# lppllppl920/EndoscopyDepthEstimation-Pytorch

Hardware: AMD Instinct MI355X
Metric: train frame-pairs/sec at 256x320 bs=8 (higher is better)
Workload: dtype f32

## Files before the change

endoscopydepthestimation-pytorch_amd/csrc/common.h:

```cpp
#pragma once

#include <hip/hip_runtime.h>
#include <stdint.h>

#include <map>
#include <mutex>
#include <utility>

#include "../../include/endo_hip.h"

#define ENDO_CHECK(expr)                                 \
    do {                                                 \
        hipError_t _e = (expr);                          \
        if (_e != hipSuccess) return static_cast<int>(_e); \
    } while (0)

#define ENDO_LAUNCH_CHECK() ENDO_CHECK(hipGetLastError())

namespace endo {

constexpr int kWave = 64;

__device__ __forceinline__ double wave_sum(double v) {
#pragma unroll
    for (int off = 32; off > 0; off >>= 1) v += __shfl_down(v, off, kWave);
    return v;
}

__device__ __forceinline__ float wave_sum(float v) {
#pragma unroll
    for (int off = 32; off > 0; off >>= 1) v += __shfl_down(v, off, kWave);
    return v;
}

constexpr int kBnSlots = 8;

__device__ __forceinline__ int64_t bn_slot_offset(int64_t slot_stride) {
    return static_cast<int64_t>((blockIdx.x + 11 * blockIdx.z) & (kBnSlots - 1)) * slot_stride;
}

__device__ __forceinline__ double bn_slot_sum(const double* __restrict__ s, int64_t slot_stride) {
    if (slot_stride == 0) return s[0];
    double t = 0.0;
#pragma unroll
    for (int k = 0; k < kBnSlots; ++k) t += s[k * slot_stride];
    return t;
}

typedef short bf16x4_bits __attribute__((ext_vector_type(4)));

__device__ __forceinline__ bf16x4_bits pack_bf16x4(float a, float b, float c, float d) {
    typedef float f32x2_t __attribute__((ext_vector_type(2)));
    typedef __bf16 bf16x2_t __attribute__((ext_vector_type(2)));
    typedef unsigned u32x2_t __attribute__((ext_vector_type(2)));
    const bf16x2_t lo = __builtin_convertvector(f32x2_t{a, b}, bf16x2_t), hi = __builtin_convertvector(f32x2_t{c, d}, bf16x2_t);
    return __builtin_bit_cast(bf16x4_bits, u32x2_t{__builtin_bit_cast(unsigned, lo), __builtin_bit_cast(unsigned, hi)});
}

typedef __bf16 bf16x8_t __attribute__((ext_vector_type(8)));
typedef float f32x4_acc __attribute__((ext_vector_type(4)));

__device__ __forceinline__ bf16x8_t pack_bf16x8(float a, float b, float c, float d, float e, float f, float g, float h) {
    typedef float f32x8_t __attribute__((ext_vector_type(8)));
    return __builtin_convertvector(f32x8_t{a, b, c, d, e, f, g, h}, bf16x8_t);
}

typedef unsigned u32x4_bits __attribute__((ext_vector_type(4)));

template <int K>
__device__ __forceinline__ void block_sum_atomic(const float (&part)[K], double* dst, double* scratch) {
    const int lane = threadIdx.x & 63;
    const int wave = threadIdx.x >> 6;
    const int nwave = (blockDim.x + 63) >> 6;
#pragma unroll
    for (int k = 0; k < K; ++k) {
        double v = wave_sum(static_cast<double>(part[k]));
        if (lane == 0) scratch[k * nwave + wave] = v;
    }
    __syncthreads();
    if (threadIdx.x < K) {
        double v = 0.0;
        for (int i = 0; i < nwave; ++i) v += scratch[threadIdx.x * nwave + i];
        atomicAdd(dst + threadIdx.x, v);
    }
    __syncthreads();
}

__device__ __forceinline__ int xcd_remap(int b, int total) {
    const int xcd = b & 7, idx = b >> 3;
    const int q = total >> 3, r = total & 7;
    return (xcd < r ? xcd * (q + 1) : r * (q + 1) + (xcd - r) * q) + idx;
}

struct TileWalk {
    int begin, end, step;
};

__host__ __device__ __forceinline__ TileWalk persistent_tile_walk(int r, int bpg, int t_total) {
    if ((bpg & 7) == 0) {
        const int q = bpg >> 3, xcd = r & 7, idx = r >> 3;
        return {static_cast<int>(static_cast<int64_t>(xcd * q) * t_total / bpg) + idx, static_cast<int>(static_cast<int64_t>((xcd + 1) * q) * t_total / bpg), q};
    }
    return {static_cast<int>(static_cast<int64_t>(r) * t_total / bpg), static_cast<int>(static_cast<int64_t>(r + 1) * t_total / bpg), 1};
}

inline int persistent_bpg(int blocks, int groups, int tiles_per_group) {
    int bpg = blocks / groups;
    if (bpg >= 8) bpg &= ~7;
    if (bpg > tiles_per_group) bpg = tiles_per_group;
    return bpg < 1 ? 1 : bpg;
}

inline int device_cu_count() {
    static std::mutex mu;
    static std::map<int, int> cus;
    int dev = 0;
    (void)hipGetDevice(&dev);
    std::lock_guard<std::mutex> lock(mu);
    int& n = cus[dev];
    if (n <= 0 && hipDeviceGetAttribute(&n, hipDeviceAttributeMultiprocessorCount, dev) != hipSuccess) n = 0;
    return n > 0 ? n : 256;
}

inline hipError_t ensure_dynamic_lds(const void* fn, size_t bytes) {
    if (bytes <= 48 * 1024) return hipSuccess;
    static std::mutex mu;
    static std::map<std::pair<const void*, int>, size_t> given;
    int dev = 0;
    (void)hipGetDevice(&dev);
    std::lock_guard<std::mutex> lock(mu);
    size_t& g = given[{fn, dev}];
    if (bytes <= g) return hipSuccess;
    const hipError_t e = hipFuncSetAttribute(fn, hipFuncAttributeMaxDynamicSharedMemorySize, static_cast<int>(bytes));
    if (e == hipSuccess) g = bytes;
    return e;
}

template <typename... Params, typename... Args>
inline hipError_t launch_dyn(void (*kernel)(Params...), dim3 grid, dim3 block, size_t smem, hipStream_t stream, Args&&... args) {
    const hipError_t e = ensure_dynamic_lds(reinterpret_cast<const void*>(kernel), smem);
    if (e != hipSuccess) return e;
    kernel<<<grid, block, smem, stream>>>(std::forward<Args>(args)...);
    return hipGetLastError();
}

}

int endo_depth_scale_fwd_impl(const float* pred, const float* sparse_depth, const float* sparse_mask, float* scaled, float* ratio, double* stats,
                              int n, int hw, float eps, int zero, hipStream_t stream);
int endo_depth_scale_bwd_impl(const float* grad_scaled, const float* grad_ratio, const float* pred, const float* sparse_depth, const double* stats,
                              float* grad_pred, double* work, int n, int hw, float eps, int zero, hipStream_t stream);
int endo_sparse_l1_fwd_impl(const float* flows, const float* flows_hat, const float* mask, float* loss, double* stats, int n, int c, int hw,
                            float eps, int zero, hipStream_t stream);

int endo_consistency_phase(int phase, const float* depth_1, const float* depth_2, const float* boundaries, const float* t_1_wrt_2,
                           const float* r_1_wrt_2, const float* t_2_wrt_1, const float* r_2_wrt_1, const float* intrinsics, float dcl_weight,
                           float eps, float* loss, float* grad_depth_1, float* grad_depth_2, float* workspace, int n, int h, int w,
                           int zero_grads, hipStream_t stream);

namespace endo {

struct ProfScope {
    int family;
    hipStream_t stream;
    void* slot;
    ProfScope(int family, hipStream_t stream, double flops, double bytes);
    ~ProfScope();
};

enum ProfFamily {
    kProfConv3x3Dense = 0,
    kProfConv3x3Up = 1,
    kProfConv1x1Pool = 2,
    kProfConvFirst = 3,
    kProfConvFinal = 4,
    kProfDgradDense = 5,
    kProfWgradDense = 6,
    kProfDgradOther = 7,
    kProfWgradOther = 8,
    kProfSmall = 9,
    kProfGeometry = 10,
    kProfLoss = 11,
    kProfOptimizer = 12,
};

}
```

endoscopydepthestimation-pytorch_amd/csrc/dgrad_wino_kernels.h:

```cpp
#pragma once

#include "dgrad_block_kernels.h"

namespace endo {

constexpr int kWinoDgradSlice = 16 * 12 * 16;
constexpr int kWinoDgradMaxLayers = 48;

struct WinoDgradTable {
    int layers;
    int start[kWinoDgradMaxLayers + 1];
    int cin[kWinoDgradMaxLayers];
    int groups[kWinoDgradMaxLayers];
    int64_t w_off[kWinoDgradMaxLayers];
    int64_t u_off[kWinoDgradMaxLayers];
};

static __global__ void __launch_bounds__(256) dgrad_wino_weights_kernel(const WinoDgradTable t, const float* __restrict__ params, float* __restrict__ u,
                                                                 int layout1_blocks = 0) {
    const int total = t.start[t.layers];
    for (int item = blockIdx.x * blockDim.x + threadIdx.x; item < total; item += gridDim.x * blockDim.x) {
        int l = 0;
        while (item >= t.start[l + 1]) ++l;
        const int e = item - t.start[l];
        const int j = e & 15, c = (e >> 4) % 12, grp = (e >> 4) / 12;
        const int ci = grp * 16 + j;
        float g[3][3];
#pragma unroll
        for (int a = 0; a < 3; ++a)
#pragma unroll
            for (int b = 0; b < 3; ++b) g[a][b] = 0.f;
        if (ci < t.cin[l]) {
            const float* src = params + t.w_off[l] + (static_cast<int64_t>(c) * t.cin[l] + ci) * 9;
#pragma unroll
            for (int a = 0; a < 3; ++a)
#pragma unroll
                for (int b = 0; b < 3; ++b) g[a][b] = src[(2 - a) * 3 + (2 - b)];
        }
        float h[4][3];
#pragma unroll
        for (int b = 0; b < 3; ++b) {
            h[0][b] = g[0][b];
            h[1][b] = 0.5f * (g[0][b] + g[1][b] + g[2][b]);
            h[2][b] = 0.5f * (g[0][b] - g[1][b] + g[2][b]);
            h[3][b] = g[2][b];
        }
        if ((layout1_blocks >> (l >> 2)) & 1) {
            float* dst = u + t.u_off[l] + static_cast<int64_t>(grp) * kWinoDgradSlice + (c * 64 + j) * 4;
#pragma unroll
            for (int a = 0; a < 4; ++a)
                *reinterpret_cast<f32x4*>(dst + a * 64) = f32x4{h[a][0], 0.5f * (h[a][0] + h[a][1] + h[a][2]), 0.5f * (h[a][0] - h[a][1] + h[a][2]), h[a][2]};
            continue;
        }
        float* dst = u + t.u_off[l] + static_cast<int64_t>(grp) * kWinoDgradSlice + c * 16 + j;
#pragma unroll
        for (int a = 0; a < 4; ++a) {
            dst[(4 * a + 0) * 192] = h[a][0];
            dst[(4 * a + 1) * 192] = 0.5f * (h[a][0] + h[a][1] + h[a][2]);
            dst[(4 * a + 2) * 192] = 0.5f * (h[a][0] - h[a][1] + h[a][2]);
            dst[(4 * a + 3) * 192] = h[a][2];
        }
    }
}

template <int NL>
struct DgradWino8Geom {
    static constexpr int kThreads = 512;
    static constexpr int kTileX = 32, kTileY = 8;
    static constexpr int kRows = kTileY + 2, kCols = kTileX + 2;
    static constexpr int kPlane = kRows * kCols;
    static constexpr int kCS = 352;
    static_assert(kCS >= kPlane && kCS % 64 == 32, "dY map stride");
    static constexpr int kU = kWinoDgradSlice;
    static constexpr int kUUnits = kU / 4;
    static constexpr int kRed = 4 * 16 * 2;
    static constexpr size_t kBytes = sizeof(float) * (NL * 12 * kCS + 2 * 2 * kU + 2 * 2 * kRed);
    static_assert(kBytes <= 160 * 1024, "one block per CU");
};

template <int NL, int EXP = 0>
__global__ void __launch_bounds__(512, 2) dgrad_wino8_kernel(const DgradBlockParams p0, const float* __restrict__ u0, const float* __restrict__ u1,
                                                             const float* __restrict__ u2, const float* __restrict__ u3) {
    using G = DgradWino8Geom<NL>;
    typedef float f32x2 __attribute__((ext_vector_type(2)));
    const int grp = p0.group_n > 0 ? blockIdx.z / p0.group_n : 0;
    const int n = blockIdx.z - grp * p0.group_n;
    const DgradBlockParams& p = p0;
    const int64_t grp_off = grp * p0.gs;
    extern __shared__ __attribute__((aligned(16))) float smem[];
    float* s_g = smem;
    float* s_u = s_g + NL * 12 * G::kCS;
    float* s_red = s_u + 4 * G::kU;

    const int tid = threadIdx.x;
    const int lane = tid & 63;
    const int wave = __builtin_amdgcn_readfirstlane(tid >> 6);
    const int half = wave >> 2, w4 = wave & 3;
    const int th = tid & 255;
    const int li = lane & 15;
    const int lk = lane >> 4;
    const int tile = (gridDim.x & 7) == 0 ? xcd_remap(blockIdx.x, gridDim.x) : blockIdx.x;
    const int x0 = (tile % p.tiles_x) * G::kTileX;
    const int y0 = (tile / p.tiles_x) * G::kTileY;
    const int px = x0 + 8 * lk;
    const int py = y0 + 2 * w4;
    const int ngroups = p.count / 16;
    const int g_per = (ngroups + gridDim.y - 1) / gridDim.y;
    const int g_begin = blockIdx.y * g_per;
    const int g_end = min(ngroups, g_begin + g_per);
    if (g_begin >= g_end) return;
    const int npairs = (g_end - g_begin + 1) / 2;
    const int nsteps = npairs * NL;
    const float* const u_layer[4] = {u0, u1, u2, u3};

    {
        int goff = 0;
        bool ok = false;
        if (tid < G::kPlane) {
            const int ry = tid / G::kCols, rx = tid - ry * G::kCols;
            const int gy = y0 - 1 + ry, gx = x0 - 1 + rx;
            if (gy >= 0 && gy < p.h && gx >= 0 && gx < p.w) { ok = true; goff = gy * p.g_w + gx; }
        }
        const float* g_n = p.g + grp_off + n * p.g_ns;
        const int e0 = wave * 64;
        if (e0 < G::kPlane) {
            for (int c = 0; c < NL * 12; ++c) {
                const float* src = ok ? g_n + static_cast<int64_t>(c) * p.g_cs + goff : g_pad_consts + 4;
                if (e0 + lane < G::kPlane) __builtin_amdgcn_global_load_lds((gptr_t)src, (lptr_t)(s_g + c * G::kCS + e0), 4, 0, 0);
            }
        }
    }

    auto step_group = [&](int step) { return g_begin + 2 * (step / NL) + half; };
    auto issue_weights = [&](int step, int buf) {
        const int gq = step_group(step), l = step % NL;
        if (gq >= g_end) return;
        const float* src = u_layer[l] + static_cast<int64_t>(gq) * G::kU + 4 * th;
        float* dst = s_u + (half * 2 + buf) * G::kU + w4 * 256;
#pragma unroll
        for (int k = 0; k < 3; ++k)
            __builtin_amdgcn_global_load_lds((gptr_t)(src + k * 1024), (lptr_t)(dst + k * 1024), 16, 0, 0);
    };

    const float* x_n = p.x + grp_off + n * p.ns;
    float* out_n = p.out + grp_off + n * p.ns;
    f32x4 xc[2][2], dc[2][2], total[2][2];
#pragma unroll
    for (int r = 0; r < 2; ++r)
#pragma unroll
        for (int hh = 0; hh < 2; ++hh) total[r][hh] = f32x4{0.f, 0.f, 0.f, 0.f};
    issue_weights(0, 0);
    asm volatile("s_waitcnt vmcnt(0)" ::: "memory");
    __syncthreads();

    for (int step = 0; step < nsteps; ++step) {
        const int buf = step & 1;
        const int gq = step_group(step), l = step % NL;
        const bool active = gq < g_end;
        const bool last_layer = (l == NL - 1);
        const int co = gq * 16 + li;
        float scale = 0.f, beta = 0.f, mean = 0.f, rstd = 0.f;
        if (active) {
            if (l == 0) {
#pragma unroll
                for (int r = 0; r < 2; ++r)
#pragma unroll
                    for (int hh = 0; hh < 2; ++hh) {
                        const int64_t o = static_cast<int64_t>(co) * p.cs + static_cast<int64_t>(py + r) * p.w + px + 4 * hh;
                        if constexpr ((EXP & 1) != 0) {
                            xc[r][hh] = f32x4{0.1f * lane, 0.2f, -0.3f, 0.4f}; dc[r][hh] = f32x4{0.f, 0.f, 0.f, 0.f};
                        } else {
                            xc[r][hh] = *reinterpret_cast<const f32x4*>(x_n + o);
                            dc[r][hh] = co >= p.acc_from ? *reinterpret_cast<const f32x4*>(out_n + o) : f32x4{0.f, 0.f, 0.f, 0.f};
                        }
                    }
            }
            mean = p.saved[l][grp_off + 2 * co]; rstd = p.saved[l][grp_off + 2 * co + 1];
            scale = p.gamma[l][co] * rstd;
            beta = p.beta[l][co];
        }
        if (step + 1 < nsteps && (!(EXP & 8) || step == 0)) issue_weights(step + 1, buf ^ 1);
        if (active) {
            f32x4 acc[16];
            const float* ub = s_u + (half * 2 + buf) * G::kU;
#pragma unroll
            for (int quad = 0; quad < 3; ++quad) {
                const float* a_base = s_g + (l * 12 + quad * 4 + lk) * G::kCS + (2 * w4) * G::kCols + 2 * li;
                const float* b_base = ub + (quad * 4 + lk) * 16 + li;
                f32x2 lo[4], hi[4];
#pragma unroll
                for (int row = 0; row < 4; ++row) {
                    lo[row] = *reinterpret_cast<const f32x2*>(a_base + row * G::kCols);
                    hi[row] = *reinterpret_cast<const f32x2*>(a_base + row * G::kCols + 2);
                }
                f32x2 tl[4], th2[4];
                tl[0] = lo[0] - lo[2]; th2[0] = hi[0] - hi[2];
                tl[1] = lo[1] + lo[2]; th2[1] = hi[1] + hi[2];
                tl[2] = lo[2] - lo[1]; th2[2] = hi[2] - hi[1];
                tl[3] = lo[1] - lo[3]; th2[3] = hi[1] - hi[3];
#pragma unroll
                for (int a = 0; a < 4; ++a) {
                    const float c0 = tl[a][0], c1 = tl[a][1], c2 = th2[a][0], c3 = th2[a][1];
                    float v0 = c0 - c2, v1 = c1 + c2, v2 = c2 - c1, v3 = c1 - c3;
                    if constexpr ((EXP & 64) != 0) { v0 = lo[a][0]; v1 = lo[a][1]; v2 = hi[a][0]; v3 = hi[a][1]; }
                    const float b0 = b_base[(4 * a + 0) * 192], b1 = b_base[(4 * a + 1) * 192];
                    const float b2 = b_base[(4 * a + 2) * 192], b3 = b_base[(4 * a + 3) * 192];
                    if constexpr ((EXP & 32) != 0) {
                        if (quad == 0) {
                            acc[4 * a + 0] = f32x4{v0 * b0, 0.f, 0.f, 0.f}; acc[4 * a + 1] = f32x4{v1 * b1, 0.f, 0.f, 0.f};
                            acc[4 * a + 2] = f32x4{v2 * b2, 0.f, 0.f, 0.f}; acc[4 * a + 3] = f32x4{v3 * b3, 0.f, 0.f, 0.f};
                        } else {
                            acc[4 * a + 0][quad] += v0 * b0; acc[4 * a + 1][quad] += v1 * b1;
                            acc[4 * a + 2][quad] += v2 * b2; acc[4 * a + 3][quad] += v3 * b3;
                        }
                    } else
// ... 101 lines not shown
```

endoscopydepthestimation-pytorch_amd/csrc/net.hip:

```cpp
#include <new>
#include <vector>

#include "dgrad_kernels.h"
#include "dgrad_block_kernels.h"
#include "dgrad_newmap_kernels.h"
#include "td_dgrad_kernels.h"
#include "td_fwd_kernels.h"
#include "wgrad_taps_kernels.h"
#include "wgrad1x1_kernels.h"
#include "wgrad_nsplit_kernels.h"
#include "wgrad_f34_kernels.h"
#include "wgrad_subpix_kernels.h"
#include "wino_fwd_kernels.h"
#include "wino4_fwd_kernels.h"
#include "dgrad_wino_kernels.h"
#include "dgrad_wino3_kernels.h"


namespace endo {

int run_dgrad_wino3_nl4(const DgradBlockParams& p, const float* const* u, hipStream_t stream);
bool dgrad_wino3p_applies(const DgradBlockParams& p);
int run_dgrad_wino3p_nl4(const DgradBlockParams& p, const float* const* u, int blocks, double* fw_parts, int* blocks_used, hipStream_t stream);

constexpr int kGrowth = 12;
constexpr int kLayers = 4;
constexpr int kFirst = 48;
constexpr int kLevels = 5;
constexpr int kNew = kGrowth * kLayers;
constexpr float kBnEps = 1.0e-5f;
constexpr float kBnMomentum = 0.1f;
constexpr int kSideStreamFromLevel = 0;

struct ConvP { int64_t w, b; int cout, cin, ks; int64_t u; int64_t ud; };
struct BnP { int64_t g, b; int c; int64_t run; int64_t saved; };

struct Table {
    ConvP first, final_;
    ConvP down_conv[kLevels][kLayers], td_conv[kLevels], bott_conv[kLayers], tu_conv[kLevels], up_conv[kLevels][kLayers];
    BnP down_bn[kLevels][kLayers], td_bn[kLevels], bott_bn[kLayers], up_bn[kLevels][kLayers];
    std::vector<int64_t> param_offsets;
    std::vector<BnP*> bn_order;
    int64_t param_floats = 0, bn_floats = 0, bn_width_total = 0;
    WinoWeightTable wino;
    WinoWeightTable wino4;
    int64_t wino4_floats = 0;
    int64_t wino_floats = 0;
    WinoDgradTable wino_dgrad;
    int64_t wino_dgrad_floats = 0;
};

inline int down_in(int level) { return kFirst + kNew * level; }
inline int level_channels(int level) { return level < kLevels ? 144 + down_in(level) : 288 + kNew; }

static const Table& table() {
    static Table* t = [] {
        Table* tb = new Table();
        int64_t off = 0;
        auto conv = [&](ConvP& c, int cout, int cin, int ks) {
            c.cout = cout; c.cin = cin; c.ks = ks; c.u = -1; c.ud = -1;
            c.w = off; tb->param_offsets.push_back(off); off += static_cast<int64_t>(cout) * cin * ks * ks;
            c.b = off; tb->param_offsets.push_back(off); off += cout;
        };
        int64_t run = 0, saved = 0;
        auto bn = [&](BnP& b, int c) {
            b.c = c;
            b.g = off; tb->param_offsets.push_back(off); off += c;
            b.b = off; tb->param_offsets.push_back(off); off += c;
            b.run = run; run += 2 * c;
            b.saved = saved; saved += c;
            tb->bn_order.push_back(&b);
        };
        conv(tb->first, kFirst, 3, 3);
        for (int l = 0; l < kLevels; ++l)
            for (int j = 0; j < kLayers; ++j) { bn(tb->down_bn[l][j], down_in(l) + kGrowth * j); conv(tb->down_conv[l][j], kGrowth, down_in(l) + kGrowth * j, 3); }
        for (int l = 0; l < kLevels; ++l) { bn(tb->td_bn[l], down_in(l) + kNew); conv(tb->td_conv[l], down_in(l) + kNew, down_in(l) + kNew, 1); }
        for (int j = 0; j < kLayers; ++j) { bn(tb->bott_bn[j], 288 + kGrowth * j); conv(tb->bott_conv[j], kGrowth, 288 + kGrowth * j, 3); }
        for (int i = 0; i < kLevels; ++i) conv(tb->tu_conv[i], kNew, kNew, 3);
        for (int i = 0; i < kLevels; ++i) {
            const int l = kLevels - 1 - i;
            for (int j = 0; j < kLayers; ++j) { const int cin = 96 + down_in(l) + kGrowth * j; bn(tb->up_bn[i][j], cin); conv(tb->up_conv[i][j], kGrowth, cin, 3); }
        }
        conv(tb->final_, 1, 192, 1);
        tb->param_floats = off;
        tb->bn_floats = run;
        tb->bn_width_total = saved;
        {
            WinoWeightTable& wt = tb->wino;
            wt.layers = 0; wt.start[0] = 0;
            int64_t uoff = 0;
            auto add = [&](ConvP& c) {
                const int l = wt.layers++;
                c.u = uoff;
                wt.cin[l] = c.cin; wt.cout[l] = c.cout; wt.w_off[l] = c.w; wt.u_off[l] = uoff;
                wt.start[l + 1] = wt.start[l] + c.cin * 16;
                uoff += static_cast<int64_t>(c.cin) * kWinoUStride;
            };
            for (int l = 0; l < kLevels; ++l) for (int j = 0; j < kLayers; ++j) add(tb->down_conv[l][j]);
            for (int j = 0; j < kLayers; ++j) add(tb->bott_conv[j]);
            for (int i = 0; i < kLevels; ++i) for (int j = 0; j < kLayers; ++j) add(tb->up_conv[i][j]);
            tb->wino_floats = uoff;
            tb->wino4 = wt;
            int64_t u4 = 0;
            for (int l = 0; l < wt.layers; ++l) { tb->wino4.u_off[l] = u4; u4 += static_cast<int64_t>(wt.cin[l]) * kW4UStride; }
            tb->wino4_floats = u4;
        }
        {
            WinoDgradTable& wd = tb->wino_dgrad;
            wd.layers = 0; wd.start[0] = 0;
            int64_t uoff = 0;
            auto add = [&](ConvP& c, int base) {
                const int l = wd.layers++;
                c.ud = uoff;
                wd.cin[l] = c.cin; wd.groups[l] = base / 16; wd.w_off[l] = c.w; wd.u_off[l] = uoff;
                wd.start[l + 1] = wd.start[l] + 16 * wd.groups[l] * 12;
                uoff += static_cast<int64_t>(wd.groups[l]) * kWinoDgradSlice;
            };
            for (int l = 0; l < kLevels; ++l) for (int j = 0; j < kLayers; ++j) add(tb->down_conv[l][j], down_in(l));
            for (int j = 0; j < kLayers; ++j) add(tb->bott_conv[j], 288);
            for (int i = 0; i < kLevels; ++i) for (int j = 0; j < kLayers; ++j) add(tb->up_conv[i][j], 96 + down_in(kLevels - 1 - i));
            tb->wino_dgrad_floats = uoff;
        }
        return tb;
    }();
    return *t;
}

}

using namespace endo;

struct endo_net {
    int n, h, w;
    int groups;
    int64_t gs;
    struct Level { int h, w, t; int64_t plane; int64_t act, grad; int64_t sums; int64_t pq; } lv[kLevels + 1];
    int64_t pre_off;
    int64_t saved_off;
    int64_t idx_off[kLevels];
    int64_t sums_off;
    int64_t sums_bytes;
    int64_t tape_floats;
    int64_t partial_off;
    int64_t wino_off;
    int64_t wino4_off;
    int64_t pq_off;
    int64_t pq_floats;
    int64_t scratch_off;
    int64_t scratch_bytes;
    int64_t slot_stride;
    int64_t wg_scratch_off;
    int64_t tuw_scratch_off;
    int64_t wd_off;
    int64_t gplane_off;
    int64_t bias_parts_off;
    int64_t fw_parts_off;
    int64_t bias_parts_floats;
    int64_t gradws_floats;
    hipStream_t wstream;
    hipEvent_t ev_fork, ev_join;
    int opt[ENDO_OPT_COUNT];
};

namespace endo {


constexpr int kBiasPartChannels = 2048;
constexpr int kBiasPartLaunches = 64;
constexpr int kFwPartBlocks = 512;
struct BiasReduceTable {
    int n;
    struct Entry { const float* parts; float* bias; int count; int nparts; } e[kBiasPartLaunches];
};
struct BiasParts {
    BiasReduceTable table;
    int64_t used;
};

struct BnFin4 {
    const double* scratch[4];
    const float* saved[4];
    const float* gamma[4];
    float* ggamma[4];
    float* gbeta[4];
};

__global__ void __launch_bounds__(256) prep_dy_kernel(float* __restrict__ dbuf, const float* __restrict__ x, int64_t ns, int plane,
                                                      const float* __restrict__ pq_p, const float* __restrict__ pq_q,
                                                      float* bias_grad, int group_n, int64_t gs, const BnFin4 fin, int nl,
                                                      double count, int training, int64_t slot_stride,
                                                      const float* __restrict__ vg, const float* __restrict__ vw, float* __restrict__ parts) {
    __shared__ double scratch[4];
    const int c = blockIdx.y;
    const int grp = blockIdx.z / group_n, n = blockIdx.z - grp * group_n;
    float pc = pq_p[grp * gs + c], qc = pq_q[grp * gs + c];
    if (nl > 0) {
        const int64_t go = grp * gs;
        double dp = 0.0, dq = 0.0;
#pragma unroll
        for (int j = 0; j < 4; ++j) {
            if (j >= nl) break;
            const double s1 = bn_slot_sum(fin.scratch[j] + go / 2 + 2 * c, slot_stride);
            const double s2 = bn_slot_sum(fin.scratch[j] + go / 2 + 2 * c + 1, slot_stride);
            if (blockIdx.x == 0 && n == 0 && threadIdx.x == 0) {
                atomicAdd(fin.ggamma[j] + c, static_cast<float>(s2));
                atomicAdd(fin.gbeta[j] + c, static_cast<float>(s1));
            }
            if (training) {
                const double mean = fin.saved[j][go + 2 * c], rstd = fin.saved[j][go + 2 * c + 1];
                const double scale = fin.gamma[j][c] * rstd;
                const double k = scale * rstd * s2 / count;
                dp += static_cast<double>(static_cast<float>(-k));
                dq += static_cast<double>(static_cast<float>(-scale * s1 / count + k * mean));
            }
        }
        pc += static_cast<float>(dp);
        qc += static_cast<float>(dq);
    }
    const int64_t base = grp * gs + n * ns + static_cast<int64_t>(c) * plane;
    const float* vg_n = vg ? vg + grp * gs + static_cast<int64_t>(n) * plane : nullptr;
    const float wf = vg ? vw[c] : 0.f;
    float part = 0.f;
    if ((plane & 3) == 0 && !vg_n) {
        const int stride = gridDim.x * blockDim.x * 4;
        int i = (blockIdx.x * blockDim.x + threadIdx.x) * 4;
        for (; i + stride < plane; i += 2 * stride) {
            f32x4 g0 = *reinterpret_cast<const f32x4*>(dbuf + base + i);
            f32x4 g1 = *reinterpret_cast<const f32x4*>(dbuf + base + i + stride);
            const f32x4 x0 = *reinterpret_cast<const f32x4*>(x + base + i);
            const f32x4 x1 = *reinterpret_cast<const f32x4*>(x + base + i + stride);
#pragma unroll
            for (int e = 0; e < 4; ++e) { g0[e] += fmaf(pc, x0[e], qc); part += g0[e]; }
#pragma unroll
            for (int e = 0; e < 4; ++e) { g1[e] += fmaf(pc, x1[e], qc); part += g1[e]; }
            *reinterpret_cast<f32x4*>(dbuf + base + i) = g0;
            *reinterpret_cast<f32x4*>(dbuf + base + i + stride) = g1;
        }
        for (; i < plane; i += stride) {
            f32x4 g = *reinterpret_cast<const f32x4*>(dbuf + base + i);
            const f32x4 xv = *reinterpret_cast<const f32x4*>(x + base + i);
#pragma unroll
            for (int e = 0; e < 4; ++e) { g[e] += fmaf(pc, xv[e], qc); part += g[e]; }
            *reinterpret_cast<f32x4*>(dbuf + base + i) = g;
        }
    } else if ((plane & 3) == 0) {
        for (int i = (blockIdx.x * blockDim.x + threadIdx.x) * 4; i < plane; i += gridDim.x * blockDim.x * 4) {
            f32x4 g;
            if (vg_n) {
                const f32x4 gv = *reinterpret_cast<const f32x4*>(vg_n + i);
                g = f32x4{gv[0] * wf, gv[1] * wf, gv[2] * wf, gv[3] * wf};
            } else {
                g = *reinterpret_cast<const f32x4*>(dbuf + base + i);
            }
            const f32x4 xv = *reinterpret_cast<const f32x4*>(x + base + i);
#pragma unroll
            for (int e = 0; e < 4; ++e) { g[e] += fmaf(pc, xv[e], qc); part += g[e]; }
            *reinterpret_cast<f32x4*>(dbuf + base + i) = g;
        }
    } else {
        for (int i = blockIdx.x * blockDim.x + threadIdx.x; i < plane; i += gridDim.x * blockDim.x) {
            const float g = (vg_n ? vg_n[i] * wf : dbuf[base + i]) + fmaf(pc, x[base + i], qc);
            dbuf[base + i] = g;
            part += g;
        }
    }
    const int lane = threadIdx.x & 63, wave = threadIdx.x >> 6;
    double v = wave_sum(static_cast<double>(part));
    if (lane == 0) scratch[wave] = v;
    __syncthreads();
    if (threadIdx.x == 0 && bias_grad) {
        const float t = static_cast<float>(scratch[0] + scratch[1] + scratch[2] + scratch[3]);
        if (parts) parts[(static_cast<int64_t>(c) * gridDim.z + blockIdx.z) * gridDim.x + blockIdx.x] = t;
        else atomicAdd(bias_grad + c, t);
    }
}

__global__ void __launch_bounds__(256) bias_reduce_kernel(const BiasReduceTable tb) {
    const BiasReduceTable::Entry& e = tb.e[blockIdx.x];
    const int lane = threadIdx.x & 63, wave = threadIdx.x >> 6;
    for (int c = blockIdx.y * 4 + wave; c < e.count; c += gridDim.y * 4) {
        const float* src = e.parts + static_cast<int64_t>(c) * e.nparts;
        double t = 0.0;
        for (int i = lane; i < e.nparts; i += 64) t += static_cast<double>(src[i]);
        t = wave_sum(t);
        if (lane == 0) e.bias[c] += static_cast<float>(t);
    }
}

__global__ void bn_bwd_finalize_kernel(const double* __restrict__ scratch, const float* __restrict__ saved,
                                       const float* __restrict__ gamma, float* __restrict__ ggamma, float* __restrict__ gbeta,
                                       float* __restrict__ pq_p, float* __restrict__ pq_q, int c_count, double count, int training,
                                       int64_t gs, int64_t slot_stride) {
    scratch += blockIdx.y * (gs / 2); saved += blockIdx.y * gs; pq_p += blockIdx.y * gs; pq_q += blockIdx.y * gs;
    for (int c = blockIdx.x * blockDim.x + threadIdx.x; c < c_count; c += gridDim.x * blockDim.x) {
        const double s1 = bn_slot_sum(scratch + 2 * c, slot_stride), s2 = bn_slot_sum(scratch + 2 * c + 1, slot_stride);
        atomicAdd(ggamma + c, static_cast<float>(s2));
        atomicAdd(gbeta + c, static_cast<float>(s1));
        if (training) {
            const double mean = saved[2 * c], rstd = saved[2 * c + 1];
            const double scale = gamma[c] * rstd;
            const double k = scale * rstd * s2 / count;
            pq_p[c] += static_cast<float>(-k);
            pq_q[c] += static_cast<float>(-scale * s1 / count + k * mean);
        }
    }
}

__global__ void bn_bwd_finalize4_kernel(const BnFin4 a, int nl, float* __restrict__ pq_p, float* __restrict__ pq_q, int c_count, double count,
                                        int training, int64_t gs, int64_t slot_stride) {
    const int64_t go = blockIdx.y * gs;
    pq_p += go; pq_q += go;
    for (int c = blockIdx.x * blockDim.x + threadIdx.x; c < c_count; c += gridDim.x * blockDim.x) {
        double dp = 0.0, dq = 0.0;
#pragma unroll
        for (int j = 0; j < 4; ++j) {
            if (j >= nl) break;
            const double s1 = bn_slot_sum(a.scratch[j] + go / 2 + 2 * c, slot_stride);
            const double s2 = bn_slot_sum(a.scratch[j] + go / 2 + 2 * c + 1, slot_stride);
            atomicAdd(a.ggamma[j] + c, static_cast<float>(s2));
            atomicAdd(a.gbeta[j] + c, static_cast<float>(s1));
            if (training) {
                const double mean = a.saved[j][go + 2 * c], rstd = a.saved[j][go + 2 * c + 1];
                const double scale = a.gamma[j][c] * rstd;
                const double k = scale * rstd * s2 / count;
                dp += static_cast<double>(static_cast<float>(-k));
                dq += static_cast<double>(static_cast<float>(-scale * s1 / count + k * mean));
            }
        }
        if (training) {
            pq_p[c] += static_cast<float>(dp);
            pq_q[c] += static_cast<float>(dq);
        }
    }
}

__global__ void tu_phase_weights_kernel(const float* __restrict__ w, int cout, int cin, float* __restrict__ out) {
    constexpr int kPhW = 2 * 12 * 16 + 16;
    const int total = 2 * cin * 2 * 12 * 16;
    for (int i = blockIdx.x * blockDim.x + threadIdx.x; i < total; i += gridDim.x * blockDim.x) {
        const int lane16 = i & 15;
        const int slot = (i >> 4) % 12;
        const int t = (i / (16 * 12)) & 1;
        const int ci = (i / (16 * 12 * 2)) % cin;
        const int a = i / (16 * 12 * 2 * cin);
        int ctap, tile;
        if (slot < 3) { ctap = 0; tile = slot; } else if (slot < 9) { ctap = 1; tile = slot - 3; } else { ctap = 2; tile = slot - 9 + 3; }
        const int b = tile / 3, co = (tile % 3) * 16 + lane16;
        float v = 0.f;
        if (co < cout) {
            const float* src = w + (static_cast<int64_t>(co) * cin + ci) * 9;
            const int ky0 = a == 0 ? (t == 0 ? 0 : 1) : (t == 0 ? 0 : 2), ky1 = a == 0 ? (t == 0 ? 0 : 2) : (t == 0 ? 1 : 2);
            int kx0, kx1;
            if (b == 0) { kx0 = ctap == 0 ? 0 : 1; kx1 = ctap == 0 ? 0 : 2; }
            else { kx0 = ctap == 1 ? 0 : 2; kx1 = ctap == 1 ? 1 : 2; }
            for (int ky = ky0; ky <= ky1; ++ky)
                for (int kx = kx0; kx <= kx1; ++kx) v += src[ky * 3 + kx];
        }
        out[(static_cast<int64_t>(a) * cin + ci) * kPhW + (t * 12 + slot) * 16 + lane16] = v;
    }
}

__global__ void tu_subpix_dgrad_weights_kernel(const float* __restrict__ w, int cout, int cin, float* __restrict__ out) {
    const int pitch = 4 * cin + 16;
    const int total = 4 * cout * 4 * cin;
    for (int i = blockIdx.x * blockDim.x + threadIdx.x; i < total; i += gridDim.x * blockDim.x) {
        const int ci = i % cin;
        const int tap = (i / cin) & 3;
        const int co = (i / (4 * cin)) % cout;
        const int ph = i / (4 * cin * cout);
        const int alpha = ph >> 1, beta = ph & 1, tyi = tap >> 1, txi = tap & 1;
        const int ky0 = alpha == 0 ? (tyi == 0 ? 1 : 0) : (tyi == 0 ? 2 : 0), ky1 = alpha == 0 ? (tyi == 0 ? 2 : 0) : (tyi == 0 ? 2 : 1);
        const int kx0 = beta == 0 ? (txi == 0 ? 1 : 0) : (txi == 0 ? 2 : 0), kx1 = beta == 0 ? (txi == 0 ? 2 : 0) : (txi == 0 ? 2 : 1);
        const float* src = w + (static_cast<int64_t>(co) * cin + ci) * 9;
        float v = 0.f;
        for (int ky = ky0; ky <= ky1; ++ky)
            for (int kx = kx0; kx <= kx1; ++kx) v += src[ky * 3 + kx];
        out[static_cast<int64_t>(ph * cout + co) * pitch + tap * cin + ci] = v;
    }
}

__global__ void __launch_bounds__(256) finalize_partial_kernel(const float* __restrict__ partial, int64_t split_stride, int ksplit,
                                                               int64_t pns, int plane, const float* __restrict__ bias,
                                                               float* __restrict__ out, int64_t out_ns, double* out_sums,
                                                               int group_n, int64_t gs) {
    __shared__ double scratch[2 * 4];
    const int c = blockIdx.y;
    const int grp = blockIdx.z / group_n, n = blockIdx.z - grp * group_n;
    partial += grp * gs; out += grp * gs;
    if (out_sums) out_sums += grp * (gs / 2);
    const float b = bias[c];
    float part[2] = {0.f, 0.f};
    for (int i = blockIdx.x * blockDim.x + threadIdx.x; i < plane; i += gridDim.x * blockDim.x) {
        float v = b;
        for (int s = 0; s < ksplit; ++s) v += partial[s * split_stride + n * pns + static_cast<int64_t>(c) * plane + i];
        out[n * out_ns + static_cast<int64_t>(c) * plane + i] = v;
        part[0] += v;
        part[1] += v * v;
    }
    if (out_sums) block_sum_atomic<2>(part, out_sums + 2 * c, scratch);
}

__global__ void __launch_bounds__(256) final_fwd_kernel(const float* __restrict__ u, int64_t ns, int plane, int cin,
                                                        const float* __restrict__ wgt, const float* __restrict__ bias,
                                                        float* __restrict__ pre, float* __restrict__ out, int group_n, int64_t gs, int c_first) {
    __shared__ float s_w[192];
    for (int c = threadIdx.x; c < cin; c += blockDim.x) s_w[c] = wgt[c];
    __syncthreads();
    const int grp = blockIdx.y / group_n, n = blockIdx.y - grp * group_n;
    u += grp * gs;
    if (pre) pre += grp * gs;
    out += static_cast<int64_t>(grp) * group_n * plane;
    const bool vec = (plane & 3) == 0;
    if (vec) {
        for (int i = (blockIdx.x * blockDim.x + threadIdx.x) * 4; i < plane; i += gridDim.x * blockDim.x * 4) {
            f32x4 acc = {0.f, 0.f, 0.f, 0.f};
            if (c_first > 0) acc = *reinterpret_cast<const f32x4*>(pre + static_cast<int64_t>(n) * plane + i);
            const float* src = u + n * ns + i;
            for (int c = c_first; c < cin; ++c) {
                const f32x4 v = *reinterpret_cast<const f32x4*>(src + static_cast<int64_t>(c) * plane);
                const float wc = s_w[c];
                acc[0] = fmaf(v[0], wc, acc[0]); acc[1] = fmaf(v[1], wc, acc[1]);
                acc[2] = fmaf(v[2], wc, acc[2]); acc[3] = fmaf(v[3], wc, acc[3]);
            }
            const float b = bias[0];
            f32x4 o;
            for (int e = 0; e < 4; ++e) { acc[e] += b; o[e] = fabsf(acc[e]); }
            if (pre) *reinterpret_cast<f32x4*>(pre + static_cast<int64_t>(n) * plane + i) = acc;
            *reinterpret_cast<f32x4*>(out + static_cast<int64_t>(n) * plane + i) = o;
        }
    } else {
        for (int i = blockIdx.x * blockDim.x + threadIdx.x; i < plane; i += gridDim.x * blockDim.x) {
            float acc = c_first > 0 ? pre[static_cast<int64_t>(n) * plane + i] : 0.f;
            for (int c = c_first; c < cin; ++c) acc = fmaf(u[n * ns + static_cast<int64_t>(c) * plane + i], s_w[c], acc);
            acc += bias[0];
            if (pre) pre[static_cast<int64_t>(n) * plane + i] = acc;
            out[static_cast<int64_t>(n) * plane + i] = fabsf(acc);
        }
    }
}

__device__ __forceinline__ float sign_of(float v) { return v > 0.f ? 1.f : (v < 0.f ? -1.f : 0.f); }

__global__ void __launch_bounds__(256) final_g_kernel(const float* __restrict__ gout, const float* __restrict__ pre, float* __restrict__ g,
                                                      int plane, int group_n, int64_t gs) {
    const int grp = blockIdx.y / group_n, n = blockIdx.y - grp * group_n;
    gout += static_cast<int64_t>(blockIdx.y) * plane; pre += grp * gs + static_cast<int64_t>(n) * plane; g += grp * gs + static_cast<int64_t>(n) * plane;
    for (int i = blockIdx.x * blockDim.x + threadIdx.x; i < plane; i += gridDim.x * blockDim.x) g[i] = gout[i] * sign_of(pre[i]);
}

__global__ void __launch_bounds__(256) final_bwd_data_kernel(const float* __restrict__ gout, const float* __restrict__ pre,
                                                             const float* __restrict__ wgt, float* __restrict__ dbuf,
                                                             int64_t ns, int plane, int cin, int group_n, int64_t gs, int c_first) {
    __shared__ float s_w[192];
    for (int c = threadIdx.x; c < cin; c += blockDim.x) s_w[c] = wgt[c];
    __syncthreads();
    const int grp = blockIdx.y / group_n, n = blockIdx.y - grp * group_n;
    gout += static_cast<int64_t>(grp) * group_n * plane; pre += grp * gs; dbuf += grp * gs;
    for (int i = blockIdx.x * blockDim.x + threadIdx.x; i < plane; i += gridDim.x * blockDim.x) {
        const float g = gout[static_cast<int64_t>(n) * plane + i] * sign_of(pre[static_cast<int64_t>(n) * plane + i]);
        for (int c = c_first; c < cin; ++c) dbuf[n * ns + static_cast<int64_t>(c) * plane + i] = g * s_w[c];
    }
}

__global__ void __launch_bounds__(256) final_bwd_weight_kernel(const float* __restrict__ gout, const float* __restrict__ pre,
                                                               const float* __restrict__ u, int64_t ns, int plane, int cin,
                                                               int group_n, int64_t gs, float* __restrict__ gw, float* __restrict__ gb, int c_first) {
    __shared__ double scratch[4];
    const int c = c_first + blockIdx.x;
    const int grp = blockIdx.z / group_n, n = blockIdx.z - grp * group_n;
    const float* gp = gout + static_cast<int64_t>(blockIdx.z) * plane;
    const float* pp = pre + grp * gs + static_cast<int64_t>(n) * plane;
    const float* up = u + grp * gs + n * ns + static_cast<int64_t>(c < cin ? c : 0) * plane;
    float part = 0.f, part2 = 0.f;
    if ((plane & 3) == 0) {
        const int stride = gridDim.y * blockDim.x * 4;
        for (int i = (blockIdx.y * blockDim.x + threadIdx.x) * 4; i < plane; i += stride) {
            const f32x4 gv = *reinterpret_cast<const f32x4*>(gp + i);
            const f32x4 pv = *reinterpret_cast<const f32x4*>(pp + i);
            f32x4 uv = {1.f, 1.f, 1.f, 1.f};
            if (c < cin) uv = *reinterpret_cast<const f32x4*>(up + i);
            part += gv[0] * sign_of(pv[0]) * uv[0] + gv[1] * sign_of(pv[1]) * uv[1];
            part2 += gv[2] * sign_of(pv[2]) * uv[2] + gv[3] * sign_of(pv[3]) * uv[3];
        }
    } else {
        for (int i = blockIdx.y * blockDim.x + threadIdx.x; i < plane; i += gridDim.y * blockDim.x)
            part += gp[i] * sign_of(pp[i]) * (c < cin ? up[i] : 1.f);
    }
    const int lane = threadIdx.x & 63, wave = threadIdx.x >> 6;
    double v = wave_sum(static_cast<double>(part + part2));
    if (lane == 0) scratch[wave] = v;
    __syncthreads();
    if (threadIdx.x == 0) {
        const float t = static_cast<float>(scratch[0] + scratch[1] + scratch[2] + scratch[3]);
        if (c < cin) atomicAdd(gw + c, t); else atomicAdd(gb, t);
    }
}

__global__ void __launch_bounds__(64) final_w_reduce_kernel(const double* __restrict__ parts, int nblocks, int count, float* __restrict__ gw) {
    const int c = blockIdx.x;
    double t = 0.0;
    for (int b = threadIdx.x; b < nblocks; b += 64) t += parts[static_cast<int64_t>(b) * count + c];
    t = wave_sum(t);
    if (threadIdx.x == 0) atomicAdd(gw + c, static_cast<float>(t));
}

constexpr int kBlocks = 2 * kLevels + 1, kDense = kBlocks * kLayers;

enum class DenseFwd { Wino4, Wino2_32x16, Wino2_32x8, SplitK, Direct32x8, Direct16x8, DirectAuto };
struct FwdPlan {
    struct Dense {
        DenseFwd form;
        int ksplit;
        bool chunk_weights;
    } dense[kDense];
    bool bf16;
    bool wino4_weights;
    bool fuse_final;
    bool td_persistent[kLevels];
    bool tu_subpix[kLevels];
};

enum class NewMap { Bf16, Persistent, Vec16, Dword };
enum class BasePass { Block8, Block8Bf16, Wino3, Wino3Persistent, Wino8 };
enum class DenseWgrad { F34, NSplit, Taps, Direct };
enum class TdDgrad { Persistent, Runs128, Dma, Staged };
enum class TuWgrad { Subpix, Taps, Direct };
enum class TuDgrad { Subpix32x8, Subpix16x8, Subpix16x4, Plain };
enum class FirstWgrad { F34Prep, F34, Taps, Direct };
struct BwdPlan {
    struct Block {
        bool fused;
        NewMap newmap[kLayers];
        BasePass base;
        bool wino3_layout;
    } block[kBlocks];
    DenseWgrad wgrad[kDense];
    bool td_wgrad_dma[kLevels];
    TdDgrad td_dgrad[kLevels];
    TuWgrad tu_wgrad[kLevels];
    TuDgrad tu_dgrad[kLevels];
    int overlap;
    bool bf16_wgrad, bf16_dgrad;
    bool dgrad_weights;
    bool use_virt;
    bool virt_base;
    bool virt_base_w;
    int materialise;
    int c_first;
    FirstWgrad first;
};

struct Ctx {
    const endo_net* net;
    const float* params;
    float* bn_running;
    float* tape;
    float* grads;
    float* gradws;
    int training;
    hipStream_t stream;
    BiasParts* bias_parts = nullptr;
    const float* x = nullptr;
    const FwdPlan* fwd = nullptr;
    const BwdPlan* bwd = nullptr;

    int nt() const { return net->n * net->groups; }
    int fork_wgrad(Ctx& side, int level) const {
        side = *this;
        if (!net->wstream || !bwd->overlap || level < kSideStreamFromLevel) return 0;
        ENDO_CHECK(hipEventRecord(net->ev_fork, stream));
        ENDO_CHECK(hipStreamWaitEvent(net->wstream, net->ev_fork, 0));
        side.stream = net->wstream;
        return 0;
    }
    float* act(int level) const { return tape + net->lv[level].act; }
    float* gbuf(int level) const { return gradws + net->lv[level].grad; }
    double* sums(int level) const { return reinterpret_cast<double*>(reinterpret_cast<char*>(tape) + net->sums_off) + net->lv[level].sums; }
    double* out_sums(int level, int channel) const { return training ? sums(level) + 2 * channel : nullptr; }
    float* saved(const BnP& b) const { return tape + net->saved_off + 2 * b.saved; }
    double* scratch(const BnP& b) const { return reinterpret_cast<double*>(reinterpret_cast<char*>(gradws) + net->scratch_off) + 2 * b.saved; }
    float* pq_p(int level) const { return gradws + net->pq_off + 2 * net->lv[level].pq; }
    float* pq_q(int level) const { return pq_p(level) + net->lv[level].t; }
    uint8_t* idx(int level) const { return reinterpret_cast<uint8_t*>(tape) + net->idx_off[level]; }
};

static void fill_bn_in(const Ctx& c, ConvParams& p, const BnP& b, int level, int ic0) {
    const auto& lv = c.net->lv[level];
    p.in_sums = c.sums(level) + 2 * ic0;
    p.gamma = c.params + b.g;
    p.beta = c.params + b.b;
    p.running_mean = c.bn_running + b.run;
    p.running_var = c.bn_running + b.run + b.c;
    p.saved = c.tape ? c.saved(b) : nullptr;
    p.count = static_cast<double>(c.net->n) * lv.h * lv.w;
    p.eps = kBnEps;
    p.momentum = kBnMomentum;
    p.training = c.training;
}

static void fill_in(const Ctx& c, ConvParams& p, const float* base, int level, int ic0, int cin) {
    const auto& lv = c.net->lv[level];
    p.in = base + ic0 * lv.plane;
    p.in_ns = lv.t * lv.plane;
    p.in_cs = static_cast<int>(lv.plane);
    p.in_w = lv.w;
    p.cin = cin;
}

static void fill_out(const Ctx& c, ConvParams& p, float* base, int level, int oc0, int cout) {
    const auto& lv = c.net->lv[level];
    p.out = base + oc0 * lv.plane;
    p.out_ns = lv.t * lv.plane;
    p.out_cs = static_cast<int>(lv.plane);
    p.out_w = lv.w;
    p.cout = cout;
}

static void fill_grid(const Ctx& c, ConvParams& p, int level) {
    const auto& lv = c.net->lv[level];
    p.n = c.nt(); p.h = lv.h; p.w = lv.w;
    p.group_n = c.net->n; p.gs = c.net->gs; p.in_gs = c.net->gs; p.out_gs = c.net->gs;
}

static double conv_flops(const endo_net* net, int level, int cin, int cout, int ks) {
    return 2.0 * net->n * net->groups * net->lv[level].plane * cin * cout * ks * ks;
}

static void default_options(int (&opt)[ENDO_OPT_COUNT]) {
    opt[ENDO_OPT_WINO_FWD] = 5;
    opt[ENDO_OPT_WINO_DGRAD] = 3;
    opt[ENDO_OPT_DGRAD_VEC] = 2;
    opt[ENDO_OPT_WINO_MIN_TILES] = 1024;
    opt[ENDO_OPT_MFMA_BF16] = 0;
    opt[ENDO_OPT_WGRAD_OVERLAP] = 1;
    opt[ENDO_OPT_WGRAD_F34] = 1;
    opt[ENDO_OPT_FINAL_VIRTUAL] = 1;
    opt[ENDO_OPT_TD_PERSIST] = 3;
}
static int bf16_mask(const int* opt) { const int v = opt[ENDO_OPT_MFMA_BF16]; return v == 1 ? 7 : (v >> 1); }

struct DenseBlock { int level, ic0, c0; const BnP* bn; const ConvP* cv; bool base_overwrite; };
static DenseBlock dense_block(int b) {
    const Table& tb = table();
    if (b < kLevels) return {b, 48, down_in(b), tb.down_bn[b], tb.down_conv[b], false};
    if (b == kLevels) return {kLevels, 0, 288, tb.bott_bn, tb.bott_conv, true};
    const int i = b - kLevels - 1, l = kLevels - 1 - i;
    return {l, 0, 96 + down_in(l), tb.up_bn[i], tb.up_conv[i], l > 0};
}
static long tile_count(const Ctx& c, int level, int tx, int ty) {
    const auto& lv = c.net->lv[level];
    return static_cast<long>((lv.w + tx - 1) / tx) * ((lv.h + ty - 1) / ty) * c.nt();
}

static ConvParams dense_fwd_params(const Ctx& c, const DenseBlock& k, int j, DenseFwd form) {
    const ConvP& cv = k.cv[j];
    const int oc0 = k.ic0 + k.c0 + kGrowth * j;
    ConvParams p{};
    fill_grid(c, p, k.level);
    fill_in(c, p, c.act(k.level), k.level, k.ic0, cv.cin);
    fill_bn_in(c, p, k.bn[j], k.level, k.ic0);
    p.wgt = c.params + cv.w; p.bias = c.params + cv.b; p.w_cout = cv.cout; p.w_cin = cv.cin;
    fill_out(c, p, c.act(k.level), k.level, oc0, cv.cout);
    p.out_sums = c.out_sums(k.level, oc0);
    if (form == DenseFwd::Wino4) p.wgt = c.tape + c.net->wino4_off + cv.u / kWinoUStride * kW4UStride;
    if (form == DenseFwd::Wino2_32x16 || form == DenseFwd::Wino2_32x8) p.wgt = c.tape + c.net->wino_off + cv.u;
    return p;
}

static ConvParams td_fwd_params(const Ctx& c, int level) {
    const BnP& b = table().td_bn[level];
    const ConvP& cv = table().td_conv[level];
    const int next = level + 1;
    const int oc0 = next < kLevels ? 48 : 0;
    ConvParams p{};
    fill_grid(c, p, level);
    fill_in(c, p, c.act(level), level, 48, cv.cin);
    fill_bn_in(c, p, b, level, 48);
    p.wgt = c.params + cv.w; p.bias = c.params + cv.b; p.w_cout = cv.cout; p.w_cin = cv.cin;
    fill_out(c, p, c.act(next), next, oc0, cv.cout);
    p.out_idx = c.idx(level);
    p.idx_ns = static_cast<int64_t>(cv.cout) * c.net->lv[next].plane;
    p.out_sums = c.out_sums(next, oc0);
    return p;
}

static FwdPlan plan_fwd(const Ctx& c) {
    const int* opt = c.net->opt;
    const int mode = opt[ENDO_OPT_WINO_FWD];
    const long min_tiles = opt[ENDO_OPT_WINO_MIN_TILES];
    FwdPlan pl{};
    pl.bf16 = (bf16_mask(opt) & 2) != 0;
    pl.wino4_weights = !pl.bf16 && mode == 5;
    for (int b = 0; b < kBlocks; ++b) {
        const DenseBlock k = dense_block(b);
        const long t64x16 = tile_count(c, k.level, 64, 16), t32x16 = tile_count(c, k.level, 32, 16), t32x8 = tile_count(c, k.level, 32, 8);
        const long t16x16 = tile_count(c, k.level, 16, 16), t16x8 = tile_count(c, k.level, 16, 8);
        const bool big = t32x16 >= min_tiles, small = t32x8 >= (min_tiles * 3) / 4;
        const bool wino4_tiles = mode == 5 && !pl.bf16 && 2 * t64x16 >= min_tiles;
        const bool wino2_tiles = mode != 0 && !pl.bf16 && (big || small);
        for (int j = 0; j < kLayers; ++j) {
            FwdPlan::Dense& d = pl.dense[b * kLayers + j];
            const int nchunks = (k.cv[j].cin + 15) / 16;
            d.chunk_weights = !pl.bf16 && !wino4_tiles && !wino2_tiles;
            if (wino4_tiles && wino4_fwd_ok(dense_fwd_params(c, k, j, DenseFwd::Wino4))) {
                d.form = DenseFwd::Wino4;
            } else if (wino2_tiles && wino_fwd_ok(dense_fwd_params(c, k, j, DenseFwd::Wino2_32x16))) {
                d.form = big ? DenseFwd::Wino2_32x16 : DenseFwd::Wino2_32x8;
            } else if (t32x16 < 512 && t16x16 < 384 && t16x8 < 512 && nchunks >= 4) {
                int want = static_cast<int>(((t16x8 < 256 ? 512 : 768) + t16x8 - 1) / t16x8);
                if (want > nchunks) want = nchunks;
                const int per = (nchunks + want - 1) / want;
                d.form = DenseFwd::SplitK;
                d.ksplit = (nchunks + per - 1) / per;
            } else {
                d.form = (t32x16 < 1024 && t32x8 >= 1024) ? DenseFwd::Direct32x8
                       : (t32x16 < 1024 && t16x8 >= 768) ? DenseFwd::Direct16x8 : DenseFwd::DirectAuto;
            }
        }
    }
    pl.fuse_final = opt[ENDO_OPT_FINAL_VIRTUAL] && pl.dense[kDense - 1].form == DenseFwd::Wino4;
    for (int l = 0; l < kLevels; ++l) {
        pl.td_persistent[l] = (opt[ENDO_OPT_TD_PERSIST] & 2) && !pl.bf16 && c.training && td_fwd_ok(td_fwd_params(c, l));
        const ConvP& tu = table().tu_conv[kLevels - 1 - l];
        pl.tu_subpix[l] = c.net->lv[l + 1].w % 4 == 0 && tu.cout == kNew && tu.cin % 4 == 0;
    }
    return pl;
}

static int dense_fwd(const Ctx& c, int b, int j) {
    const DenseBlock k = dense_block(b);
    const FwdPlan::Dense& d = c.fwd->dense[b * kLayers + j];
    const ConvP& cv = k.cv[j];
    const auto& lv = c.net->lv[k.level];
    const int oc0 = k.ic0 + k.c0 + kGrowth * j;
    ConvParams p = dense_fwd_params(c, k, j, d.form);
    ProfScope prof(kProfConv3x3Dense, c.stream, conv_flops(c.net, k.level, cv.cin, cv.cout, 3),
                   4.0 * c.nt() * lv.plane * (cv.cin + cv.cout));
    const float* chunk_weights = d.chunk_weights ? c.tape + c.net->wino_off + cv.u : nullptr;
    const bool bf16 = c.fwd->bf16;
    switch (d.form) {
        case DenseFwd::Wino4:
            if (c.fwd->fuse_final && b == kBlocks - 1 && j == kLayers - 1) { p.fin_w = c.params + table().final_.w + k.ic0; p.fin_out = c.tape + c.net->pre_off; }
            return launch_wino4_fwd(p, c.stream);
        case DenseFwd::Wino2_32x16:
            return launch_wino_fwd<2, 4, 2>(p, c.stream);
        case DenseFwd::Wino2_32x8:
            return launch_wino_fwd<1, 4, 3>(p, c.stream);
        case DenseFwd::SplitK: {
            float* partial = c.tape + c.net->partial_off;
            p.ksplit = d.ksplit;
            p.split_stride = static_cast<int64_t>(c.net->n) * cv.cout * lv.plane;
            p.out = partial; p.out_ns = static_cast<int64_t>(cv.cout) * lv.plane;
            p.bias = nullptr; p.out_sums = nullptr;
            p.wgt_chunks = chunk_weights;
            int rc = bf16 ? launch_conv_dma<3, 16, 1, IN_BNRELU, EPI_FWD, 1, 2, 2, 1, 1>(p, c.stream)
                          : launch_conv_dma<3, 16, 1, IN_BNRELU, EPI_FWD, 1, 2, 2, 1>(p, c.stream);
            if (rc) return rc;
            int bx = static_cast<int>((lv.plane + 255) / 256);
            bx = bx > 8 ? 8 : bx;
            finalize_partial_kernel<<<dim3(bx, cv.cout, c.nt()), 256, 0, c.stream>>>(
                partial, p.split_stride, d.ksplit, p.out_ns, static_cast<int>(lv.plane), c.params + cv.b, c.act(k.level) + oc0 * lv.plane,
                lv.t * lv.plane, c.out_sums(k.level, oc0), c.net->n, c.net->gs);
            ENDO_LAUNCH_CHECK();
            return 0;
        }
        case DenseFwd::Direct32x8:
            return bf16 ? launch_conv_dma<3, 4, 1, IN_BNRELU, EPI_FWD, 2, 4, 2, 1, 1>(p, c.stream) : launch_conv_dma<3, 4, 1, IN_BNRELU, EPI_FWD, 2, 4, 2, 1>(p, c.stream);
        case DenseFwd::Direct16x8:
            return bf16 ? launch_conv_dma<3, 8, 1, IN_BNRELU, EPI_FWD, 1, 2, 2, 1, 1>(p, c.stream) : launch_conv_dma<3, 8, 1, IN_BNRELU, EPI_FWD, 1, 2, 2, 1>(p, c.stream);
        case DenseFwd::DirectAuto:
            if (bf16) return launch_conv_dma_auto<3, 4, 1, IN_BNRELU, EPI_FWD, 8, 2, 1, 1>(p, c.stream);
            p.wgt_chunks = chunk_weights;
            return launch_conv_dma_auto<3, 4, 1, IN_BNRELU, EPI_FWD, 8, 2, 1>(p, c.stream);
    }
    return ENDO_E_BADARG;
}

static int td_fwd(const Ctx& c, int level) {
    const ConvP& cv = table().td_conv[level];
    const ConvParams p = td_fwd_params(c, level);
    ProfScope prof(kProfConv1x1Pool, c.stream, conv_flops(c.net, level, cv.cin, cv.cout, 1),
                   4.0 * c.nt() * c.net->lv[level].plane * (cv.cin + cv.cout / 4.0));
    if (c.fwd->td_persistent[level]) return launch_td_fwd(p, device_cu_count(), c.stream);
    if (c.fwd->bf16) return launch_conv_dma_auto<1, 8, 3, IN_BNRELU, EPI_FWD_POOL, 4, 2, 1, 1>(p, c.stream);
    return launch_conv_dma_auto<1, 8, 3, IN_BNRELU, EPI_FWD_POOL, 4>(p, c.stream);
}

static int tu_fwd(const Ctx& c, int level, int src_level, int src_c0, const ConvP& cv) {
    ProfScope prof(kProfConv3x3Up, c.stream, conv_flops(c.net, level, cv.cin, cv.cout, 3),
                   4.0 * c.nt() * c.net->lv[level].plane * (cv.cin / 4.0 + cv.cout));
    if (c.fwd->tu_subpix[level]) {
        float* w3 = c.tape + c.net->partial_off;
        tu_phase_weights_kernel<<<(2 * cv.cin * 384 + 255) / 256, 256, 0, c.stream>>>(c.params + cv.w, cv.cout, cv.cin, w3);
        ENDO_LAUNCH_CHECK();
        ConvParams p{};
        fill_grid(c, p, src_level);
        fill_in(c, p, c.act(src_level), src_level, src_c0, cv.cin);
        p.wgt = w3; p.w_cout = 2 * cv.cout; p.w_cin = cv.cin;
        p.bias = c.params + cv.b;
        fill_out(c, p, c.act(level), level, 0, cv.cout);
        p.out_sums = c.out_sums(level, 0);
        return launch_conv_dma_vec<3, 4, 6, IN_PLAIN, EPI_FWD, 2, 4, 2, 1, 4, 0, 0, 2>(p, c.stream);
    }
    ConvParams p{};
    fill_grid(c, p, level);
    fill_in(c, p, c.act(src_level), src_level, src_c0, cv.cin);
    p.wgt = c.params + cv.w; p.bias = c.params + cv.b; p.w_cout = cv.cout; p.w_cin = cv.cin;
    fill_out(c, p, c.act(level), level, 0, cv.cout);
    p.out_sums = c.out_sums(level, 0);
    return launch_conv_dma_auto<3, 4, 3, IN_UPSAMPLE, EPI_FWD>(p, c.stream);
}

struct FinalVirt { const float* vg; const float* vw; float* gw; };

static int prep_dy(const Ctx& c, int level, int c0, int count, float* bias_grad, const BnFin4* fin = nullptr, int nl = 0, const FinalVirt* fv = nullptr) {
    const auto& lv = c.net->lv[level];
    BnFin4 none{};
    int bx = static_cast<int>((lv.plane + 4095) / 4096);
    bx = bx < 1 ? 1 : (bx > 32 ? 32 : bx);
    float* parts = nullptr;
    if (bias_grad && c.bias_parts) {
        BiasParts& bp = *c.bias_parts;
        const int64_t need = static_cast<int64_t>(count) * c.nt() * bx;
        if (bp.table.n >= kBiasPartLaunches || bp.used + need > c.net->bias_parts_floats) return ENDO_E_UNSUPPORTED;
        parts = c.gradws + c.net->bias_parts_off + bp.used;
        bp.table.e[bp.table.n++] = {parts, bias_grad, count, c.nt() * bx};
        bp.used += need;
    }
    ProfScope prof(kProfSmall, c.stream, 0.0, 12.0 * c.nt() * lv.plane * count);
    prep_dy_kernel<<<dim3(bx, count, c.nt()), 256, 0, c.stream>>>(c.gbuf(level) + c0 * lv.plane, c.act(level) + c0 * lv.plane,
                                                                     lv.t * lv.plane, static_cast<int>(lv.plane), c.pq_p(level) + c0,
                                                                     c.pq_q(level) + c0, bias_grad, c.net->n, c.net->gs, fin ? *fin : none, fin ? nl : 0,
                                                                     static_cast<double>(c.net->n) * lv.h * lv.w, c.training, c.net->slot_stride,
                                                                     fv ? fv->vg : nullptr, fv ? fv->vw + c0 : nullptr, parts);
    ENDO_LAUNCH_CHECK();
    return 0;
}

static int bn_finalize(const Ctx& c, const BnP& b, int level, int ic0, int first = 0, int count = -1) {
    const auto& lv = c.net->lv[level];
    if (count < 0) count = b.c - first;
    if (count <= 0) return 0;
    ProfScope prof(kProfSmall, c.stream, 0.0, 0.0);
    bn_bwd_finalize_kernel<<<dim3((count + 127) / 128, c.net->groups), 128, 0, c.stream>>>(c.scratch(b) + 2 * first, c.saved(b) + 2 * first, c.params + b.g + first,
                                                                       c.grads + b.g + first, c.grads + b.b + first,
                                                                       c.pq_p(level) + ic0 + first, c.pq_q(level) + ic0 + first, count,
                                                                       static_cast<double>(c.net->n) * lv.h * lv.w, c.training, c.net->gs, c.net->slot_stride);
    ENDO_LAUNCH_CHECK();
    return 0;
}

static void fill_wgrad_grid(const Ctx& c, WgradParams& p, int level) {
    const auto& lv = c.net->lv[level];
    p.n = c.nt(); p.h = lv.h; p.w = lv.w;
    p.group_n = c.net->n; p.gs = c.net->gs; p.in_gs = c.net->gs;
    p.tiles_x = (lv.w + kWgTileX - 1) / kWgTileX;
    p.tiles_y = (lv.h + kWgTileY - 1) / kWgTileY;
}

static WgradParams dense_wgrad_params(const Ctx& c, const DenseBlock& k, int j) {
    const auto& lv = c.net->lv[k.level];
    const BnP& b = k.bn[j];
    const ConvP& cv = k.cv[j];
    const int oc0 = k.ic0 + k.c0 + kGrowth * j;
    WgradParams p{};
    fill_wgrad_grid(c, p, k.level);
    p.in = c.act(k.level) + k.ic0 * lv.plane; p.in_ns = lv.t * lv.plane; p.in_cs = static_cast<int>(lv.plane); p.in_w = lv.w; p.cin = cv.cin;
    p.saved = c.saved(b); p.gamma = c.params + b.g; p.beta = c.params + b.b;
    p.dy = c.gbuf(k.level) + oc0 * lv.plane; p.dy_ns = lv.t * lv.plane; p.dy_cs = static_cast<int>(lv.plane); p.dy_w = lv.w; p.cout = cv.cout;
    p.dw = c.grads + cv.w;
    return p;
}

static void fill_dgrad_block(const Ctx& c, DgradBlockParams& p, int level) {
    const auto& lv = c.net->lv[level];
    p.n = c.nt(); p.h = lv.h; p.w = lv.w;
    p.group_n = c.net->n; p.gs = c.net->gs; p.slot_stride = c.net->slot_stride;
    p.g_ns = lv.t * lv.plane; p.g_cs = static_cast<int>(lv.plane); p.g_w = lv.w;
    p.ns = lv.t * lv.plane; p.cs = static_cast<int>(lv.plane);
}

static DgradBlockParams newmap_params(const Ctx& c, const DenseBlock& k, int j, BnFin4* a = nullptr) {
    const auto& lv = c.net->lv[k.level];
    const int nl = kLayers - j;
    const int t0 = k.c0 + kGrowth * (j - 1);
    DgradBlockParams p{};
    fill_dgrad_block(c, p, k.level);
    p.g = c.gbuf(k.level) + (k.ic0 + k.c0 + kGrowth * j) * lv.plane;
    p.x = c.act(k.level) + (k.ic0 + t0) * lv.plane;
    p.out = c.gbuf(k.level) + (k.ic0 + t0) * lv.plane;
    p.count = kGrowth;
    p.acc_from = 0;
    p.w_ci_off = t0;
    for (int l = 0; l < nl; ++l) {
        const BnP& b = k.bn[j + l];
        p.wgt[l] = c.params + k.cv[j + l].w; p.w_cin[l] = k.cv[j + l].cin;
        p.saved[l] = c.saved(b) + 2 * t0; p.gamma[l] = c.params + b.g + t0; p.beta[l] = c.params + b.b + t0;
        p.scratch[l] = c.scratch(b) + 2 * t0;
        if (a) { a->scratch[l] = p.scratch[l]; a->saved[l] = p.saved[l]; a->gamma[l] = p.gamma[l]; a->ggamma[l] = c.grads + b.g + t0; a->gbeta[l] = c.grads + b.b + t0; }
    }
    return p;
}

static DgradBlockParams base_pass_params(const Ctx& c, const DenseBlock& k) {
    const auto& lv = c.net->lv[k.level];
    DgradBlockParams p{};
    fill_dgrad_block(c, p, k.level);
    p.g = c.gbuf(k.level) + (k.ic0 + k.c0) * lv.plane;
    p.x = c.act(k.level) + k.ic0 * lv.plane;
    p.out = c.gbuf(k.level) + k.ic0 * lv.plane;
    p.count = k.c0;
    p.acc_from = k.base_overwrite ? k.c0 : 0;
    p.w_ci_off = 0;
    for (int j = 0; j < kLayers; ++j) {
        p.wgt[j] = c.params + k.cv[j].w; p.w_cin[j] = k.cv[j].cin;
        p.saved[j] = c.saved(k.bn[j]); p.gamma[j] = c.params + k.bn[j].g; p.beta[j] = c.params + k.bn[j].b;
        p.scratch[j] = c.scratch(k.bn[j]);
    }
    return p;
}

static WgradParams td_wgrad_params(const Ctx& c, int level) {
    const BnP& b = table().td_bn[level];
    const ConvP& cv = table().td_conv[level];
    const int next = level + 1, oc0 = next < kLevels ? 48 : 0;
    const auto& lv = c.net->lv[level];
    const auto& nx = c.net->lv[next];
    WgradParams p{};
    fill_wgrad_grid(c, p, level);
    p.in = c.act(level) + 48 * lv.plane; p.in_ns = lv.t * lv.plane; p.in_cs = static_cast<int>(lv.plane); p.in_w = lv.w; p.cin = cv.cin;
    p.saved = c.saved(b); p.gamma = c.params + b.g; p.beta = c.params + b.b;
    p.dy = c.gbuf(next) + oc0 * nx.plane; p.dy_ns = nx.t * nx.plane; p.dy_cs = static_cast<int>(nx.plane); p.dy_w = nx.w; p.cout = cv.cout;
    p.dy_idx = c.idx(level); p.idx_ns = static_cast<int64_t>(cv.cout) * nx.plane;
    p.dw = c.grads + cv.w;
    return p;
}

static ConvParams td_dgrad_params(const Ctx& c, int level) {
    const BnP& b = table().td_bn[level];
    const ConvP& cv = table().td_conv[level];
    const int next = level + 1, oc0 = next < kLevels ? 48 : 0;
    const auto& lv = c.net->lv[level];
    ConvParams p{};
    fill_grid(c, p, level);
    fill_in(c, p, c.gbuf(next), next, oc0, cv.cout);
    p.in_idx = c.idx(level); p.idx_ns = static_cast<int64_t>(cv.cout) * c.net->lv[next].plane;
    p.wgt = c.params + cv.w; p.w_cout = cv.cout; p.w_cin = cv.cin;
    fill_out(c, p, c.gbuf(level), level, 48, cv.cin);
    p.x = c.act(level) + 48 * lv.plane; p.x_ns = lv.t * lv.plane; p.x_cs = static_cast<int>(lv.plane);
    p.bn_saved = c.saved(b); p.bn_gamma = c.params + b.g; p.bn_beta = c.params + b.b;
    p.bn_scratch = c.scratch(b); p.bn_slot_stride = c.net->slot_stride;
    p.acc_from = 0;
    return p;
}

static WgradParams tu_wgrad_params(const Ctx& c, int level, bool subpix) {
    const ConvP& cv = table().tu_conv[kLevels - 1 - level];
    const int src_level = level + 1, src_c0 = src_level == kLevels ? 288 : 96 + down_in(src_level);
    const auto& lv = c.net->lv[level];
    const auto& sv = c.net->lv[src_level];
    WgradParams p{};
    fill_wgrad_grid(c, p, level);
    p.in = c.act(src_level) + src_c0 * sv.plane; p.in_ns = sv.t * sv.plane; p.in_cs = static_cast<int>(sv.plane); p.in_w = sv.w; p.cin = cv.cin;
    p.dy = c.gbuf(level); p.dy_ns = lv.t * lv.plane; p.dy_cs = static_cast<int>(lv.plane); p.dy_w = lv.w; p.cout = cv.cout;
    p.dw = c.grads + cv.w;
    if (subpix) { p.h = sv.h; p.w = sv.w; }
    return p;
}

static WgradParams first_wgrad_params(const Ctx& c) {
    const auto& lv = c.net->lv[0];
    WgradParams p{};
    fill_wgrad_grid(c, p, 0);
    p.in = c.x; p.in_ns = 3 * lv.plane; p.in_cs = static_cast<int>(lv.plane); p.in_w = lv.w; p.cin = 3;
    p.in_gs = c.net->n * p.in_ns;
    p.dy = c.gbuf(0) + 48 * lv.plane; p.dy_ns = lv.t * lv.plane; p.dy_cs = static_cast<int>(lv.plane); p.dy_w = lv.w; p.cout = kFirst;
    p.dw = c.grads + table().first.w;
    return p;
}

static BwdPlan plan_bwd(const Ctx& c) {
    const int* opt = c.net->opt;
    const int wino_dgrad = opt[ENDO_OPT_WINO_DGRAD];
    const long min_tiles = opt[ENDO_OPT_WINO_MIN_TILES];
    BwdPlan pl{};
    pl.overlap = opt[ENDO_OPT_WGRAD_OVERLAP];
    pl.bf16_wgrad = (bf16_mask(opt) & 1) != 0;
    pl.bf16_dgrad = (bf16_mask(opt) & 4) != 0;
    const bool f34 = opt[ENDO_OPT_WGRAD_F34] && !pl.bf16_wgrad;
    const long f34_min_tiles = min_tiles / 4;
    pl.dgrad_weights = wino_dgrad != 0 && !pl.bf16_dgrad;
    for (int b = 0; b < kBlocks; ++b) {
        const DenseBlock k = dense_block(b);
        const auto& lv = c.net->lv[k.level];
        BwdPlan::Block& bl = pl.block[b];
        const DgradBlockParams base = base_pass_params(c, k);
        bl.fused = dgrad_block_ok(base);
        const long wtiles = static_cast<long>(lv.w / 32) * (lv.h / 8) * c.nt();
        if (pl.bf16_dgrad) bl.base = BasePass::Block8Bf16;
        else if (wino_dgrad != 0 && dgrad_wino_ok(base) && wtiles >= min_tiles)
            bl.base = !((wino_dgrad == 1 || wino_dgrad == 3) && dgrad_wino3_ok(base)) ? BasePass::Wino8
                    : (wino_dgrad == 3 && dgrad_wino3p_applies(base)) ? BasePass::Wino3Persistent : BasePass::Wino3;
        else bl.base = BasePass::Block8;
        bl.wino3_layout = bl.base == BasePass::Wino3 || bl.base == BasePass::Wino3Persistent;
        for (int j = 1; j < kLayers; ++j) {
            const DgradBlockParams p = newmap_params(c, k, j);
            const bool vec = dgrad_block_vec_ok(p);
            bl.newmap[j] = (pl.bf16_dgrad && vec) ? NewMap::Bf16 : (vec && opt[ENDO_OPT_DGRAD_VEC] >= 2 && dgrad_newmap_ok(p)) ? NewMap::Persistent
                         : (vec && opt[ENDO_OPT_DGRAD_VEC] != 0) ? NewMap::Vec16 : NewMap::Dword;
        }
        for (int j = 0; j < kLayers; ++j) {
            const WgradParams p = dense_wgrad_params(c, k, j);
            pl.wgrad[b * kLayers + j] = (f34 && wgrad_f34_ok(p, f34_min_tiles)) ? DenseWgrad::F34 : wgrad_nsplit_ok(p) ? DenseWgrad::NSplit
                                      : wgrad_taps_ok(p) ? DenseWgrad::Taps : DenseWgrad::Direct;
        }
    }
    for (int l = 0; l < kLevels; ++l) {
        const auto& sv = c.net->lv[l + 1];
        pl.td_wgrad_dma[l] = wgrad1x1_dma_ok(td_wgrad_params(c, l));
        const ConvParams td = td_dgrad_params(c, l);
        const bool persist = (opt[ENDO_OPT_TD_PERSIST] & 1) && !pl.bf16_dgrad;
        pl.td_dgrad[l] = (persist && td_dgrad_ok(td)) ? TdDgrad::Persistent : (persist && sv.w % 4 != 0 && td_dgrad_small_ok(td)) ? TdDgrad::Runs128
                       : sv.w % 4 == 0 ? TdDgrad::Dma : TdDgrad::Staged;
        const ConvP& tu = table().tu_conv[kLevels - 1 - l];
        pl.tu_wgrad[l] = tu_wgrad_subpix_ok(tu_wgrad_params(c, l, true)) ? TuWgrad::Subpix : wgrad_taps_ok(tu_wgrad_params(c, l, false), true) ? TuWgrad::Taps : TuWgrad::Direct;
        pl.tu_dgrad[l] = !(sv.w % 4 == 0 && tu.cin == kNew && tu.cout == kNew) ? TuDgrad::Plain : tile_count(c, l + 1, 32, 8) >= 1024 ? TuDgrad::Subpix32x8
                       : tile_count(c, l + 1, 16, 8) >= 512 ? TuDgrad::Subpix16x8 : TuDgrad::Subpix16x4;
    }
    const BwdPlan::Block& last = pl.block[kBlocks - 1];
    const int last_base = dense_block(kBlocks - 1).c0;
    pl.use_virt = opt[ENDO_OPT_FINAL_VIRTUAL] && last.fused;
    pl.virt_base = pl.use_virt && last.wino3_layout;
    pl.virt_base_w = pl.use_virt && last.base == BasePass::Wino3Persistent;
    pl.materialise = !pl.use_virt ? 192 : (pl.virt_base ? 0 : last_base);
    pl.c_first = pl.virt_base_w ? last_base : 0;
    const WgradParams first = first_wgrad_params(c);
    pl.first = (f34 && wgrad_f34_raw_ok(first, f34_min_tiles)) ? (opt[ENDO_OPT_FINAL_VIRTUAL] ? FirstWgrad::F34Prep : FirstWgrad::F34)
             : wgrad_taps_ok(first) ? FirstWgrad::Taps : FirstWgrad::Direct;
    return pl;
}

static int dense_wgrad(const Ctx& c, int b, int j, F34ReduceBatch* batch = nullptr, int slice = 0) {
    const DenseBlock k = dense_block(b);
    const ConvP& cv = k.cv[j];
    const auto& lv = c.net->lv[k.level];
    const WgradParams p = dense_wgrad_params(c, k, j);
    float* scratch = c.gradws + c.net->wg_scratch_off;
    ProfScope prof(kProfWgradDense, c.stream, conv_flops(c.net, k.level, cv.cin, cv.cout, 3), 4.0 * c.nt() * lv.plane * (cv.cin + cv.cout));
    switch (c.bwd->wgrad[b * kLayers + j]) {
        case DenseWgrad::F34: return launch_wgrad_f34(p, scratch + (batch ? slice : 0) * kF34ScratchFloats, c.stream, batch);
        case DenseWgrad::NSplit: return launch_wgrad_nsplit(p, scratch, c.stream, c.bwd->bf16_wgrad);
        case DenseWgrad::Taps: return c.bwd->bf16_wgrad ? launch_wgrad_taps<12, IN_BNRELU, 1>(p, c.stream) : launch_wgrad_taps<12, IN_BNRELU>(p, c.stream);
        case DenseWgrad::Direct: return launch_wgrad<3, 1, IN_BNRELU, DY_PLAIN>(p, c.stream);
    }
    return ENDO_E_BADARG;
}

static int dense_bwd(const Ctx& c, int b, int j, int acc_from) {
    const DenseBlock k = dense_block(b);
    const BnP& bn = k.bn[j];
    const ConvP& cv = k.cv[j];
    const int level = k.level, ic0 = k.ic0, oc0 = k.ic0 + k.c0 + kGrowth * j;
    const auto& lv = c.net->lv[level];
    int rc = prep_dy(c, level, oc0, cv.cout, c.grads + cv.b);
    if (rc) return rc;
    {
        Ctx cw;
        rc = c.fork_wgrad(cw, level);
        if (rc) return rc;
        rc = dense_wgrad(cw, b, j);
        if (rc) return rc;
    }
    {
        ConvParams p{};
        fill_grid(c, p, level);
        fill_in(c, p, c.gbuf(level), level, oc0, cv.cout);
        p.wgt = c.params + cv.w; p.w_cout = cv.cout; p.w_cin = cv.cin;
        fill_out(c, p, c.gbuf(level), level, ic0, cv.cin);
        p.x = c.act(level) + ic0 * lv.plane; p.x_ns = lv.t * lv.plane; p.x_cs = static_cast<int>(lv.plane);
        p.bn_saved = c.saved(bn); p.bn_gamma = c.params + bn.g; p.bn_beta = c.params + bn.b;
        p.bn_scratch = c.scratch(bn); p.bn_slot_stride = c.net->slot_stride;
        p.acc_from = acc_from - ic0;
        ProfScope prof(kProfDgradDense, c.stream, conv_flops(c.net, level, cv.cin, cv.cout, 3), 4.0 * c.nt() * lv.plane * (3.0 * cv.cin + cv.cout));
        rc = launch_dgrad_dense_auto(p, c.stream);
        if (rc) return rc;
    }
    return bn_finalize(c, bn, level, ic0);
}

template <int NL>
static int launch_newmap(NewMap form, const DgradBlockParams& p, hipStream_t stream) {
    switch (form) {
        case NewMap::Bf16: return launch_dgrad_block<NL, 2, 3, 1, 0, 4, 1>(p, stream);
        case NewMap::Persistent: return launch_dgrad_newmap<NL>(p, stream);
        case NewMap::Vec16: return launch_dgrad_block<NL, 2, 3, 1, 0, 4>(p, stream);
        case NewMap::Dword: return launch_dgrad_block<NL, 2, 3>(p, stream);
    }
    return ENDO_E_BADARG;
}

static int dense_block_bwd(const Ctx& c, int b, const FinalVirt* fv = nullptr) {
    const DenseBlock k = dense_block(b);
    const BwdPlan::Block& bl = c.bwd->block[b];
    const int level = k.level, ic0 = k.ic0, c0 = k.c0, new0 = ic0 + c0;
    const auto& lv = c.net->lv[level];
    if (!bl.fused) {
        for (int j = kLayers - 1; j >= 0; --j) {
            const int acc_from = (j == kLayers - 1 && k.base_overwrite) ? new0 : 0;
            int rc = dense_bwd(c, b, j, acc_from < ic0 ? ic0 : acc_from);
            if (rc) return rc;
        }
        return 0;
    }
    BnFin4 pending{};
    int pending_nl = 0;
    F34ReduceBatch red{};
    for (int j = kLayers - 1; j >= 0; --j) {
        int rc = prep_dy(c, level, new0 + kGrowth * j, kGrowth, c.grads + k.cv[j].b, &pending, pending_nl, (fv && j == kLayers - 1) ? fv : nullptr);
        if (rc) return rc;
        const bool defer = c.bwd->overlap == 2;
        if (!defer || j == 0) {
            Ctx cw;
            rc = c.fork_wgrad(cw, level);
            if (rc) return rc;
            for (int jj = defer ? kLayers - 1 : j; jj >= j; --jj) {
                rc = dense_wgrad(cw, b, jj, &red, jj);
                if (rc) return rc;
            }
            if (j == 0 && red.count > 0) {
                ProfScope prof(kProfSmall, cw.stream, 0.0, 0.0);
                rc = launch_wgrad_f34_reduce_batch(red, cw.stream);
                if (rc) return rc;
            }
        }
        if (j > 0) {
            const int nl = kLayers - j;
            BnFin4 a{};
            DgradBlockParams p = newmap_params(c, k, j, &a);
            if (fv) { p.vg = fv->vg; p.vw = fv->vw + ic0 + p.w_ci_off; }
            ProfScope prof(kProfDgradDense, c.stream, 2.0 * c.nt() * lv.plane * kGrowth * kGrowth * 9 * nl,
                           4.0 * c.nt() * lv.plane * (3.0 * kGrowth + kGrowth * nl));
            rc = nl == 1 ? launch_newmap<1>(bl.newmap[j], p, c.stream) : nl == 2 ? launch_newmap<2>(bl.newmap[j], p, c.stream) : launch_newmap<3>(bl.newmap[j], p, c.stream);
            if (rc) return rc;
            pending = a;
            pending_nl = nl;
        }
    }
    {
        DgradBlockParams p = base_pass_params(c, k);
        const bool virt = fv && c.bwd->virt_base;
        if (virt) { p.vg = fv->vg; p.vw = fv->vw + ic0; }
        ProfScope prof(kProfDgradDense, c.stream, 2.0 * c.nt() * lv.plane * c0 * kGrowth * 9 * kLayers,
                       4.0 * c.nt() * lv.plane * (3.0 * c0 + kGrowth * kLayers));
        const float* ub = c.gradws + c.net->wd_off;
        const float* const u[4] = {ub + k.cv[0].ud, ub + k.cv[1].ud, ub + k.cv[2].ud, ub + k.cv[3].ud};
        int rc = 0;
        switch (bl.base) {
            case BasePass::Block8Bf16: rc = launch_dgrad_block8<4, 1>(p, c.stream); break;
            case BasePass::Block8: rc = launch_dgrad_block8<4>(p, c.stream); break;
            case BasePass::Wino8: rc = launch_dgrad_wino8<4>(p, u, c.stream); break;
            case BasePass::Wino3: rc = run_dgrad_wino3_nl4(p, u, c.stream); break;
            case BasePass::Wino3Persistent: {
                double* fwp = (virt && c.bwd->virt_base_w) ? reinterpret_cast<double*>(c.gradws + c.net->fw_parts_off) : nullptr;
                int used = 0;
                rc = run_dgrad_wino3p_nl4(p, u, std::min(device_cu_count(), kFwPartBlocks), fwp, &used, c.stream);
                if (rc == 0 && fwp) {
                    final_w_reduce_kernel<<<c0, 64, 0, c.stream>>>(fwp, used, c0, fv->gw + ic0);
                    ENDO_LAUNCH_CHECK();
                }
                break;
            }
        }
        if (rc) return rc;
    }
    {
        BnFin4 a;
        for (int j = 0; j < kLayers; ++j) {
            a.scratch[j] = c.scratch(k.bn[j]); a.saved[j] = c.saved(k.bn[j]); a.gamma[j] = c.params + k.bn[j].g;
            a.ggamma[j] = c.grads + k.bn[j].g; a.gbeta[j] = c.grads + k.bn[j].b;
        }
        ProfScope prof(kProfSmall, c.stream, 0.0, 0.0);
        bn_bwd_finalize4_kernel<<<dim3((c0 + 127) / 128, c.net->groups), 128, 0, c.stream>>>(a, kLayers, c.pq_p(level) + ic0, c.pq_q(level) + ic0, c0,
                                                                         static_cast<double>(c.net->n) * lv.h * lv.w, c.training, c.net->gs,
                                                                         c.net->slot_stride);
        ENDO_LAUNCH_CHECK();
    }
    return 0;
}

static int td_bwd(const Ctx& c, int level) {
    const BnP& b = table().td_bn[level];
    const ConvP& cv = table().td_conv[level];
    const int next = level + 1;
    const auto& lv = c.net->lv[level];
    int rc = prep_dy(c, next, next < kLevels ? 48 : 0, cv.cout, c.grads + cv.b);
    if (rc) return rc;
    {
        const WgradParams p = td_wgrad_params(c, level);
        Ctx cw;
        rc = c.fork_wgrad(cw, level);
        if (rc) return rc;
        ProfScope prof(kProfWgradOther, cw.stream, conv_flops(c.net, level, cv.cin, cv.cout, 1), 4.0 * c.nt() * lv.plane * cv.cin);
        rc = !c.bwd->td_wgrad_dma[level] ? launch_wgrad1x1(p, cw.stream) : c.bwd->bf16_wgrad ? launch_wgrad1x1_dma<1>(p, cw.stream) : launch_wgrad1x1_dma<0>(p, cw.stream);
        if (rc) return rc;
    }
    {
        const ConvParams p = td_dgrad_params(c, level);
        ProfScope prof(kProfDgradOther, c.stream, conv_flops(c.net, level, cv.cin, cv.cout, 1), 4.0 * c.nt() * lv.plane * 3.0 * cv.cin);
        switch (c.bwd->td_dgrad[level]) {
            case TdDgrad::Persistent: rc = launch_td_dgrad(p, device_cu_count(), c.stream); break;
            case TdDgrad::Runs128: rc = launch_td_dgrad_small(p, c.stream); break;
            case TdDgrad::Dma: rc = c.bwd->bf16_dgrad ? launch_conv_dma_auto<1, 16, 2, IN_UNPOOL, EPI_DGRAD_BN, 4, 2, 1, 1>(p, c.stream)
                                                      : launch_conv_dma_auto<1, 16, 2, IN_UNPOOL, EPI_DGRAD_BN, 4>(p, c.stream); break;
            case TdDgrad::Staged: rc = launch_conv_auto<1, 16, 3, IN_UNPOOL, EPI_DGRAD_BN, 4>(p, c.stream); break;
        }
        if (rc) return rc;
    }
    return bn_finalize(c, b, level, 48);
}

static int tu_bwd(const Ctx& c, int level, int src_level, int src_c0, const ConvP& cv) {
    const auto& lv = c.net->lv[level];
    int rc = prep_dy(c, level, 0, cv.cout, c.grads + cv.b);
    if (rc) return rc;
    {
        const TuWgrad form = c.bwd->tu_wgrad[level];
        const WgradParams p = tu_wgrad_params(c, level, form == TuWgrad::Subpix);
        Ctx cw;
        rc = c.fork_wgrad(cw, level);
        if (rc) return rc;
        ProfScope prof(kProfWgradOther, cw.stream, conv_flops(c.net, level, cv.cin, cv.cout, 3), 4.0 * c.nt() * lv.plane * (cv.cin / 4.0 + cv.cout));
        rc = form == TuWgrad::Subpix ? launch_tu_wgrad_subpix(p, c.gradws + c.net->wg_scratch_off, cw.stream)
           : form == TuWgrad::Taps ? launch_wgrad_taps<12, IN_UPSAMPLE>(p, cw.stream) : launch_wgrad<3, 1, IN_UPSAMPLE, DY_PLAIN>(p, cw.stream);
        if (rc) return rc;
    }
    ProfScope prof(kProfDgradOther, c.stream, conv_flops(c.net, level, cv.cin, cv.cout, 3), 4.0 * c.nt() * lv.plane * (cv.cout + cv.cin / 4.0));
    const TuDgrad form = c.bwd->tu_dgrad[level];
    if (form == TuDgrad::Plain) {
        ConvParams p{};
        fill_grid(c, p, level);
        fill_in(c, p, c.gbuf(level), level, 0, cv.cout);
        p.wgt = c.params + cv.w; p.w_cout = cv.cout; p.w_cin = cv.cin;
        fill_out(c, p, c.gbuf(src_level), src_level, src_c0, cv.cin);
        return launch_conv_dma_auto<3, 4, 3, IN_PLAIN, EPI_DGRAD_SUMPOOL, 4>(p, c.stream);
    }
    float* wd = c.gradws + c.net->tuw_scratch_off;
    tu_subpix_dgrad_weights_kernel<<<(16 * cv.cout * cv.cin + 255) / 256, 256, 0, c.stream>>>(c.params + cv.w, cv.cout, cv.cin, wd);
    ENDO_LAUNCH_CHECK();
    ConvParams p{};
    fill_grid(c, p, src_level);
    fill_in(c, p, c.gbuf(level), level, 0, 4 * cv.cout);
    p.sub_c = cv.cout;
    p.wgt = wd; p.w_cout = cv.cin; p.w_cin = 4 * cv.cout;
    fill_out(c, p, c.gbuf(src_level), src_level, src_c0, cv.cin);
    if (form == TuDgrad::Subpix32x8) return launch_conv_dma_vec<3, 8, 3, IN_SUBPIX, EPI_FWD, 2, 4, 2, 1, 1>(p, c.stream);
    if (form == TuDgrad::Subpix16x8) return launch_conv_dma_vec<3, 8, 3, IN_SUBPIX, EPI_FWD, 1, 2, 2, 1, 1>(p, c.stream);
    return launch_conv_dma_vec<3, 8, 3, IN_SUBPIX, EPI_FWD, 1, 1, 2, 1, 1>(p, c.stream);
}

static int64_t align_up(int64_t v, int64_t a) { return (v + a - 1) / a * a; }

}

extern "C" int endo_net_create_grouped(endo_net** out, int n, int h, int w, int groups) {
    if (!out || n <= 0 || h <= 0 || w <= 0 || groups <= 0) return ENDO_E_BADARG;
    if (groups > kMaxGroups) return ENDO_E_UNSUPPORTED;
    if ((h % 32) != 0 || (w % 32) != 0) return ENDO_E_UNSUPPORTED;
    const Table& tb = table();
    endo_net* net = new (std::nothrow) endo_net();
    if (!net) return ENDO_E_BADARG;
    net->n = n; net->h = h; net->w = w; net->groups = groups;
    net->wstream = nullptr; net->ev_fork = nullptr; net->ev_join = nullptr;
    default_options(net->opt);
    int64_t off = 0, sums = 0, pq = 0;
    for (int l = 0; l <= kLevels; ++l) {
        auto& lv = net->lv[l];
        lv.h = h >> l; lv.w = w >> l; lv.t = level_channels(l);
        lv.plane = static_cast<int64_t>(lv.h) * lv.w;
        lv.act = off; lv.grad = off;
        off += align_up(static_cast<int64_t>(n) * lv.t * lv.plane, 64);
        lv.sums = sums; sums += 2 * lv.t;
        lv.pq = pq; pq += lv.t;
    }
    const int64_t acts = off;
    net->pre_off = off; off += align_up(static_cast<int64_t>(n) * h * w, 64);
    net->saved_off = off; off += align_up(2 * tb.bn_width_total, 64);
    int64_t byte_off = off * 4;
    for (int l = 0; l < kLevels; ++l) {
        net->idx_off[l] = byte_off;
        byte_off += align_up(static_cast<int64_t>(n) * (down_in(l) + kNew) * net->lv[l + 1].plane, 256);
    }
    net->sums_off = byte_off;
    net->sums_bytes = sums * 8;
    byte_off += align_up(net->sums_bytes, 256);
    net->partial_off = byte_off / 4;
    byte_off += static_cast<int64_t>(kGrowth) * 163840 * 4;
    net->wino_off = byte_off / 4;
    byte_off += align_up(tb.wino_floats * 4, 256);
    net->wino4_off = byte_off / 4;
    byte_off += align_up(tb.wino4_floats * 4, 256);
    net->tape_floats = byte_off / 4;
    net->pq_off = acts;
    net->pq_floats = 2 * pq;
    net->scratch_off = align_up((acts + net->pq_floats) * 4, 256);
    net->slot_stride = align_up(tb.bn_width_total * 2, 32);
    net->scratch_bytes = net->slot_stride * 8 * kBnSlots;
    net->wg_scratch_off = (net->scratch_off + align_up(net->scratch_bytes, 256)) / 4;
    net->tuw_scratch_off = net->wg_scratch_off + std::max(std::max(kNsScratchFloats, kSpScratchFloats), 4 * kF34ScratchFloats);
    net->wd_off = align_up(net->tuw_scratch_off + 4 * kNew * (4 * kNew + 16), 64);
    net->gplane_off = align_up(net->wd_off + tb.wino_dgrad_floats, 64);
    net->bias_parts_off = net->gplane_off + align_up(static_cast<int64_t>(n) * h * w, 64);
    net->bias_parts_floats = static_cast<int64_t>(kBiasPartChannels) * n * groups * 32;
    {
        int launches = 1, channels = tb.first.cout;
        for (int l = 0; l < kLevels; ++l) {
            for (int j = 0; j < kLayers; ++j) { launches += 2; channels += tb.down_conv[l][j].cout + tb.up_conv[l][j].cout; }
            launches += 2; channels += tb.td_conv[l].cout + tb.tu_conv[l].cout;
        }
        for (int j = 0; j < kLayers; ++j) { ++launches; channels += tb.bott_conv[j].cout; }
        if (launches > kBiasPartLaunches || channels > kBiasPartChannels) { delete net; return ENDO_E_UNSUPPORTED; }
    }
    net->fw_parts_off = net->bias_parts_off + align_up(net->bias_parts_floats, 64);
    net->gradws_floats = net->fw_parts_off + 2 * static_cast<int64_t>(kFwPartBlocks) * 192;
    net->gs = align_up(net->tape_floats > net->gradws_floats ? net->tape_floats : net->gradws_floats, 64);
    *out = net;
    return 0;
}

extern "C" int endo_net_create(endo_net** out, int n, int h, int w) { return endo_net_create_grouped(out, n, h, w, 1); }

static bool option_id_ok(int id) { return id >= 0 && id < ENDO_OPT_COUNT && id != 6; }

extern "C" int endo_net_set_option(endo_net* net, int option_id, int value) {
    if (!net || !option_id_ok(option_id)) return ENDO_E_BADARG;
    const int old = net->opt[option_id];
    net->opt[option_id] = value;
    return old;
}

extern "C" int endo_net_get_option(const endo_net* net, int option_id) {
    if (!net || !option_id_ok(option_id)) return ENDO_E_BADARG;
    return net->opt[option_id];
}

extern "C" void endo_net_destroy(endo_net* net) {
    if (!net) return;
    if (net->ev_fork) (void)hipEventDestroy(net->ev_fork);
    if (net->ev_join) (void)hipEventDestroy(net->ev_join);
    if (net->wstream) (void)hipStreamDestroy(net->wstream);
    delete net;
}
extern "C" int64_t endo_net_param_floats(void) { return table().param_floats; }
extern "C" int64_t endo_net_bn_floats(void) { return table().bn_floats; }
extern "C" int64_t endo_net_tape_floats(const endo_net* net) { return !net ? 0 : (net->groups > 1 ? net->groups * net->gs : net->tape_floats); }
extern "C" int64_t endo_net_gradws_floats(const endo_net* net) { return !net ? 0 : (net->groups > 1 ? net->groups * net->gs : net->gradws_floats); }
extern "C" int endo_net_groups(const endo_net* net) { return net ? net->groups : 0; }
extern "C" int64_t endo_net_group_stride(const endo_net* net) { return net ? net->gs : 0; }
extern "C" int64_t endo_net_param_offset(int index) {
    const Table& tb = table();
    if (index < 0 || index >= static_cast<int>(tb.param_offsets.size())) return -1;
    return tb.param_offsets[index];
}
extern "C" int64_t endo_net_bn_offset(int bn_index, int which) {
    const Table& tb = table();
    if (bn_index < 0 || bn_index >= static_cast<int>(tb.bn_order.size()) || which < 0 || which > 1) return -1;
    return tb.bn_order[bn_index]->run + which * tb.bn_order[bn_index]->c;
}
extern "C" int endo_net_level_channels(int level) { return (level < 0 || level > kLevels) ? -1 : level_channels(level); }
extern "C" int64_t endo_net_act_offset(const endo_net* net, int level) { return (!net || level < 0 || level > kLevels) ? -1 : net->lv[level].act; }

extern "C" int64_t endo_net_tape_offset(const endo_net* net, int what, int index) {
    if (!net) return -1;
    const Table& tb = table();
    switch (what) {
        case ENDO_TAPE_PRE: return net->pre_off;
        case ENDO_TAPE_BN_SAVED:
            if (index < 0 || index >= static_cast<int>(tb.bn_order.size())) return -1;
            return net->saved_off + 2 * tb.bn_order[index]->saved;
        case ENDO_TAPE_POOL:
            if (index < 0 || index >= kLevels) return -1;
            return net->idx_off[index];
        default: return -1;
    }
}

extern "C" int endo_net_fwd(endo_net* net, const float* params, float* bn_running, const float* x, float* out, float* tape,
                            int training, void* stream_) {
    if (!net || !params || !bn_running || !x || !out || !tape) return ENDO_E_BADARG;
    const Table& tb = table();
    Ctx c{net, params, bn_running, tape, nullptr, nullptr, training, static_cast<hipStream_t>(stream_)};
    const FwdPlan plan = plan_fwd(c);
    c.fwd = &plan;
    for (int g = 0; g < net->groups; ++g)
        ENDO_CHECK(hipMemsetAsync(reinterpret_cast<char*>(tape + g * net->gs) + net->sums_off, 0, net->sums_bytes, c.stream));
    if (!plan.bf16) {
        ProfScope prof(kProfSmall, c.stream, 0.0, 4.0 * (tb.wino_floats + tb.wino_floats * 9 / 16));
        WinoWeightTable wt = tb.wino;
        for (int l = 0; l < wt.layers; ++l) wt.mode[l] = plan.dense[l].chunk_weights ? 1 : 0;
        wino_fwd_weights_kernel<<<(wt.start[wt.layers] + 255) / 256, 256, 0, c.stream>>>(wt, params, tape + net->wino_off);
        ENDO_LAUNCH_CHECK();
        if (plan.wino4_weights) wino4_fwd_weights_kernel<<<(tb.wino4.start[tb.wino4.layers] + 255) / 256, 256, 0, c.stream>>>(tb.wino4, params, tape + net->wino4_off);
        ENDO_LAUNCH_CHECK();
    }
    int rc;
    {
        ConvParams p{};
        fill_grid(c, p, 0);
        p.in = x; p.in_ns = 3 * net->lv[0].plane; p.in_cs = static_cast<int>(net->lv[0].plane); p.in_w = net->w; p.cin = 3;
        p.in_gs = net->n * p.in_ns;
        p.wgt = params + tb.first.w; p.bias = params + tb.first.b; p.w_cout = kFirst; p.w_cin = 3;
        fill_out(c, p, c.act(0), 0, 48, kFirst);
        p.out_sums = c.out_sums(0, 48);
        ProfScope prof(kProfConvFirst, c.stream, conv_flops(net, 0, 3, kFirst, 3), 4.0 * c.nt() * net->lv[0].plane * (3 + kFirst));
        rc = launch_conv_dma_auto<3, 4, 3, IN_PLAIN, EPI_FWD>(p, c.stream);
        if (rc) return rc;
    }
    for (int b = 0; b < kBlocks; ++b) {
        if (b > kLevels) {
            const int i = b - kLevels - 1, l = kLevels - 1 - i;
            rc = tu_fwd(c, l, l + 1, (i == 0) ? 288 : 96 + down_in(l + 1), tb.tu_conv[i]);
            if (rc) return rc;
        }
        for (int j = 0; j < kLayers; ++j) {
            rc = dense_fwd(c, b, j);
            if (rc) return rc;
        }
        if (b < kLevels) {
            rc = td_fwd(c, b);
            if (rc) return rc;
        }
    }
    {
        const auto& lv = net->lv[0];
        const int c_first = plan.fuse_final ? 96 + down_in(0) + kGrowth * (kLayers - 1) : 0;
        ProfScope prof(kProfConvFinal, c.stream, 2.0 * c.nt() * lv.plane * 192, 4.0 * c.nt() * lv.plane * (194 - c_first));
        int bx = static_cast<int>((lv.plane / 4 + 255) / 256);
        bx = bx < 1 ? 1 : bx;
        final_fwd_kernel<<<dim3(bx, c.nt()), 256, 0, c.stream>>>(c.act(0), lv.t * lv.plane, static_cast<int>(lv.plane), 192,
                                                                 params + tb.final_.w, params + tb.final_.b, tape + net->pre_off, out,
                                                                 net->n, net->gs, c_first);
        ENDO_LAUNCH_CHECK();
    }
    return 0;
}

extern "C" int endo_net_bwd(endo_net* net, const float* params, const float* x, const float* tape, const float* grad_out,
                            float* grads, float* gradws, int training, void* stream_) {
    if (!net || !params || !x || !tape || !grad_out || !grads || !gradws) return ENDO_E_BADARG;
    const Table& tb = table();
    Ctx c{net, params, nullptr, const_cast<float*>(tape), grads, gradws, training, static_cast<hipStream_t>(stream_)};
    c.x = x;
    const BwdPlan plan = plan_bwd(c);
    c.bwd = &plan;
    BiasParts bias_parts{};
    c.bias_parts = &bias_parts;
    if (!net->wstream) {
        ENDO_CHECK(hipStreamCreateWithFlags(&net->wstream, hipStreamNonBlocking));
        ENDO_CHECK(hipEventCreateWithFlags(&net->ev_fork, hipEventDisableTiming));
        ENDO_CHECK(hipEventCreateWithFlags(&net->ev_join, hipEventDisableTiming));
    }
    for (int g = 0; g < net->groups; ++g)
        ENDO_CHECK(hipMemsetAsync(gradws + g * net->gs + net->pq_off, 0,
                                  static_cast<size_t>(net->scratch_off + net->scratch_bytes - net->pq_off * 4), c.stream));
    if (plan.dgrad_weights) {
        ProfScope prof(kProfSmall, c.stream, 0.0, 4.0 * 2.0 * tb.wino_dgrad_floats);
        int layout1_blocks = 0;
        for (int b = 0; b < kBlocks; ++b) layout1_blocks |= plan.block[b].wino3_layout ? 1 << b : 0;
        dgrad_wino_weights_kernel<<<(tb.wino_dgrad.start[tb.wino_dgrad.layers] + 255) / 256, 256, 0, c.stream>>>(tb.wino_dgrad, params, gradws + net->wd_off, layout1_blocks);
        ENDO_LAUNCH_CHECK();
    }
    int rc;
    const FinalVirt virt{gradws + net->gplane_off, params + tb.final_.w, grads + tb.final_.w};
    {
        const auto& lv = net->lv[0];
        const int materialise = plan.materialise;
        {
            Ctx cw;
            rc = c.fork_wgrad(cw, 0);
            if (rc) return rc;
            const int c_first = plan.c_first;
            int by = static_cast<int>((lv.plane + 256 * 16 - 1) / (256 * 16));
            by = by < 1 ? 1 : (by > 16 ? 16 : by);
            ProfScope prof(kProfConvFinal, cw.stream, 2.0 * c.nt() * lv.plane * (192 - c_first), 4.0 * c.nt() * lv.plane * (192 - c_first + 2));
            final_bwd_weight_kernel<<<dim3(192 - c_first + 1, by, c.nt()), 256, 0, cw.stream>>>(grad_out, tape + net->pre_off, c.act(0), lv.t * lv.plane,
                                                                         static_cast<int>(lv.plane), 192, net->n, net->gs, grads + tb.final_.w,
                                                                         grads + tb.final_.b, c_first);
            ENDO_LAUNCH_CHECK();
        }
        ProfScope prof(kProfConvFinal, c.stream, 2.0 * c.nt() * lv.plane * 192, 4.0 * c.nt() * lv.plane * (materialise + 2));
        if (plan.use_virt) {
            int bx = static_cast<int>((lv.plane + 1023) / 1024);
            final_g_kernel<<<dim3(bx, c.nt()), 256, 0, c.stream>>>(grad_out, tape + net->pre_off, gradws + net->gplane_off, static_cast<int>(lv.plane), net->n, net->gs);
            ENDO_LAUNCH_CHECK();
        }
        if (materialise > 0) {
            int bx = static_cast<int>((lv.plane + 255) / 256);
            final_bwd_data_kernel<<<dim3(bx, c.nt()), 256, 0, c.stream>>>(grad_out, tape + net->pre_off, params + tb.final_.w, c.gbuf(0),
                                                                          lv.t * lv.plane, static_cast<int>(lv.plane), materialise, net->n, net->gs, 0);
            ENDO_LAUNCH_CHECK();
        }
    }
    for (int b = kBlocks - 1; b >= 0; --b) {
        if (b < kLevels) {
            rc = td_bwd(c, b);
            if (rc) return rc;
        }
        rc = dense_block_bwd(c, b, (b == kBlocks - 1 && plan.use_virt) ? &virt : nullptr);
        if (rc) return rc;
        if (b > kLevels) {
            const int i = b - kLevels - 1, l = kLevels - 1 - i;
            rc = tu_bwd(c, l, l + 1, (i == 0) ? 288 : 96 + down_in(l + 1), tb.tu_conv[i]);
            if (rc) return rc;
        }
    }
    {
        WgradParams p = first_wgrad_params(c);
        const auto& lv = net->lv[0];
        if (plan.first == FirstWgrad::F34Prep) {
            p.prep_x = c.act(0) + 48 * lv.plane;
            p.prep_p = c.pq_p(0) + 48; p.prep_q = c.pq_q(0) + 48;
            p.prep_bias = grads + tb.first.b;
        } else {
            rc = prep_dy(c, 0, 48, kFirst, grads + tb.first.b);
            if (rc) return rc;
        }
        Ctx cw;
        rc = c.fork_wgrad(cw, 0);
        if (rc) return rc;
        ProfScope prof(kProfWgradOther, cw.stream, conv_flops(net, 0, 3, kFirst, 3), 4.0 * c.nt() * lv.plane * (3 + kFirst));
        switch (plan.first) {
            case FirstWgrad::F34Prep: rc = launch_wgrad_f34<0, true, true>(p, gradws + net->wg_scratch_off, cw.stream); break;
            case FirstWgrad::F34: rc = launch_wgrad_f34<0, true>(p, gradws + net->wg_scratch_off, cw.stream); break;
            case FirstWgrad::Taps: rc = launch_wgrad_taps<12, IN_PLAIN>(p, cw.stream); break;
            case FirstWgrad::Direct: rc = launch_wgrad<3, 3, IN_PLAIN, DY_PLAIN>(p, cw.stream); break;
        }
        if (rc) return rc;
    }
    if (bias_parts.table.n > 0) {
        ProfScope prof(kProfSmall, c.stream, 0.0, 4.0 * bias_parts.used);
        bias_reduce_kernel<<<dim3(bias_parts.table.n, 8), 256, 0, c.stream>>>(bias_parts.table);
        ENDO_LAUNCH_CHECK();
    }
    if (net->wstream) {
        ENDO_CHECK(hipEventRecord(net->ev_join, net->wstream));
        ENDO_CHECK(hipStreamWaitEvent(c.stream, net->ev_join, 0));
    }
    return 0;
}
```

endoscopydepthestimation-pytorch_amd/csrc/wgrad_f34_kernels.h:

```cpp
#pragma once

#include <algorithm>

#include "conv_dma_kernels.h"
#include "wgrad_kernels.h"

namespace endo {

typedef float f32x2 __attribute__((ext_vector_type(2)));

constexpr int kF34XsPair = 264;
constexpr int kF34Xs = 8 * kF34XsPair;
constexpr int kF34WavesPerXcd = 256;

struct F34Plan {
    int groups;
    int wpg;
    int segq;
    int spb;
    int slots;
};
__host__ __device__ inline int f34_first_block(const F34Plan& plan, int g) { return (g * plan.wpg) >> 2; }
__host__ __device__ inline int f34_block_count(const F34Plan& plan, int g) { return (((g + 1) * plan.wpg - 1) >> 2) - ((g * plan.wpg) >> 2) + 1; }
__host__ __device__ inline bool f34_row_written(const F34Plan& plan, int g, int slot) { return slot % plan.spb < f34_block_count(plan, g); }

template <typename T>
__device__ __forceinline__ T f34_fma(const float a, const T b, const T c) {
    if constexpr (sizeof(T) == 8) return __builtin_elementwise_fma(T{a, a}, b, c);
    else return fmaf(a, b, c);
}
template <typename T>
__device__ __forceinline__ void f34_bt(const T d0, const T d1, const T d2, const T d3, const T d4, const T d5, T (&t)[6]) {
    t[0] = f34_fma<T>(4.f, d0, f34_fma<T>(-5.f, d2, d4));
    const T pp = f34_fma<T>(-4.f, d2, d4), qq = f34_fma<T>(-4.f, d1, d3);
    t[1] = pp + qq;
    t[2] = pp - qq;
    const T rr = d4 - d2, ss = d3 - d1;
    t[3] = f34_fma<T>(2.f, ss, rr);
    t[4] = f34_fma<T>(-2.f, ss, rr);
    t[5] = f34_fma<T>(4.f, d1, f34_fma<T>(-5.f, d3, d5));
}

template <typename T>
__device__ __forceinline__ void f34_s(const T g0, const T g1, const T g2, const T g3, T (&u)[6]) {
    const T e = g0 + g2, o = g1 + g3;
    const T e4 = f34_fma<T>(4.f, g2, g0), o4 = f34_fma<T>(4.f, g3, g1);
    u[0] = g0;
    u[1] = e + o;
    u[2] = e - o;
    u[3] = f34_fma<T>(2.f, o4, e4);
    u[4] = f34_fma<T>(-2.f, o4, e4);
    u[5] = g3;
}

__device__ __forceinline__ void f34_pin(f32x2& v) { asm("" : "+v"(v)); }

__device__ __forceinline__ __amdgpu_buffer_rsrc_t f34_rsrc(const void* base, int bytes) {
    return __builtin_amdgcn_make_buffer_rsrc(const_cast<void*>(base), 0, bytes, 0x00020000);
}
__device__ __forceinline__ f32x4 f34_ld4(__amdgpu_buffer_rsrc_t r, unsigned voff, unsigned soff) {
    typedef unsigned u32x4 __attribute__((ext_vector_type(4)));
    return __builtin_bit_cast(f32x4, __builtin_amdgcn_raw_buffer_load_b128(r, voff, soff, 0));
}
__device__ __forceinline__ float f34_ld1(__amdgpu_buffer_rsrc_t r, unsigned voff, unsigned soff) {
    return __builtin_bit_cast(float, __builtin_amdgcn_raw_buffer_load_b32(r, voff, soff, 0));
}

template <int EXP = 0, bool RAW = false, bool PREP = false>
__global__ void __launch_bounds__(kConvThreads, 2) wgrad_f34_kernel(const WgradParams p, float* __restrict__ partial, const F34Plan plan) {
    extern __shared__ __attribute__((aligned(16))) float smem[];
    const int tid = threadIdx.x;
    const int lane = tid & 63;
    const int wave = __builtin_amdgcn_readfirstlane(tid >> 6);
    const int li = lane & 15;
    const int lk = lane >> 4;

    const int xcd = blockIdx.x & 7;
    const int bi = blockIdx.x >> 3;
    const int wi = bi * 4 + wave;
    const bool active = wi < plan.groups * plan.wpg;
    const int group = active ? wi / plan.wpg : 0;
    const int wq = wi - group * plan.wpg;

    const int S = (p.w + 15) >> 4, CY = p.h >> 4, segq = plan.segq, YS = CY / segq;
    const int units = p.n * YS * S;
    const int per_xcd = (units + 7) >> 3;
    const int u_end = min(units, (xcd + 1) * per_xcd);
    const int u_first = active ? xcd * per_xcd + wq : u_end;

    f32x4 acc[36];
#pragma unroll
    for (int m = 0; m < 36; ++m) acc[m] = f32x4{0.f, 0.f, 0.f, 0.f};

    const int ch = RAW ? li : 16 * group + li;
    const bool ch_ok = ch < p.cin;
    const unsigned bo = 4u * static_cast<unsigned>(min(ch, p.cin - 1) * p.in_cs + 4 * lk);
    float* const xs = smem + wave * 2 * kF34Xs;
    const unsigned x_vo = 4u * static_cast<unsigned>((lane >> 5) * p.in_cs + ((lane >> 3) & 3) * p.in_w + 4 * (lane & 7));
    const float* const xs_r = xs + (li >> 1) * kF34XsPair + (li & 1) * 128 + 4 * lk;
    const unsigned x_grp = RAW ? 0u : 4u * static_cast<unsigned>(16 * group * p.in_cs);
    const unsigned g_vo_in = li < 12 ? 4u * static_cast<unsigned>(li * p.dy_cs + 4 * lk) : 0x80000000u;

    float sc = 0.f, sh = 0.f;
    int cst_grp = -1;
    float prep_pc = 0.f, prep_qc = 0.f, prep_sum = 0.f;
    float keep[2][6];

    auto act_row = [&](const float hl, const f32x4 m, const float hr, const f32x2 sc_e, const f32x2 sh_e, float (&o)[6]) {
        const f32x2 e = __builtin_elementwise_fma(f32x2{hl, hr}, sc_e, sh_e);
        const f32x2 a = __builtin_elementwise_fma(f32x2{m[0], m[1]}, f32x2{sc, sc}, f32x2{sh, sh});
        const f32x2 b = __builtin_elementwise_fma(f32x2{m[2], m[3]}, f32x2{sc, sc}, f32x2{sh, sh});
        if constexpr (RAW) {
            o[0] = sc_e[0] != 0.f ? e[0] : 0.f; o[1] = sc_e[1] != 0.f ? e[1] : 0.f;
            o[2] = a[0]; o[3] = a[1]; o[4] = b[0]; o[5] = b[1];
        } else {
            o[0] = fmaxf(e[0], 0.f); o[1] = fmaxf(e[1], 0.f);
            o[2] = fmaxf(a[0], 0.f); o[3] = fmaxf(a[1], 0.f);
            o[4] = fmaxf(b[0], 0.f); o[5] = fmaxf(b[1], 0.f);
        }
    };
    auto x_issue = [&](const __amdgpu_buffer_rsrc_t r, int s, int row, int img) {
        const unsigned so = x_grp + 4u * static_cast<unsigned>(row * p.in_w + 16 * s - (s > 0 ? 8 : 0));
        const int unit = lane & 7;
        float* dst = xs + img * kF34Xs;
        if (s > 0 ? (unit >= 1 && unit <= 6) : unit <= 4) {
#pragma unroll
            for (int i = 0; i < 8; ++i)
                if (!(EXP & 2))
                    __builtin_amdgcn_raw_ptr_buffer_load_lds(r, (lptr_t)(dst + i * kF34XsPair), 16, x_vo, so + 8u * static_cast<unsigned>(i * p.in_cs), 0, 0);
        }
    };

    for (int u = u_first; u < u_end; u += plan.wpg) {
        const int s = u % S;
        const int rest = u / S;
        const int yseg = rest % YS;
        const int n = rest / YS;
        const WgSample sm(p, n);
        const __amdgpu_buffer_rsrc_t xr = f34_rsrc(p.in + sm.in_off(p), p.cin * p.in_cs * 4);
        const __amdgpu_buffer_rsrc_t gr = f34_rsrc(p.dy + sm.dy_off(p) + (RAW ? static_cast<int64_t>(12 * group) * p.dy_cs : 0), 12 * p.dy_cs * 4);
        const __amdgpu_buffer_rsrc_t pr = f34_rsrc((PREP ? p.prep_x : p.dy) + sm.dy_off(p) + (RAW ? static_cast<int64_t>(12 * group) * p.dy_cs : 0), 12 * p.dy_cs * 4);
        if (PREP && sm.grp != cst_grp) {
            prep_pc = li < 12 ? p.prep_p[sm.grp * p.gs + 12 * group + li] : 0.f;
            prep_qc = li < 12 ? p.prep_q[sm.grp * p.gs + 12 * group + li] : 0.f;
        }
        if (sm.grp != cst_grp) {
            sc = 0.f; sh = 0.f;
            if constexpr (RAW) {
                if (ch_ok) sc = 1.f;
            } else if (ch_ok) {
                const float* saved = p.saved + sm.grp * p.gs;
                sc = p.gamma[ch] * saved[2 * ch + 1];
                sh = fmaf(-saved[2 * ch], sc, p.beta[ch]);
            }
            cst_grp = sm.grp;
        }
        const unsigned g_vo = 16 * s + 4 * lk < p.w ? g_vo_in : 0x80000000u;
        const bool l_out = s == 0 && lk == 0, r_out = 16 * s + 4 * lk + 4 >= p.w;
        const f32x2 sc_e = {l_out ? 0.f : sc, r_out ? 0.f : sc}, sh_e = {l_out ? 0.f : sh, r_out ? 0.f : sh};
        const int rd_shift = s > 0 ? 8 : 0;
        const int row_begin = 16 * yseg * segq, row_end = row_begin + 16 * segq;

        x_issue(xr, s, row_begin + 1, 0);
        if (row_begin + 4 < row_end) x_issue(xr, s, row_begin + 5, 1);
#pragma unroll
        for (int i = 0; i < 2; ++i) {
            const int row = row_begin - 1 + i;
            if (row >= 0) {
                const unsigned off = bo + 4u * static_cast<unsigned>(row * p.in_w + 16 * s);
                const f32x4 m = f34_ld4(xr, off, 0);
                const float a = f34_ld1(xr, off - (l_out ? 0u : 4u), 0), b = f34_ld1(xr, off + (r_out ? 0u : 16u), 0);
                act_row(a, m, b, sc_e, sh_e, keep[i]);
            } else {
#pragma unroll
                for (int e = 0; e < 6; ++e) keep[i][e] = 0.f;
            }
        }

#pragma unroll 1
        for (int row = row_begin; row < row_end; row += 4) {
            f32x4 gt[4], xa[4];
            {
                const unsigned so = 4u * static_cast<unsigned>(row * p.dy_w + 16 * s);
                const unsigned pitch = 4u * static_cast<unsigned>(p.dy_w);
#pragma unroll
                for (int i = 0; i < 4; ++i) gt[i] = f34_ld4(gr, g_vo, so + i * pitch);
                if constexpr (PREP) {
#pragma unroll
                    for (int i = 0; i < 4; ++i) xa[i] = f34_ld4(pr, g_vo, so + i * pitch);
                }
            }
            const int img = ((row - row_begin) >> 2) & 1;
            if (row + 4 < row_end) asm volatile("s_waitcnt vmcnt(%0)" ::"n"(PREP ? 16 : 12) : "memory");
            else asm volatile("s_waitcnt vmcnt(%0)" ::"n"(PREP ? 8 : 4) : "memory");
            __builtin_amdgcn_sched_barrier(0);
            float d[6][6];
#pragma unroll
            for (int e = 0; e < 6; ++e) { d[0][e] = keep[0][e]; d[1][e] = keep[1][e]; }
            {
                const float* rp = xs_r + img * kF34Xs + rd_shift;
                f32x4 m[4];
                float hl[4], hr[4];
#pragma unroll
                for (int i = 0; i < 4; ++i) {
                    m[i] = *reinterpret_cast<const f32x4*>(rp + 32 * i);
                    hl[i] = rp[32 * i - 1];
                    hr[i] = rp[32 * i + 4];
                }
                asm volatile("s_waitcnt lgkmcnt(0)" ::: "memory");
                __builtin_amdgcn_sched_barrier(0);
                if (row + 8 < row_end) x_issue(xr, s, row + 9, img);
                __builtin_amdgcn_sched_barrier(0);
#pragma unroll
                for (int i = 0; i < 4; ++i) act_row(hl[i], m[i], hr[i], sc_e, sh_e, d[2 + i]);
            }
            if (row + 4 >= p.h) {
#pragma unroll
                for (int e = 0; e < 6; ++e) d[5][e] = 0.f;
            }
#pragma unroll
            for (int e = 0; e < 6; ++e) { keep[0][e] = d[4][e]; keep[1][e] = d[5][e]; }

            if constexpr (PREP) {
                const float pc = g_vo != 0x80000000u ? prep_pc : 0.f, qc = g_vo != 0x80000000u ? prep_qc : 0.f;
#pragma unroll
                for (int i = 0; i < 4; ++i)
#pragma unroll
                    for (int k = 0; k < 4; ++k) { gt[i][k] += fmaf(pc, xa[i][k], qc); prep_sum += gt[i][k]; }
            }
            f32x2 va[6], vb[6];
            f34_s(f32x2{gt[0][0], gt[0][1]}, f32x2{gt[1][0], gt[1][1]}, f32x2{gt[2][0], gt[2][1]}, f32x2{gt[3][0], gt[3][1]}, va);
            f34_s(f32x2{gt[0][2], gt[0][3]}, f32x2{gt[1][2], gt[1][3]}, f32x2{gt[2][2], gt[2][3]}, f32x2{gt[3][2], gt[3][3]}, vb);
            f32x2 t05[6], t12[6], t34[6];
            f34_bt(f32x2{d[0][0], d[0][1]}, f32x2{d[1][0], d[1][1]}, f32x2{d[2][0], d[2][1]}, f32x2{d[3][0], d[3][1]}, f32x2{d[4][0], d[4][1]},
                   f32x2{d[5][0], d[5][1]}, t05);
            f34_bt(f32x2{d[0][2], d[0][3]}, f32x2{d[1][2], d[1][3]}, f32x2{d[2][2], d[2][3]}, f32x2{d[3][2], d[3][3]}, f32x2{d[4][2], d[4][3]},
                   f32x2{d[5][2], d[5][3]}, t12);
            f34_bt(f32x2{d[0][4], d[0][5]}, f32x2{d[1][4], d[1][5]}, f32x2{d[2][4], d[2][5]}, f32x2{d[3][4], d[3][5]}, f32x2{d[4][4], d[4][5]},
                   f32x2{d[5][4], d[5][5]}, t34);
#pragma unroll
            for (int i = 0; i < 6; ++i) { f34_pin(va[i]); f34_pin(vb[i]); f34_pin(t05[i]); f34_pin(t12[i]); f34_pin(t34[i]); }
#pragma unroll
            for (int i = 0; i < 6; ++i) {
                f32x2 eo = va[i] + vb[i], eo4 = f34_fma<f32x2>(4.f, vb[i], va[i]);
                f34_pin(eo); f34_pin(eo4);
                const float u0 = va[i][0], u1 = eo[0] + eo[1], u2 = eo[0] - eo[1];
                const float u3 = fmaf(2.f, eo4[1], eo4[0]), u4 = fmaf(-2.f, eo4[1], eo4[0]), u5 = vb[i][1];
                const f32x2 p05 = t05[i], p12 = t12[i], p34 = t34[i];
                const float x0 = fmaf(4.f, p05[0], fmaf(-5.f, p12[1], p34[1]));
                const float x5 = fmaf(4.f, p12[0], fmaf(-5.f, p34[0], p05[1]));
                f32x2 qp = f34_fma<f32x2>(-4.f, p12, p34);
                f32x2 sr = p34 - p12;
                f34_pin(qp); f34_pin(sr);
                const float x1 = qp[1] + qp[0], x2 = qp[1] - qp[0];
                const float x3 = fmaf(2.f, sr[0], sr[1]), x4 = fmaf(-2.f, sr[0], sr[1]);
                acc[6 * i + 0] = __builtin_amdgcn_mfma_f32_16x16x4f32(u0, x0, acc[6 * i + 0], 0, 0, 0);
                acc[6 * i + 1] = __builtin_amdgcn_mfma_f32_16x16x4f32(u1, x1, acc[6 * i + 1], 0, 0, 0);
                acc[6 * i + 2] = __builtin_amdgcn_mfma_f32_16x16x4f32(u2, x2, acc[6 * i + 2], 0, 0, 0);
                acc[6 * i + 3] = __builtin_amdgcn_mfma_f32_16x16x4f32(u3, x3, acc[6 * i + 3], 0, 0, 0);
                acc[6 * i + 4] = __builtin_amdgcn_mfma_f32_16x16x4f32(u4, x4, acc[6 * i + 4], 0, 0, 0);
                acc[6 * i + 5] = __builtin_amdgcn_mfma_f32_16x16x4f32(u5, x5, acc[6 * i + 5], 0, 0, 0);
            }
        }
    }

    if constexpr (PREP) {
        if (p.prep_bias) {
            float v = prep_sum;
            v += __shfl_xor(v, 16, 64);
            v += __shfl_xor(v, 32, 64);
            if (active && lk == 0 && li < 12) atomicAdd(p.prep_bias + 12 * group + li, v);
        }
    }
    const float C[3][6] = {{0.25f, -1.f / 6.f, -1.f / 6.f, 1.f / 24.f, 1.f / 24.f, 0.f},
                           {0.f, -1.f / 6.f, 1.f / 6.f, 1.f / 12.f, -1.f / 12.f, 0.f},
                           {0.f, -1.f / 6.f, -1.f / 6.f, 1.f / 6.f, 1.f / 6.f, 1.f}};
    f32x4 h[3][6];
#pragma unroll
    for (int j = 0; j < 6; ++j) {
        const f32x4 m1 = acc[6 + j], m2 = acc[12 + j], m3 = acc[18 + j], m4 = acc[24 + j];
        const f32x4 s12 = m1 + m2, d12 = m2 - m1, s34 = m3 + m4, d34 = m3 - m4;
        h[0][j] = 0.25f * acc[j] - (1.f / 6.f) * s12 + (1.f / 24.f) * s34;
        h[1][j] = (1.f / 6.f) * d12 + (1.f / 12.f) * d34;
        h[2][j] = -(1.f / 6.f) * s12 + (1.f / 6.f) * s34 + acc[30 + j];
    }
    __syncthreads();
    float* const red = smem + wave * (9 * 256);
#pragma unroll
    for (int a = 0; a < 3; ++a)
#pragma unroll
        for (int b = 0; b < 3; ++b) {
            f32x4 o = {0.f, 0.f, 0.f, 0.f};
#pragma unroll
            for (int j = 0; j < 6; ++j)
                if (C[b][j] != 0.f) o += C[b][j] * h[a][j];
#pragma unroll
            for (int r = 0; r < 4; ++r) red[(3 * a + b) * 256 + r * 64 + lane] = o[r];
        }
    __syncthreads();
    const int total = plan.groups * plan.wpg;
    int gw[5];
    int64_t row[4];
#pragma unroll
    for (int w = 0; w < 4; ++w) {
        gw[w] = bi * 4 + w < total ? (bi * 4 + w) / plan.wpg : -1;
        row[w] = ((static_cast<int64_t>(max(gw[w], 0)) * 9) * plan.slots + xcd * plan.spb + (bi - f34_first_block(plan, max(gw[w], 0)))) * 256 + tid;
    }
    gw[4] = -1;
#pragma unroll
    for (int t = 0; t < 9; ++t) {
        float sum = 0.f;
#pragma unroll
        for (int w = 0; w < 4; ++w) {
            if (gw[w] < 0) continue;
            sum += smem[w * (9 * 256) + t * 256 + tid];
            if (gw[w + 1] != gw[w]) {
                partial[row[w] + static_cast<int64_t>(t) * plan.slots * 256] = sum;
                sum = 0.f;
            }
        }
    }
}

__global__ void __launch_bounds__(256) wgrad_f34_reduce_kernel(const float* __restrict__ partial, const F34Plan plan, int cin, float* __restrict__ dw, int raw) {
    __shared__ f32x4 s_part[4][64];
    const int gm = blockIdx.x;
    const int group = gm / 9, tap = gm - group * 9;
    const int slots = plan.slots;
    const int per = (slots + gridDim.y - 1) / gridDim.y;
    const int b0 = blockIdx.y * per, b1 = min(slots, b0 + per);
    if (b0 >= b1) return;
    const int q = threadIdx.x & 63, sub = threadIdx.x >> 6;
    const f32x4* src = reinterpret_cast<const f32x4*>(partial + (static_cast<int64_t>(gm) * slots) * 256) + q;
    f32x4 s0 = {0.f, 0.f, 0.f, 0.f};
    for (int b = b0 + sub; b < b1; b += 4)
        if (f34_row_written(plan, group, b)) s0 += src[static_cast<int64_t>(b) * 64];
    s_part[sub][q] = s0;
    __syncthreads();
    const int e = threadIdx.x;
    const float* sp = reinterpret_cast<const float*>(s_part);
    const float total = (sp[e] + sp[256 + e]) + (sp[512 + e] + sp[768 + e]);
    const int lane = e & 63, r = e >> 6;
    const int co = 4 * (lane >> 4) + r;
    const int ci = (raw ? 0 : 16 * group) + (lane & 15);
    if (co < 12 && ci < cin) atomicAdd(dw + (static_cast<int64_t>(co + (raw ? 12 * group : 0)) * cin + ci) * 9 + tap, total);
}

struct F34ReduceBatch {
    const float* partial[4];
    float* dw[4];
    F34Plan plan[4];
    int cin[4];
    int count;
};
__global__ void __launch_bounds__(256) wgrad_f34_reduce_batch_kernel(const F34ReduceBatch a) {
    __shared__ f32x4 s_part[4][64];
    const int l = blockIdx.z;
    const int gm = blockIdx.x;
    const F34Plan plan = a.plan[l];
    if (gm >= plan.groups * 9) return;
    const int slots = plan.slots, cin = a.cin[l];
    const int group = gm / 9, tap = gm - group * 9;
    const int per = (slots + gridDim.y - 1) / gridDim.y;
    const int b0 = blockIdx.y * per, b1 = min(slots, b0 + per);
    if (b0 >= b1) return;
    const int q = threadIdx.x & 63, sub = threadIdx.x >> 6;
    const f32x4* src = reinterpret_cast<const f32x4*>(a.partial[l] + (static_cast<int64_t>(gm) * slots) * 256) + q;
    f32x4 s0 = {0.f, 0.f, 0.f, 0.f};
    for (int b = b0 + sub; b < b1; b += 4)
        if (f34_row_written(plan, group, b)) s0 += src[static_cast<int64_t>(b) * 64];
    s_part[sub][q] = s0;
    __syncthreads();
    const int e = threadIdx.x;
    const float* sp = reinterpret_cast<const float*>(s_part);
    const float total = (sp[e] + sp[256 + e]) + (sp[512 + e] + sp[768 + e]);
    const int lane = e & 63, r = e >> 6;
    const int co = 4 * (lane >> 4) + r;
    const int ci = 16 * group + (lane & 15);
    if (co < 12 && ci < cin) atomicAdd(a.dw[l] + (static_cast<int64_t>(co) * cin + ci) * 9 + tap, total);
}

constexpr int kF34Blocks = 512;
constexpr int kF34MinTiles = 256;
constexpr int64_t kF34ScratchFloats = static_cast<int64_t>(9) * 8 * kF34WavesPerXcd * 256;

inline bool wgrad_f34_ok(const WgradParams& p, long min_tiles = kF34MinTiles) {
    const bool aligned = (p.w % 4 == 0) && (p.h % 16 == 0) && (p.dy_w % 4 == 0) && (p.dy_cs % 4 == 0) && (p.dy_ns % 4 == 0) && (p.in_w % 4 == 0) &&
                         (p.in_cs % 4 == 0) && (p.in_ns % 4 == 0) && (reinterpret_cast<uintptr_t>(p.dy) % 16 == 0) &&
                         (reinterpret_cast<uintptr_t>(p.in) % 16 == 0);
    const long quads = static_cast<long>((p.w + 15) / 16) * (p.h / 16) * p.n;
    const bool small = static_cast<int64_t>(p.in_cs) * (p.cin + 16) * 4 < (1ll << 31) && static_cast<int64_t>(p.dy_cs) * 12 * 4 < (1ll << 31);
    return aligned && small && p.cout == 12 && p.cin >= 16 && (p.cin + 15) / 16 <= kF34WavesPerXcd && quads * 16 >= min_tiles;
}
inline bool wgrad_f34_raw_ok(const WgradParams& p, long min_tiles = kF34MinTiles) {
    WgradParams q = p;
    q.cout = 12; q.cin = 16;
    return p.cin <= 16 && p.cout % 12 == 0 && p.cout / 12 <= 16 && static_cast<int64_t>(p.in_cs) * 32 * 4 < (1ll << 31) && wgrad_f34_ok(q, min_tiles);
}

inline F34Plan wgrad_f34_plan(const WgradParams& p, int waves_per_xcd = kF34WavesPerXcd, bool raw = false) {
    F34Plan plan{};
    plan.groups = raw ? p.cout / 12 : (p.cin + 15) / 16;
    const int CY = p.h / 16, S = (p.w + 15) / 16;
    float best = 1e30f;
    for (int segq = 4; segq >= 1; segq >>= 1) {
        if (CY % segq) continue;
        const int per_xcd = (p.n * (CY / segq) * S + 7) / 8;
        const int wpg = std::min(waves_per_xcd / plan.groups, per_xcd);
        const int iters = (per_xcd + wpg - 1) / wpg;
        const float cost = iters * (4.f * segq + 1.5f);
        if (cost < best * 0.97f) { best = cost; plan.segq = segq; plan.wpg = wpg; }
    }
    plan.spb = 1;
    for (int g = 0; g < plan.groups; ++g) plan.spb = std::max(plan.spb, f34_block_count(plan, g));
    plan.slots = 8 * plan.spb;
    return plan;
}

template <int EXP = 0, bool RAW = false, bool PREP = false>
inline int launch_wgrad_f34(const WgradParams& p, float* scratch, hipStream_t stream, F34ReduceBatch* batch = nullptr) {
    static_assert(!PREP || RAW, "the fused gradient preparation belongs to the first convolution's form");
    const F34Plan plan = wgrad_f34_plan(p, kF34Blocks / 2, RAW);
    constexpr int lds = 4 * 2 * kF34Xs * 4;
    ENDO_CHECK(launch_dyn(wgrad_f34_kernel<EXP, RAW, PREP>, kF34Blocks, kConvThreads, lds, stream, p, scratch, plan));
    if (batch && !RAW && batch->count < 4) {
        const int k = batch->count++;
        batch->partial[k] = scratch; batch->dw[k] = p.dw; batch->plan[k] = plan; batch->cin[k] = p.cin;
        return 0;
    }
    wgrad_f34_reduce_kernel<<<dim3(plan.groups * 9, 2), 256, 0, stream>>>(scratch, plan, p.cin, p.dw, RAW ? 1 : 0);
    ENDO_LAUNCH_CHECK();
    return 0;
}

inline int launch_wgrad_f34_reduce_batch(F34ReduceBatch& batch, hipStream_t stream) {
    if (batch.count == 0) return 0;
    int gmax = 0;
    for (int k = 0; k < batch.count; ++k) gmax = std::max(gmax, batch.plan[k].groups);
    wgrad_f34_reduce_batch_kernel<<<dim3(gmax * 9, 1, batch.count), 256, 0, stream>>>(batch);
    ENDO_LAUNCH_CHECK();
    batch.count = 0;
    return 0;
}

}
```

endoscopydepthestimation-pytorch_amd/csrc/wgrad_kernels.h:

```cpp
#pragma once

#include "conv_kernels.h"

namespace endo {

constexpr int kWgTileX = 32;
constexpr int kWgTileY = 8;
constexpr int kWgKC = 16;

enum DyMode { DY_PLAIN = 0, DY_UNPOOL = 1 };

struct WgradParams {
    int n, h, w;
    int tiles_x, tiles_y;
    const float* in;
    int64_t in_ns;
    int in_cs, in_w;
    int cin;
    const float* saved;
    const float* gamma;
    const float* beta;
    const float* dy;
    int64_t dy_ns;
    int dy_cs, dy_w;
    const uint8_t* dy_idx;
    int64_t idx_ns;
    int cout;
    float* dw;
    int group_n;
    int64_t gs, in_gs;
    const float* prep_x;
    const float* prep_p;
    const float* prep_q;
    float* prep_bias;
};

constexpr int kMaxGroups = 4;

struct WgSample {
    int grp, nl;
    __device__ __forceinline__ WgSample(const WgradParams& p, int s) {
        grp = p.group_n > 0 ? s / p.group_n : 0;
        nl = s - grp * p.group_n;
    }
    __device__ __forceinline__ int64_t in_off(const WgradParams& p) const { return grp * p.in_gs + nl * p.in_ns; }
    __device__ __forceinline__ int64_t dy_off(const WgradParams& p) const { return grp * p.gs + nl * p.dy_ns; }
    __device__ __forceinline__ int64_t idx_off(const WgradParams& p) const { return 4 * grp * p.gs + nl * p.idx_ns; }
};
__device__ __forceinline__ int wg_groups(const WgradParams& p) { return p.group_n > 0 ? p.n / p.group_n : 1; }

template <int KS>
struct WgradGeom {
    static constexpr int kHalo = KS / 2;
    static constexpr int kRows = kWgTileY + 2 * kHalo;
    static constexpr int kCols = kWgTileX + 2 * kHalo;
    static constexpr int kPlane = kRows * kCols;
    static constexpr int kCS = ((kPlane - 2 + 31) / 32) * 32 + 2;
    static constexpr int kDyPlane = kWgTileX * kWgTileY;
    static constexpr int kDS = kDyPlane + 2;
    static constexpr int kPos = (kPlane + kConvThreads - 1) / kConvThreads;
    static constexpr int kPre = kWgKC * kPos;
};

template <int KS, int Q, int IN, int DY>
__global__ void __launch_bounds__(kConvThreads) wgrad_mfma_kernel(const WgradParams p) {
    using G = WgradGeom<KS>;
    constexpr int KK = KS * KS;
    constexpr int NB = 16 * Q;
    constexpr int kDyElems = NB * G::kDyPlane;
    constexpr int kDyPre = kDyElems / kConvThreads;
    constexpr int RW = kWgTileY / 4;

    extern __shared__ __attribute__((aligned(16))) float smem[];
    float* s_in = smem;
    float* s_dy = s_in + kWgKC * G::kCS;
    __shared__ float s_cst[kMaxGroups * 4 * kWgKC];

    const int tid = threadIdx.x;
    const int lane = tid & 63;
    const int wave = tid >> 6;
    const int li = lane & 15;
    const int lk = lane >> 4;
    const int ci_base = blockIdx.x * kWgKC;
    const int co_base = blockIdx.z * NB;
    const int tiles_per_sample = p.tiles_x * p.tiles_y;
    const int tiles_total = tiles_per_sample * p.n;

    if constexpr (IN == IN_BNRELU) {
        if (tid < kWgKC * wg_groups(p)) {
            const int g = tid / kWgKC, t = tid - g * kWgKC;
            const int c = ci_base + t;
            float scale = 0.f, mean = 0.f, beta = 0.f;
            if (c < p.cin) {
                const float* saved = p.saved + g * p.gs;
                mean = saved[2 * c];
                scale = p.gamma[c] * saved[2 * c + 1];
                beta = p.beta[c];
            }
            s_cst[g * 4 * kWgKC + t] = scale;
            s_cst[g * 4 * kWgKC + kWgKC + t] = mean;
            s_cst[g * 4 * kWgKC + 2 * kWgKC + t] = beta;
        }
    }

    f32x4 acc[KK][Q];
#pragma unroll
    for (int t = 0; t < KK; ++t)
#pragma unroll
        for (int q = 0; q < Q; ++q) acc[t][q] = f32x4{0.f, 0.f, 0.f, 0.f};

    float pre[G::kPre];
    float dpre[kDyPre];
    unsigned pos_ok = 0;

    int in_ry[G::kPos], in_rx[G::kPos];
#pragma unroll
    for (int k = 0; k < G::kPos; ++k) {
        const int e = tid + k * kConvThreads;
        in_ry[k] = e / G::kCols;
        in_rx[k] = e - in_ry[k] * G::kCols;
    }
    const int dy_ry = tid / kWgTileX, dy_rx = tid % kWgTileX;
    static_assert(kWgTileX * kWgTileY == kConvThreads, "one dY pixel per thread");
    static_assert(kDyPre == NB, "dY staging is one value per thread per output channel");

    int pre_grp = 0;
    auto load_tile = [&](int tile) {
        const int n = tile / tiles_per_sample;
        const int trem = tile - n * tiles_per_sample;
        const int x0 = (trem % p.tiles_x) * kWgTileX;
        const int y0 = (trem / p.tiles_x) * kWgTileY;
        const WgSample sm(p, n);
        pre_grp = sm.grp;
        const float* in_n = p.in + sm.in_off(p);
        pos_ok = 0;
        int goff[G::kPos];
#pragma unroll
        for (int k = 0; k < G::kPos; ++k) {
            const int gy = y0 - G::kHalo + in_ry[k];
            const int gx = x0 - G::kHalo + in_rx[k];
            goff[k] = 0;
            if (tid + k * kConvThreads < G::kPlane && gy >= 0 && gy < p.h && gx >= 0 && gx < p.w) {
                pos_ok |= (1u << k);
                if constexpr (IN == IN_UPSAMPLE) goff[k] = (gy >> 1) * p.in_w + (gx >> 1);
                else goff[k] = gy * p.in_w + gx;
            }
        }
#pragma unroll
        for (int c = 0; c < kWgKC; ++c) {
            const int ch = ci_base + c;
            const int64_t coff = static_cast<int64_t>(ch) * p.in_cs;
#pragma unroll
            for (int k = 0; k < G::kPos; ++k)
                pre[c * G::kPos + k] = (ch < p.cin && (pos_ok & (1u << k))) ? in_n[coff + goff[k]] : 0.f;
        }
        const int gy = y0 + dy_ry, gx = x0 + dy_rx;
        const bool ok = gy < p.h && gx < p.w;
        const float* dy_n = p.dy + sm.dy_off(p);
#pragma unroll
        for (int j = 0; j < NB; ++j) {
            const int co = co_base + j;
            float v = 0.f;
            if (ok && co < p.cout) {
                if constexpr (DY == DY_UNPOOL) {
                    const int64_t o = static_cast<int64_t>(co) * p.dy_cs + (gy >> 1) * p.dy_w + (gx >> 1);
                    const int code = ((gy & 1) << 1) | (gx & 1);
                    v = (p.dy_idx[sm.idx_off(p) + o] == code) ? dy_n[o] : 0.f;
                } else {
                    v = dy_n[static_cast<int64_t>(co) * p.dy_cs + gy * p.dy_w + gx];
                }
            }
            dpre[j] = v;
        }
    };

    auto store_tile = [&]() {
        const float* cst = s_cst + pre_grp * 4 * kWgKC;
#pragma unroll
        for (int c = 0; c < kWgKC; ++c) {
#pragma unroll
            for (int k = 0; k < G::kPos; ++k) {
                const int e = tid + k * kConvThreads;
                if (e < G::kPlane) {
                    float v = pre[c * G::kPos + k];
                    if constexpr (IN == IN_BNRELU) {
                        if (ci_base + c < p.cin && (pos_ok & (1u << k))) {
// ... 235 lines not shown
```

endoscopydepthestimation-pytorch_amd/csrc/wino4_fwd_kernels.h:

```cpp
#pragma once

#include "conv_dma_kernels.h"
#include "wgrad_f34_kernels.h"
#include "wino_fwd_kernels.h"

namespace endo {

constexpr float kW4A = 0.625f, kW4B = 1.5f;
constexpr float kW4A2 = kW4A * kW4A, kW4B2 = kW4B * kW4B;
constexpr float kW4A3 = kW4A2 * kW4A, kW4B3 = kW4B2 * kW4B;
constexpr float kW4P = kW4A2 * kW4B2, kW4S = kW4A2 + kW4B2;
constexpr float kW4N0 = 1.f / kW4P;
constexpr float kW4NA = 1.f / (2.f * kW4A2 * (kW4A2 - kW4B2));
constexpr float kW4NB = 1.f / (2.f * kW4B2 * (kW4B2 - kW4A2));

constexpr int kW4UStride = 576;

__global__ void __launch_bounds__(256) wino4_fwd_weights_kernel(const WinoWeightTable t, const float* __restrict__ params, float* __restrict__ u) {
    const int total = t.start[t.layers];
    for (int item = blockIdx.x * blockDim.x + threadIdx.x; item < total; item += gridDim.x * blockDim.x) {
        int l = 0;
        while (item >= t.start[l + 1]) ++l;
        const int e = item - t.start[l];
        const int ci = e >> 4, j = e & 15;
        float g[3][3];
#pragma unroll
        for (int a = 0; a < 3; ++a)
#pragma unroll
            for (int b = 0; b < 3; ++b) g[a][b] = 0.f;
        if (j < t.cout[l]) {
            const float* src = params + t.w_off[l] + (static_cast<int64_t>(j) * t.cin[l] + ci) * 9;
#pragma unroll
            for (int a = 0; a < 3; ++a)
#pragma unroll
                for (int b = 0; b < 3; ++b) g[a][b] = src[a * 3 + b];
        }
        auto gt = [](float a, float b, float c, float (&o)[6]) {
            const float ea = fmaf(kW4A2, c, a), eb = fmaf(kW4B2, c, a);
            o[0] = kW4N0 * a;
            o[1] = kW4NA * fmaf(kW4A, b, ea);
            o[2] = kW4NA * fmaf(-kW4A, b, ea);
            o[3] = kW4NB * fmaf(kW4B, b, eb);
            o[4] = kW4NB * fmaf(-kW4B, b, eb);
            o[5] = c;
        };
        float h[6][3];
#pragma unroll
        for (int b = 0; b < 3; ++b) {
            float o[6];
            gt(g[0][b], g[1][b], g[2][b], o);
#pragma unroll
            for (int i = 0; i < 6; ++i) h[i][b] = o[i];
        }
        float* dst = u + t.u_off[l] + static_cast<int64_t>(ci) * kW4UStride + j * 12;
#pragma unroll
        for (int i = 0; i < 6; ++i) {
            float o[6];
            gt(h[i][0], h[i][1], h[i][2], o);
#pragma unroll
            for (int jj = 0; jj < 6; ++jj) dst[(i >> 1) * 192 + (i & 1) * 6 + jj] = o[jj];
        }
    }
}

struct Wino4Geom {
    static constexpr int kTileX = 64, kTileY = 16;
    static constexpr int kCols = kTileX + 8;
    static constexpr int kRows = kTileY + 2;
    static constexpr int kPlane = kRows * kCols;
    static constexpr int kKC = 4;
    static constexpr int kXUnits = kKC * kPlane / 4;
    static constexpr int kUUnits = kKC * kW4UStride / 4;
    static constexpr int kXRounds = (kXUnits + kConvThreads - 1) / kConvThreads;
    static constexpr int kURounds = (kUUnits + kConvThreads - 1) / kConvThreads;
    static constexpr int kBuf = kKC * kPlane + kKC * kW4UStride;
    static constexpr int kTail = 4 * 16 * 2;
    static size_t bytes(int bn_cap) { return sizeof(float) * (2 * kBuf + 4 * bn_cap + kTail); }
};

__device__ __forceinline__ void w4_at(const float m0, const float m1, const float m2, const float m3, const float m4, const float m5, float (&y)[4]) {
    const float s1 = m1 + m2, d1 = m1 - m2, s2 = m3 + m4, d2 = m3 - m4;
    y[0] = m0 + s1 + s2;
    y[1] = fmaf(kW4B, d2, kW4A * d1);
    y[2] = fmaf(kW4B2, s2, kW4A2 * s1);
    y[3] = fmaf(kW4B3, d2, fmaf(kW4A3, d1, m5));
}

template <typename T>
__device__ __forceinline__ void w4_bt(const T d0, const T d1, const T d2, const T d3, const T d4, const T d5, T (&t)[6]) {
    t[0] = f34_fma<T>(kW4P, d0, f34_fma<T>(-kW4S, d2, d4));
    const T pp = f34_fma<T>(-kW4B2, d2, d4), qh = f34_fma<T>(-kW4B2, d1, d3);
    t[1] = f34_fma<T>(kW4A, qh, pp);
    t[2] = f34_fma<T>(-kW4A, qh, pp);
    const T rr = f34_fma<T>(-kW4A2, d2, d4), sh = f34_fma<T>(-kW4A2, d1, d3);
    t[3] = f34_fma<T>(kW4B, sh, rr);
    t[4] = f34_fma<T>(-kW4B, sh, rr);
    t[5] = f34_fma<T>(kW4P, d1, f34_fma<T>(-kW4S, d3, d5));
}

template <bool FIN = false>
__global__ void __launch_bounds__(kConvThreads, 2) wino4_fwd_kernel(const ConvParams p0) {
    using G = Wino4Geom;
    extern __shared__ __attribute__((aligned(16))) float smem[];
    float* s_aux = smem + 2 * G::kBuf;
    int grp, n;
    group_of(p0, blockIdx.z, grp, n);
    const ConvParams p = group_view(p0, grp);
    const int groups = p0.group_n > 0 ? gridDim.z / p0.group_n : 1;
    const bool first_of_group = blockIdx.x == 0 && n == 0;
    const int cap = p.bn_cap;

    const int tid = threadIdx.x;
    const int lane = tid & 63;
    const int wave = __builtin_amdgcn_readfirstlane(tid >> 6);
    const int li = lane & 15;
    const int lk = lane >> 4;
    const int tile = (gridDim.x & 7) == 0 ? xcd_remap(blockIdx.x, gridDim.x) : blockIdx.x;
    const int x0 = (tile % p.tiles_x) * G::kTileX;
    const int y0 = (tile / p.tiles_x) * G::kTileY;

    for (int c = tid; c < p.cin; c += kConvThreads) {
        float scale, mean, beta;
        bn_input_constants(p, p0, grp, groups, first_of_group, c, scale, mean, beta);
        s_aux[c] = scale;
        s_aux[cap + c] = mean;
        s_aux[2 * cap + c] = beta;
        if constexpr (FIN) s_aux[3 * cap + G::kTail + c] = p.fin_w[c];
    }
    f32x4 fin[4];
#pragma unroll
    for (int r = 0; r < 4; ++r) fin[r] = f32x4{0.f, 0.f, 0.f, 0.f};

    f32x4 acc[36];
#pragma unroll
    for (int xi = 0; xi < 36; ++xi) acc[xi] = f32x4{0.f, 0.f, 0.f, 0.f};

    const __amdgpu_buffer_rsrc_t xr = f34_rsrc(p.in + n * p.in_ns, p.cin * p.in_cs * 4);
    const __amdgpu_buffer_rsrc_t ur = f34_rsrc(p.wgt, p.cin * kW4UStride * 4);
    unsigned x_vo[G::kXRounds];
#pragma unroll
    for (int k = 0; k < G::kXRounds; ++k) {
        const int e = tid + k * kConvThreads;
        x_vo[k] = 0x80000000u;
        if (e < G::kXUnits) {
            const int c = e / (G::kPlane / 4), u = e - c * (G::kPlane / 4);
            const int ry = u / (G::kCols / 4);
            const int rx = (u - ry * (G::kCols / 4)) * 4;
            const int gy = y0 - 1 + ry;
            const int gx = x0 - 4 + rx;
            if (gy >= 0 && gy < p.h && gx >= 0 && gx < p.w) x_vo[k] = 4u * static_cast<unsigned>(c * p.in_cs + gy * p.in_w + gx);
        }
    }
    const unsigned u_vo = 16u * static_cast<unsigned>(tid);
    const int nchunks = p.cin / G::kKC;

    auto issue_dma = [&](int chunk, int buf) {
        float* s_stage = smem + buf * G::kBuf + wave * 256;
        const unsigned xs = 4u * static_cast<unsigned>(chunk * G::kKC * p.in_cs);
        const unsigned us = 4u * static_cast<unsigned>(chunk * G::kKC * kW4UStride);
#pragma unroll
        for (int k = 0; k < G::kXRounds; ++k) {
            const int e0 = k * kConvThreads + wave * 64;
            if (e0 < G::kXUnits) {
                if (e0 + 64 <= G::kXUnits || e0 + lane < G::kXUnits)
                    __builtin_amdgcn_raw_ptr_buffer_load_lds(xr, (lptr_t)(s_stage + k * 4 * kConvThreads), 16, x_vo[k], xs, 0, 0);
            }
        }
        float* s_u = s_stage + G::kKC * G::kPlane;
#pragma unroll
        for (int k = 0; k < G::kURounds; ++k) {
            const int e0 = k * kConvThreads + wave * 64;
            if (e0 < G::kUUnits)
                __builtin_amdgcn_raw_ptr_buffer_load_lds(ur, (lptr_t)(s_u + k * 4 * kConvThreads), 16, u_vo + 16u * static_cast<unsigned>(k * kConvThreads), us, 0, 0);
        }
    };

    const bool l_out = x0 + 4 * li == 0, r_out = x0 + 4 * li + 4 >= p.w;
    const int py = y0 + 4 * wave - 1;
    const bool top_out = py < 0, bottom_out = py + 5 >= p.h;

    auto compute = [&](int chunk, int buf) {
        const float* s_in = smem + buf * G::kBuf;
        const float* s_u = s_in + G::kKC * G::kPlane;
        const int ch = chunk * G::kKC + lk;
        const float sc = s_aux[ch], mn = s_aux[cap + ch], bt = s_aux[2 * cap + ch];
        const float sh = fmaf(-mn, sc, bt);
        const f32x2 sc_m = {sc, sc}, sh_m = {sh, sh};
        const f32x2 sc_e = {l_out ? 0.f : sc, r_out ? 0.f : sc}, sh_e = {l_out ? 0.f : sh, r_out ? 0.f : sh};
        const float* a_base = s_in + lk * G::kPlane + (4 * wave) * G::kCols + 4 * li + 4;
        float wfin = 0.f;
        if constexpr (FIN) wfin = s_aux[3 * cap + G::kTail + ch];
        float d[6][6];
#pragma unroll
        for (int r = 0; r < 6; ++r) {
            const f32x4 m = *reinterpret_cast<const f32x4*>(a_base + r * G::kCols);
            if constexpr (FIN) {
                if (r >= 1 && r <= 4) {
#pragma unroll
                    for (int k = 0; k < 4; ++k) fin[r - 1][k] = fmaf(wfin, m[k], fin[r - 1][k]);
                }
            }
            const float hl = a_base[r * G::kCols - 1], hr = a_base[r * G::kCols + 4];
            const f32x2 e = __builtin_elementwise_fma(f32x2{hl, hr}, sc_e, sh_e);
            const f32x2 a = __builtin_elementwise_fma(f32x2{m[0], m[1]}, sc_m, sh_m);
            const f32x2 b = __builtin_elementwise_fma(f32x2{m[2], m[3]}, sc_m, sh_m);
            d[r][0] = fmaxf(e[0], 0.f); d[r][1] = fmaxf(e[1], 0.f);
            d[r][2] = fmaxf(a[0], 0.f); d[r][3] = fmaxf(a[1], 0.f);
            d[r][4] = fmaxf(b[0], 0.f); d[r][5] = fmaxf(b[1], 0.f);
        }
        if (top_out) {
#pragma unroll
            for (int e = 0; e < 6; ++e) d[0][e] = 0.f;
        }
        if (bottom_out) {
#pragma unroll
// ... 128 lines not shown
```

endoscopydepthestimation-pytorch_amd/csrc/wino_fwd_kernels.h:

```cpp
#pragma once

#include "conv_dma_kernels.h"

namespace endo {

constexpr int kWinoUStride = 16 * 16 + 16;
constexpr int kWinoMaxLayers = 48;

struct WinoWeightTable {
    int layers;
    int start[kWinoMaxLayers + 1];
    int cin[kWinoMaxLayers];
    int cout[kWinoMaxLayers];
    int64_t w_off[kWinoMaxLayers];
    int64_t u_off[kWinoMaxLayers];
    int mode[kWinoMaxLayers];
};
constexpr int kDenseChunkFloats = 9 * 16 * 16;

__global__ void __launch_bounds__(256) wino_fwd_weights_kernel(const WinoWeightTable t, const float* __restrict__ params, float* __restrict__ u) {
    const int total = t.start[t.layers];
    for (int item = blockIdx.x * blockDim.x + threadIdx.x; item < total; item += gridDim.x * blockDim.x) {
        int l = 0;
        while (item >= t.start[l + 1]) ++l;
        const int e = item - t.start[l];
        const int ci = e >> 4, j = e & 15;
        float g[3][3];
#pragma unroll
        for (int a = 0; a < 3; ++a)
#pragma unroll
            for (int b = 0; b < 3; ++b) g[a][b] = 0.f;
        if (j < t.cout[l]) {
            const float* src = params + t.w_off[l] + (static_cast<int64_t>(j) * t.cin[l] + ci) * 9;
#pragma unroll
            for (int a = 0; a < 3; ++a)
#pragma unroll
                for (int b = 0; b < 3; ++b) g[a][b] = src[a * 3 + b];
        }
        if (t.mode[l] == 1) {
            float* dst = u + t.u_off[l] + static_cast<int64_t>(ci >> 4) * kDenseChunkFloats + (ci & 15) * 16 + j;
#pragma unroll
            for (int tap = 0; tap < 9; ++tap) dst[tap * 256] = g[tap / 3][tap % 3];
            if (ci == t.cin[l] - 1)
                for (int cz = (ci & 15) + 1; cz < 16; ++cz)
#pragma unroll
                    for (int tap = 0; tap < 9; ++tap) dst[tap * 256 + (cz - (ci & 15)) * 16] = 0.f;
            continue;
        }
        float h[4][3];
#pragma unroll
        for (int b = 0; b < 3; ++b) {
            h[0][b] = g[0][b];
            h[1][b] = 0.5f * (g[0][b] + g[1][b] + g[2][b]);
            h[2][b] = 0.5f * (g[0][b] - g[1][b] + g[2][b]);
            h[3][b] = g[2][b];
        }
        float* dst = u + t.u_off[l] + static_cast<int64_t>(ci) * kWinoUStride + j;
#pragma unroll
        for (int a = 0; a < 4; ++a) {
            dst[(4 * a + 0) * 16] = h[a][0];
            dst[(4 * a + 1) * 16] = 0.5f * (h[a][0] + h[a][1] + h[a][2]);
            dst[(4 * a + 2) * 16] = 0.5f * (h[a][0] - h[a][1] + h[a][2]);
            dst[(4 * a + 3) * 16] = h[a][2];
        }
        if (j == 0) {
#pragma unroll
            for (int k = 0; k < 16; ++k) dst[256 + k] = 0.f;
        }
    }
}

constexpr int kWinoFwdStages = 2;

template <int R, int KC>
struct WinoFwdGeom {
    static constexpr int kTileX = 32;
    static constexpr int kTileY = 8 * R;
    static constexpr int kLeft = 4;
    static constexpr int kCols = kTileX + 2 * kLeft;
    static constexpr int kRows = kTileY + 2;
    static constexpr int kPlane = kRows * kCols;
    static constexpr int kCS = ((kPlane - 32 + 63) / 64) * 64 + 32;
    static constexpr int kUnits = kCS / 4;
    static constexpr int kPos = (kUnits + kConvThreads - 1) / kConvThreads;
    static constexpr int kUUnits = KC * kWinoUStride / 4;
    static constexpr int kUPos = (kUUnits + kConvThreads - 1) / kConvThreads;
    static constexpr int kFlat = KC * kUnits + kUUnits;
    static constexpr int kDma = (kFlat + kConvThreads - 1) / kConvThreads;
    static constexpr int kDmaMin = (kFlat - (kDma - 1) * kConvThreads > 3 * 64) ? kDma : kDma - 1;
    static_assert(kCS == 4 * kUnits, "a stage is one contiguous array of DMA units");
    static constexpr int kBuf = KC * kCS + KC * kWinoUStride;
    static constexpr int kTail = 4 * 16 * 2;
    static size_t bytes(int bn_cap) { return sizeof(float) * (kWinoFwdStages * kBuf + 3 * bn_cap + kTail); }
};

template <int R, int KC, int MINW, int EXP = 0>
__global__ void __launch_bounds__(kConvThreads, MINW) wino_fwd_kernel(const ConvParams p0) {
    using G = WinoFwdGeom<R, KC>;
    constexpr int NS = kWinoFwdStages;
    typedef float f32x2 __attribute__((ext_vector_type(2)));
    extern __shared__ __attribute__((aligned(16))) float smem[];
    float* s_aux = smem + NS * G::kBuf;
    int grp, n;
    group_of(p0, blockIdx.z, grp, n);
    const ConvParams p = group_view(p0, grp);
    const int groups = p0.group_n > 0 ? gridDim.z / p0.group_n : 1;
    const bool first_of_group = blockIdx.x == 0 && n == 0;
    const int cap = p.bn_cap;

    const int tid = threadIdx.x;
    const int lane = tid & 63;
    const int wave = __builtin_amdgcn_readfirstlane(tid >> 6);
    const int li = lane & 15;
    const int lk = lane >> 4;
    const int tile = (gridDim.x & 7) == 0 ? xcd_remap(blockIdx.x, gridDim.x) : blockIdx.x;
    const int x0 = (tile % p.tiles_x) * G::kTileX;
    const int y0 = (tile / p.tiles_x) * G::kTileY;

    for (int c = tid; c < p.cin; c += kConvThreads) {
        float scale, mean, beta;
        bn_input_constants(p, p0, grp, groups, first_of_group, c, scale, mean, beta);
        s_aux[c] = scale;
        s_aux[cap + c] = mean;
        s_aux[2 * cap + c] = beta;
    }
    for (int c = p.cin + tid; c < ((p.cin + KC - 1) / KC) * KC; c += kConvThreads) {
        s_aux[c] = 0.f; s_aux[cap + c] = 0.f; s_aux[2 * cap + c] = 0.f;
    }

    f32x4 acc[R][16];
#pragma unroll
    for (int r = 0; r < R; ++r)
#pragma unroll
        for (int xi = 0; xi < 16; ++xi) acc[r][xi] = f32x4{0.f, 0.f, 0.f, 0.f};

    const float* d_ptr[G::kDma];
    unsigned d_stride[G::kDma];
    {
        const float* in_n = p.in + n * p.in_ns;
#pragma unroll
        for (int k = 0; k < G::kDma; ++k) {
            const int e = tid + k * kConvThreads;
            d_ptr[k] = g_pad_consts;
            d_stride[k] = 0;
            if (e < KC * G::kUnits) {
                const int c = e / G::kUnits, u = e - c * G::kUnits;
                const int ry = u / (G::kCols / 4);
                const int rx = (u - ry * (G::kCols / 4)) * 4;
                const int gy = y0 - 1 + ry;
                const int gx = x0 - G::kLeft + rx;
                if (ry < G::kRows && gy >= 0 && gy < p.h && gx >= 0 && gx < p.w) {
                    d_ptr[k] = in_n + static_cast<int64_t>(c) * p.in_cs + gy * p.in_w + gx;
                    d_stride[k] = static_cast<unsigned>(KC) * static_cast<unsigned>(p.in_cs) * 4u;
                }
            } else if (e < G::kFlat) {
                d_ptr[k] = p.wgt + 4 * (e - KC * G::kUnits);
                d_stride[k] = KC * kWinoUStride * 4u;
            }
        }
    }
    const int nchunks = p.cin / KC;

    auto issue_dma = [&](int buf) {
        float* s_stage = smem + buf * G::kBuf + wave * 256;
#pragma unroll
        for (int k = 0; k < G::kDma; ++k) {
            if (k + 1 < G::kDma) {
                __builtin_amdgcn_global_load_lds((gptr_t)d_ptr[k], (lptr_t)(s_stage + k * 4 * kConvThreads), 16, 0, 0);
            } else {
                const int e0 = k * kConvThreads + wave * 64;
                if (e0 < G::kFlat && e0 + lane < G::kFlat)
                    __builtin_amdgcn_global_load_lds((gptr_t)d_ptr[k], (lptr_t)(s_stage + k * 4 * kConvThreads), 16, 0, 0);
            }
            d_ptr[k] = reinterpret_cast<const float*>(reinterpret_cast<const char*>(d_ptr[k]) + d_stride[k]);
        }
    };

    auto compute = [&](int chunk, int buf) {
        const float* s_in = smem + buf * G::kBuf;
        const float* s_u = s_in + KC * G::kCS;
#pragma unroll
        for (int quad = 0; quad < KC / 4; ++quad) {
            const int ch = chunk * KC + quad * 4 + lk;
            const float sc = s_aux[ch], mn = s_aux[cap + ch], bt = s_aux[2 * cap + ch];
            const f32x2 mn2 = {mn, mn}, sc2 = {sc, sc}, bt2 = {bt, bt};
            const float* b_base = s_u + (quad * 4 + lk) * kWinoUStride + li;
            float b[16];
#pragma unroll
            for (int xi = 0; xi < 16; ++xi) b[xi] = (EXP & 16) ? static_cast<float>(xi + lane) : b_base[xi * 16];
            const float* a_base = s_in + (quad * 4 + lk) * G::kCS + (2 * wave * R) * G::kCols + 2 * li + 2;
            f32x2 mid[2 * R + 2], end[2 * R + 2];
#pragma unroll
            for (int row = 0; row < 2 * R + 2; ++row) {
                f32x2 m, e;
                if constexpr ((EXP & 8) != 0) {
                    m = f32x2{sc + row, mn + row}; e = f32x2{bt + row, sc - row};
                } else {
                    const f32x2 left = *reinterpret_cast<const f32x2*>(a_base + row * G::kCols);
                    const f32x2 right = *reinterpret_cast<const f32x2*>(a_base + row * G::kCols + 4);
                    m = *reinterpret_cast<const f32x2*>(a_base + row * G::kCols + 2);
                    e = f32x2{left[1], right[0]};
                }
                if constexpr ((EXP & 2) == 0) {
                    m = __builtin_elementwise_fma(m - mn2, sc2, bt2);
                    e = __builtin_elementwise_fma(e - mn2, sc2, bt2);
                    mid[row] = f32x2{__builtin_fmaxf(m[0], 0.f), __builtin_fmaxf(m[1], 0.f)};
                    end[row] = f32x2{__builtin_fmaxf(e[0], 0.f), __builtin_fmaxf(e[1], 0.f)};
                } else {
                    mid[row] = m; end[row] = e;
                }
            }
#pragma unroll
            for (int r = 0; r < R; ++r) {
                f32x2 tm[4], te[4];
                if constexpr ((EXP & 4) == 0) {
                    tm[0] = mid[2 * r] - mid[2 * r + 2];     te[0] = end[2 * r] - end[2 * r + 2];
                    tm[1] = mid[2 * r + 1] + mid[2 * r + 2]; te[1] = end[2 * r + 1] + end[2 * r + 2];
                    tm[2] = mid[2 * r + 2] - mid[2 * r + 1]; te[2] = end[2 * r + 2] - end[2 * r + 1];
                    tm[3] = mid[2 * r + 1] - mid[2 * r + 3]; te[3] = end[2 * r + 1] - end[2 * r + 3];
                } else {
#pragma unroll
                    for (int a = 0; a < 4; ++a) { tm[a] = mid[2 * r + a]; te[a] = end[2 * r + a]; }
// ... 116 lines not shown
```

Baseline: 511.7.

## Fold BN backward finalize into consumers and merge weight-prep launches

Removes the separate BN backward finalize kernels and the pq buffer. Each consumer (prep_dy and the fused first-layer wgrad) now computes the per-channel p/q terms directly from the BN scratch sums, across up to nine BN consumers. Forward and backward weight transforms (Winograd, transposed-conv phase weights) and buffer zeroing are merged into single prepare kernels, and the final-layer weight reduce is folded into bias_reduce_kernel. The aim is fewer small kernel launches and fewer syncs, at the cost of redundant per-block recomputation of the BN terms and more complex kernels.

```diff
diff --git a/endoscopydepthestimation-pytorch_amd/csrc/common.h b/endoscopydepthestimation-pytorch_amd/csrc/common.h
--- a/endoscopydepthestimation-pytorch_amd/csrc/common.h
+++ b/endoscopydepthestimation-pytorch_amd/csrc/common.h
@@ -45,6 +45,42 @@
 #pragma unroll
     for (int k = 0; k < kBnSlots; ++k) t += s[k * slot_stride];
     return t;
+}
+
+constexpr int kBnMaxConsumers = 9;
+struct BnConsumers {
+    int n;
+    unsigned group_end;
+    int training;
+    double count;
+    int64_t slot_stride;
+    struct Entry {
+        const double* scratch;
+        const float* saved;
+        const float* gamma;
+        float* ggamma;
+        float* gbeta;
+    } e[kBnMaxConsumers];
+};
+
+__device__ __forceinline__ void bn_consumer_term(const BnConsumers& cs, int e, int c, int64_t go, double& s1, double& s2, float& pe, float& qe) {
+    const BnConsumers::Entry en = cs.e[e];
+    float mean = 0.f, rstd = 0.f, gamma = 0.f;
+    if (cs.training) { mean = en.saved[go + 2 * c]; rstd = en.saved[go + 2 * c + 1]; gamma = en.gamma[c]; }
+    s1 = bn_slot_sum(en.scratch + go / 2 + 2 * c, cs.slot_stride);
+    s2 = bn_slot_sum(en.scratch + go / 2 + 2 * c + 1, cs.slot_stride);
+    pe = 0.f; qe = 0.f;
+    if (cs.training) {
+        const double scale = gamma * static_cast<double>(rstd);
+        const double k = scale * rstd * s2 / cs.count;
+        pe = static_cast<float>(-k);
+        qe = static_cast<float>(-scale * s1 / cs.count + k * mean);
+    }
+}
+
+__device__ __forceinline__ void bn_consumer_fold_step(const BnConsumers& cs, int e, float term, float& v, double& run) {
+    run += static_cast<double>(term);
+    if ((cs.group_end >> e) & 1u) { v += static_cast<float>(run); run = 0.0; }
 }
 
 typedef short bf16x4_bits __attribute__((ext_vector_type(4)));
diff --git a/endoscopydepthestimation-pytorch_amd/csrc/dgrad_wino_kernels.h b/endoscopydepthestimation-pytorch_amd/csrc/dgrad_wino_kernels.h
--- a/endoscopydepthestimation-pytorch_amd/csrc/dgrad_wino_kernels.h
+++ b/endoscopydepthestimation-pytorch_amd/csrc/dgrad_wino_kernels.h
@@ -16,10 +16,10 @@
     int64_t u_off[kWinoDgradMaxLayers];
 };
 
-static __global__ void __launch_bounds__(256) dgrad_wino_weights_kernel(const WinoDgradTable t, const float* __restrict__ params, float* __restrict__ u,
-                                                                 int layout1_blocks = 0) {
+__device__ __forceinline__ void dgrad_wino_weights_items(const WinoDgradTable& t, const float* __restrict__ params, float* __restrict__ u, int layout1_blocks,
+                                                         int first, int step) {
     const int total = t.start[t.layers];
-    for (int item = blockIdx.x * blockDim.x + threadIdx.x; item < total; item += gridDim.x * blockDim.x) {
+    for (int item = first; item < total; item += step) {
         int l = 0;
         while (item >= t.start[l + 1]) ++l;
         const int e = item - t.start[l];
@@ -61,6 +61,10 @@
             dst[(4 * a + 3) * 192] = h[a][2];
         }
     }
+}
+static __global__ void __launch_bounds__(256) dgrad_wino_weights_kernel(const WinoDgradTable t, const float* __restrict__ params, float* __restrict__ u,
+                                                                 int layout1_blocks = 0) {
+    dgrad_wino_weights_items(t, params, u, layout1_blocks, blockIdx.x * blockDim.x + threadIdx.x, gridDim.x * blockDim.x);
 }
 
 template <int NL>
diff --git a/endoscopydepthestimation-pytorch_amd/csrc/net.hip b/endoscopydepthestimation-pytorch_amd/csrc/net.hip
--- a/endoscopydepthestimation-pytorch_amd/csrc/net.hip
+++ b/endoscopydepthestimation-pytorch_amd/csrc/net.hip
@@ -49,6 +49,9 @@
     WinoDgradTable wino_dgrad;
     int64_t wino_dgrad_floats = 0;
 };
+
+struct BnUse { const BnP* bn; int ch0; int block; };
+struct ConsumerRange { int level, c0, count, n; BnUse use[kBnMaxConsumers]; };
 
 inline int down_in(int level) { return kFirst + kNew * level; }
 inline int level_channels(int level) { return level < kLevels ? 144 + down_in(level) : 288 + kNew; }
@@ -134,7 +137,7 @@
     int n, h, w;
     int groups;
     int64_t gs;
-    struct Level { int h, w, t; int64_t plane; int64_t act, grad; int64_t sums; int64_t pq; } lv[kLevels + 1];
+    struct Level { int h, w, t; int64_t plane; int64_t act, grad; int64_t sums; } lv[kLevels + 1];
     int64_t pre_off;
     int64_t saved_off;
     int64_t idx_off[kLevels];
@@ -144,8 +147,8 @@
     int64_t partial_off;
     int64_t wino_off;
     int64_t wino4_off;
-    int64_t pq_off;
-    int64_t pq_floats;
+    int64_t tuw_off;
+    std::vector<ConsumerRange> ranges;
     int64_t scratch_off;
     int64_t scratch_bytes;
     int64_t slot_stride;
@@ -171,51 +174,39 @@
 struct BiasReduceTable {
     int n;
     struct Entry { const float* parts; float* bias; int count; int nparts; } e[kBiasPartLaunches];
+    const double* fw_parts;
+    float* fw_gw;
+    int fw_blocks, fw_count;
 };
 struct BiasParts {
     BiasReduceTable table;
     int64_t used;
 };
 
-struct BnFin4 {
-    const double* scratch[4];
-    const float* saved[4];
-    const float* gamma[4];
-    float* ggamma[4];
-    float* gbeta[4];
-};
-
 __global__ void __launch_bounds__(256) prep_dy_kernel(float* __restrict__ dbuf, const float* __restrict__ x, int64_t ns, int plane,
-                                                      const float* __restrict__ pq_p, const float* __restrict__ pq_q,
-                                                      float* bias_grad, int group_n, int64_t gs, const BnFin4 fin, int nl,
-                                                      double count, int training, int64_t slot_stride,
+                                                      float* bias_grad, int group_n, int64_t gs, const BnConsumers cons,
                                                       const float* __restrict__ vg, const float* __restrict__ vw, float* __restrict__ parts) {
     __shared__ double scratch[4];
+    __shared__ float s_term[2][kBnMaxConsumers];
     const int c = blockIdx.y;
     const int grp = blockIdx.z / group_n, n = blockIdx.z - grp * group_n;
-    float pc = pq_p[grp * gs + c], qc = pq_q[grp * gs + c];
-    if (nl > 0) {
-        const int64_t go = grp * gs;
-        double dp = 0.0, dq = 0.0;
-#pragma unroll
-        for (int j = 0; j < 4; ++j) {
-            if (j >= nl) break;
-            const double s1 = bn_slot_sum(fin.scratch[j] + go / 2 + 2 * c, slot_stride);
-            const double s2 = bn_slot_sum(fin.scratch[j] + go / 2 + 2 * c + 1, slot_stride);
-            if (blockIdx.x == 0 && n == 0 && threadIdx.x == 0) {
-                atomicAdd(fin.ggamma[j] + c, static_cast<float>(s2));
-                atomicAdd(fin.gbeta[j] + c, static_cast<float>(s1));
+    float pc = 0.f, qc = 0.f;
+    if (cons.n > 0) {
+        const int e = threadIdx.x;
+        if (e < cons.n) {
+            double s1, s2;
+            bn_consumer_term(cons, e, c, grp * gs, s1, s2, s_term[0][e], s_term[1][e]);
+            if (blockIdx.x == 0 && n == 0) {
+                atomicAdd(cons.e[e].ggamma + c, static_cast<float>(s2));
+                atomicAdd(cons.e[e].gbeta + c, static_cast<float>(s1));
             }
-            if (training) {
-                const double mean = fin.saved[j][go + 2 * c], rstd = fin.saved[j][go + 2 * c + 1];
-                const double scale = fin.gamma[j][c] * rstd;
-                const double k = scale * rstd * s2 / count;
-                dp += static_cast<double>(static_cast<float>(-k));
-                dq += static_cast<double>(static_cast<float>(-scale * s1 / count + k * mean));
-            }
-        }
-        pc += static_cast<float>(dp);
-        qc += static_cast<float>(dq);
+        }
+        __syncthreads();
+        double prun = 0.0, qrun = 0.0;
+        for (int i = 0; i < cons.n; ++i) {
+            bn_consumer_fold_step(cons, i, s_term[0][i], pc, prun);
+            bn_consumer_fold_step(cons, i, s_term[1][i], qc, qrun);
+        }
     }
     const int64_t base = grp * gs + n * ns + static_cast<int64_t>(c) * plane;
     const float* vg_n = vg ? vg + grp * gs + static_cast<int64_t>(n) * plane : nullptr;
@@ -276,8 +267,17 @@
 }
 
 __global__ void __launch_bounds__(256) bias_reduce_kernel(const BiasReduceTable tb) {
+    const int lane = threadIdx.x & 63, wave = threadIdx.x >> 6;
+    if (static_cast<int>(blockIdx.x) == tb.n) {
+        for (int c = blockIdx.y * 4 + wave; c < tb.fw_count; c += gridDim.y * 4) {
+            double t = 0.0;
+            for (int b = lane; b < tb.fw_blocks; b += 64) t += tb.fw_parts[static_cast<int64_t>(b) * tb.fw_count + c];
+            t = wave_sum(t);
+            if (lane == 0) atomicAdd(tb.fw_gw + c, static_cast<float>(t));
+        }
+        return;
+    }
     const BiasReduceTable::Entry& e = tb.e[blockIdx.x];
-    const int lane = threadIdx.x & 63, wave = threadIdx.x >> 6;
     for (int c = blockIdx.y * 4 + wave; c < e.count; c += gridDim.y * 4) {
         const float* src = e.parts + static_cast<int64_t>(c) * e.nparts;
         double t = 0.0;
@@ -287,57 +287,11 @@
     }
 }
 
-__global__ void bn_bwd_finalize_kernel(const double* __restrict__ scratch, const float* __restrict__ saved,
-                                       const float* __restrict__ gamma, float* __restrict__ ggamma, float* __restrict__ gbeta,
-                                       float* __restrict__ pq_p, float* __restrict__ pq_q, int c_count, double count, int training,
-                                       int64_t gs, int64_t slot_stride) {
-    scratch += blockIdx.y * (gs / 2); saved += blockIdx.y * gs; pq_p += blockIdx.y * gs; pq_q += blockIdx.y * gs;
-    for (int c = blockIdx.x * blockDim.x + threadIdx.x; c < c_count; c += gridDim.x * blockDim.x) {
-        const double s1 = bn_slot_sum(scratch + 2 * c, slot_stride), s2 = bn_slot_sum(scratch + 2 * c + 1, slot_stride);
-        atomicAdd(ggamma + c, static_cast<float>(s2));
-        atomicAdd(gbeta + c, static_cast<float>(s1));
-        if (training) {
-            const double mean = saved[2 * c], rstd = saved[2 * c + 1];
-            const double scale = gamma[c] * rstd;
-            const double k = scale * rstd * s2 / count;
-            pq_p[c] += static_cast<float>(-k);
-            pq_q[c] += static_cast<float>(-scale * s1 / count + k * mean);
-        }
-    }
-}
-
-__global__ void bn_bwd_finalize4_kernel(const BnFin4 a, int nl, float* __restrict__ pq_p, float* __restrict__ pq_q, int c_count, double count,
-                                        int training, int64_t gs, int64_t slot_stride) {
-    const int64_t go = blockIdx.y * gs;
-    pq_p += go; pq_q += go;
-    for (int c = blockIdx.x * blockDim.x + threadIdx.x; c < c_count; c += gridDim.x * blockDim.x) {
-        double dp = 0.0, dq = 0.0;
-#pragma unroll
-        for (int j = 0; j < 4; ++j) {
-            if (j >= nl) break;
-            const double s1 = bn_slot_sum(a.scratch[j] + go / 2 + 2 * c, slot_stride);
-            const double s2 = bn_slot_sum(a.scratch[j] + go / 2 + 2 * c + 1, slot_stride);
-            atomicAdd(a.ggamma[j] + c, static_cast<float>(s2));
-            atomicAdd(a.gbeta[j] + c, static_cast<float>(s1));
-            if (training) {
-                const double mean = a.saved[j][go + 2 * c], rstd = a.saved[j][go + 2 * c + 1];
-                const double scale = a.gamma[j][c] * rstd;
-                const double k = scale * rstd * s2 / count;
-                dp += static_cast<double>(static_cast<float>(-k));
-                dq += static_cast<double>(static_cast<float>(-scale * s1 / count + k * mean));
-            }
-        }
-        if (training) {
-            pq_p[c] += static_cast<float>(dp);
-            pq_q[c] += static_cast<float>(dq);
-        }
-    }
-}
-
-__global__ void tu_phase_weights_kernel(const float* __restrict__ w, int cout, int cin, float* __restrict__ out) {
+constexpr int kTuPhaseFloats = 2 * kNew * (2 * 12 * 16 + 16);
+__device__ __forceinline__ void tu_phase_weights_items(const float* __restrict__ w, int cout, int cin, float* __restrict__ out, int first, int step) {
     constexpr int kPhW = 2 * 12 * 16 + 16;
     const int total = 2 * cin * 2 * 12 * 16;
-    for (int i = blockIdx.x * blockDim.x + threadIdx.x; i < total; i += gridDim.x * blockDim.x) {
+    for (int i = first; i < total; i += step) {
         const int lane16 = i & 15;
         const int slot = (i >> 4) % 12;
         const int t = (i / (16 * 12)) & 1;
@@ -360,10 +314,11 @@
     }
 }
 
-__global__ void tu_subpix_dgrad_weights_kernel(const float* __restrict__ w, int cout, int cin, float* __restrict__ out) {
+constexpr int kTuSubpixFloats = 4 * kNew * (4 * kNew + 16);
+__device__ __forceinline__ void tu_subpix_dgrad_weights_items(const float* __restrict__ w, int cout, int cin, float* __restrict__ out, int first, int step) {
     const int pitch = 4 * cin + 16;
     const int total = 4 * cout * 4 * cin;
-    for (int i = blockIdx.x * blockDim.x + threadIdx.x; i < total; i += gridDim.x * blockDim.x) {
+    for (int i = first; i < total; i += step) {
         const int ci = i % cin;
         const int tap = (i / cin) & 3;
         const int co = (i / (4 * cin)) % cout;
@@ -377,6 +332,49 @@
             for (int kx = kx0; kx <= kx1; ++kx) v += src[ky * 3 + kx];
         out[static_cast<int64_t>(ph * cout + co) * pitch + tap * cin + ci] = v;
     }
+}
+
+struct PassPrep {
+    int dense_blocks, dense4_blocks;
+    int tu_blocks[kLevels];
+    int zero_blocks;
+    struct Tu { const float* w; float* out; int cout, cin; } tu[kLevels];
+    f32x4* zero;
+    int64_t zero_vecs, zero_gs;
+    int groups;
+    int total() const { int t = dense_blocks + dense4_blocks + zero_blocks; for (int l = 0; l < kLevels; ++l) t += tu_blocks[l]; return t; }
+};
+
+__device__ __forceinline__ bool prep_part(int& b, int blocks, int& first, int& step) {
+    if (b < blocks) { first = b * blockDim.x + threadIdx.x; step = blocks * blockDim.x; return true; }
+    b -= blocks;
+    return false;
+}
+
+__device__ __forceinline__ void prep_zero(const PassPrep& pp, int first, int step) {
+    for (int64_t v = first; v < pp.zero_vecs * pp.groups; v += step) {
+        const int64_t g = v / pp.zero_vecs;
+        pp.zero[g * pp.zero_gs + (v - g * pp.zero_vecs)] = f32x4{0.f, 0.f, 0.f, 0.f};
+    }
+}
+
+__global__ void __launch_bounds__(256) fwd_prepare_kernel(const WinoWeightTable wt, const WinoWeightTable wt4, const PassPrep pp, const float* __restrict__ params,
+                                                          float* __restrict__ u, float* __restrict__ u4) {
+    int b = blockIdx.x, first, step;
+    if (prep_part(b, pp.dense_blocks, first, step)) return wino_fwd_weights_items(wt, params, u, first, step);
+    if (prep_part(b, pp.dense4_blocks, first, step)) return wino4_fwd_weights_items(wt4, params, u4, first, step);
+    for (int l = 0; l < kLevels; ++l)
+        if (prep_part(b, pp.tu_blocks[l], first, step)) return tu_phase_weights_items(pp.tu[l].w, pp.tu[l].cout, pp.tu[l].cin, pp.tu[l].out, first, step);
+    prep_zero(pp, b * blockDim.x + threadIdx.x, pp.zero_blocks * blockDim.x);
+}
+
+__global__ void __launch_bounds__(256) bwd_prepare_kernel(const WinoDgradTable wd, int layout1_blocks, const PassPrep pp, const float* __restrict__ params,
+                                                          float* __restrict__ u) {
+    int b = blockIdx.x, first, step;
+    if (prep_part(b, pp.dense_blocks, first, step)) return dgrad_wino_weights_items(wd, params, u, layout1_blocks, first, step);
+    for (int l = 0; l < kLevels; ++l)
+        if (prep_part(b, pp.tu_blocks[l], first, step)) return tu_subpix_dgrad_weights_items(pp.tu[l].w, pp.tu[l].cout, pp.tu[l].cin, pp.tu[l].out, first, step);
+    prep_zero(pp, b * blockDim.x + threadIdx.x, pp.zero_blocks * blockDim.x);
 }
 
 __global__ void __launch_bounds__(256) finalize_partial_kernel(const float* __restrict__ partial, int64_t split_stride, int ksplit,
@@ -494,14 +492,6 @@
         const float t = static_cast<float>(scratch[0] + scratch[1] + scratch[2] + scratch[3]);
         if (c < cin) atomicAdd(gw + c, t); else atomicAdd(gb, t);
     }
-}
-
-__global__ void __launch_bounds__(64) final_w_reduce_kernel(const double* __restrict__ parts, int nblocks, int count, float* __restrict__ gw) {
-    const int c = blockIdx.x;
-    double t = 0.0;
-    for (int b = threadIdx.x; b < nblocks; b += 64) t += parts[static_cast<int64_t>(b) * count + c];
-    t = wave_sum(t);
-    if (threadIdx.x == 0) atomicAdd(gw + c, static_cast<float>(t));
 }
 
 constexpr int kBlocks = 2 * kLevels + 1, kDense = kBlocks * kLayers;
@@ -579,8 +569,6 @@
     double* out_sums(int level, int channel) const { return training ? sums(level) + 2 * channel : nullptr; }
     float* saved(const BnP& b) const { return tape + net->saved_off + 2 * b.saved; }
     double* scratch(const BnP& b) const { return reinterpret_cast<double*>(reinterpret_cast<char*>(gradws) + net->scratch_off) + 2 * b.saved; }
-    float* pq_p(int level) const { return gradws + net->pq_off + 2 * net->lv[level].pq; }
-    float* pq_q(int level) const { return pq_p(level) + net->lv[level].t; }
     uint8_t* idx(int level) const { return reinterpret_cast<uint8_t*>(tape) + net->idx_off[level]; }
 };
 
@@ -647,6 +635,46 @@
     const int i = b - kLevels - 1, l = kLevels - 1 - i;
     return {l, 0, 96 + down_in(l), tb.up_bn[i], tb.up_conv[i], l > 0};
 }
+static int build_consumer_ranges(std::vector<ConsumerRange>& out) {
+    const Table& tb = table();
+    struct Layer { const BnP* bn; int level, ch0, block; };
+    std::vector<Layer> chain;
+    for (int b = kBlocks - 1; b >= 0; --b) {
+        if (b < kLevels) chain.push_back({&tb.td_bn[b], b, 48, -1});
+        const DenseBlock k = dense_block(b);
+        for (int j = kLayers - 1; j >= 0; --j) chain.push_back({&k.bn[j], k.level, k.ic0, b});
+    }
+    auto add = [&](int level, int c0, int count) {
+        ConsumerRange r{level, c0, count, 0, {}};
+        for (const Layer& l : chain) {
+            if (l.level != level || l.ch0 + l.bn->c <= c0 || l.ch0 >= c0 + count) continue;
+            if (l.ch0 > c0 || l.ch0 + l.bn->c < c0 + count || r.n >= kBnMaxConsumers) return false;
+            r.use[r.n++] = {l.bn, l.ch0, l.block};
+        }
+        out.push_back(r);
+        return true;
+    };
+    out.clear();
+    bool ok = add(0, 48, kFirst);
+    for (int l = 0; l < kLevels; ++l) ok = ok && add(l + 1, l + 1 < kLevels ? 48 : 0, tb.td_conv[l].cout);
+    for (int b = 0; b < kBlocks; ++b) {
+        const DenseBlock k = dense_block(b);
+        for (int j = 0; j < kLayers; ++j) ok = ok && add(k.level, k.ic0 + k.c0 + kGrowth * j, kGrowth);
+    }
+    for (int l = 0; l < kLevels; ++l) ok = ok && add(l, 0, tb.tu_conv[kLevels - 1 - l].cout);
+    if (!ok) return ENDO_E_UNSUPPORTED;
+    for (const Layer& l : chain) {
+        std::vector<int> seen(l.bn->c, 0);
+        for (const ConsumerRange& r : out)
+            for (int e = 0; e < r.n; ++e)
+                if (r.use[e].bn == l.bn)
+                    for (int ch = 0; ch < r.count; ++ch) ++seen[r.c0 - r.use[e].ch0 + ch];
+        for (int v : seen)
+            if (v != 1) return ENDO_E_UNSUPPORTED;
+    }
+    return 0;
+}
+
 static long tile_count(const Ctx& c, int level, int tx, int ty) {
     const auto& lv = c.net->lv[level];
     return static_cast<long>((lv.w + tx - 1) / tx) * ((lv.h + ty - 1) / ty) * c.nt();
@@ -790,9 +818,7 @@
     ProfScope prof(kProfConv3x3Up, c.stream, conv_flops(c.net, level, cv.cin, cv.cout, 3),
                    4.0 * c.nt() * c.net->lv[level].plane * (cv.cin / 4.0 + cv.cout));
     if (c.fwd->tu_subpix[level]) {
-        float* w3 = c.tape + c.net->partial_off;
-        tu_phase_weights_kernel<<<(2 * cv.cin * 384 + 255) / 256, 256, 0, c.stream>>>(c.params + cv.w, cv.cout, cv.cin, w3);
-        ENDO_LAUNCH_CHECK();
+        const float* w3 = c.tape + c.net->tuw_off + level * kTuPhaseFloats;
         ConvParams p{};
         fill_grid(c, p, src_level);
         fill_in(c, p, c.act(src_level), src_level, src_c0, cv.cin);
@@ -813,9 +839,32 @@
 
 struct FinalVirt { const float* vg; const float* vw; float* gw; };
 
-static int prep_dy(const Ctx& c, int level, int c0, int count, float* bias_grad, const BnFin4* fin = nullptr, int nl = 0, const FinalVirt* fv = nullptr) {
+static int bn_consumers(const Ctx& c, int level, int c0, int count, BnConsumers& cons) {
+    const ConsumerRange* r = nullptr;
+    for (const ConsumerRange& k : c.net->ranges)
+        if (k.level == level && k.c0 == c0 && k.count == count) r = &k;
+    if (!r) return ENDO_E_BADARG;
     const auto& lv = c.net->lv[level];
-    BnFin4 none{};
+    cons = BnConsumers{};
+    cons.n = r->n;
+    cons.training = c.training;
+    cons.count = static_cast<double>(c.net->n) * lv.h * lv.w;
+    cons.slot_stride = c.net->slot_stride;
+    for (int e = 0; e < r->n; ++e) {
+        const BnUse& u = r->use[e];
+        const int off = c0 - u.ch0;
+        cons.e[e] = {c.scratch(*u.bn) + 2 * off, c.saved(*u.bn) + 2 * off, c.params + u.bn->g + off, c.grads + u.bn->g + off, c.grads + u.bn->b + off};
+        const bool run_goes_on = e + 1 < r->n && u.block >= 0 && r->use[e + 1].block == u.block && c.bwd->block[u.block].fused;
+        if (!run_goes_on) cons.group_end |= 1u << e;
+    }
+    return 0;
+}
+
+static int prep_dy(const Ctx& c, int level, int c0, int count, float* bias_grad, const FinalVirt* fv = nullptr) {
+    const auto& lv = c.net->lv[level];
+    BnConsumers cons;
+    int rc = bn_consumers(c, level, c0, count, cons);
+    if (rc) return rc;
     int bx = static_cast<int>((lv.plane + 4095) / 4096);
     bx = bx < 1 ? 1 : (bx > 32 ? 32 : bx);
     float* parts = nullptr;
@@ -829,23 +878,8 @@
     }
     ProfScope prof(kProfSmall, c.stream, 0.0, 12.0 * c.nt() * lv.plane * count);
     prep_dy_kernel<<<dim3(bx, count, c.nt()), 256, 0, c.stream>>>(c.gbuf(level) + c0 * lv.plane, c.act(level) + c0 * lv.plane,
-                                                                     lv.t * lv.plane, static_cast<int>(lv.plane), c.pq_p(level) + c0,
-                                                                     c.pq_q(level) + c0, bias_grad, c.net->n, c.net->gs, fin ? *fin : none, fin ? nl : 0,
-                                                                     static_cast<double>(c.net->n) * lv.h * lv.w, c.training, c.net->slot_stride,
+                                                                     lv.t * lv.plane, static_cast<int>(lv.plane), bias_grad, c.net->n, c.net->gs, cons,
                                                                      fv ? fv->vg : nullptr, fv ? fv->vw + c0 : nullptr, parts);
-    ENDO_LAUNCH_CHECK();
-    return 0;
-}
-
-static int bn_finalize(const Ctx& c, const BnP& b, int level, int ic0, int first = 0, int count = -1) {
-    const auto& lv = c.net->lv[level];
-    if (count < 0) count = b.c - first;
-    if (count <= 0) return 0;
-    ProfScope prof(kProfSmall, c.stream, 0.0, 0.0);
-    bn_bwd_finalize_kernel<<<dim3((count + 127) / 128, c.net->groups), 128, 0, c.stream>>>(c.scratch(b) + 2 * first, c.saved(b) + 2 * first, c.params + b.g + first,
-                                                                       c.grads + b.g + first, c.grads + b.b + first,
-                                                                       c.pq_p(level) + ic0 + first, c.pq_q(level) + ic0 + first, count,
-                                                                       static_cast<double>(c.net->n) * lv.h * lv.w, c.training, c.net->gs, c.net->slot_stride);
     ENDO_LAUNCH_CHECK();
     return 0;
 }
@@ -880,7 +914,7 @@
     p.ns = lv.t * lv.plane; p.cs = static_cast<int>(lv.plane);
 }
 
-static DgradBlockParams newmap_params(const Ctx& c, const DenseBlock& k, int j, BnFin4* a = nullptr) {
+static DgradBlockParams newmap_params(const Ctx& c, const DenseBlock& k, int j) {
     const auto& lv = c.net->lv[k.level];
     const int nl = kLayers - j;
     const int t0 = k.c0 + kGrowth * (j - 1);
@@ -897,7 +931,6 @@
         p.wgt[l] = c.params + k.cv[j + l].w; p.w_cin[l] = k.cv[j + l].cin;
         p.saved[l] = c.saved(b) + 2 * t0; p.gamma[l] = c.params + b.g + t0; p.beta[l] = c.params + b.b + t0;
         p.scratch[l] = c.scratch(b) + 2 * t0;
-        if (a) { a->scratch[l] = p.scratch[l]; a->saved[l] = p.saved[l]; a->gamma[l] = p.gamma[l]; a->ggamma[l] = c.grads + b.g + t0; a->gbeta[l] = c.grads + b.b + t0; }
     }
     return p;
 }
@@ -1085,7 +1118,7 @@
         rc = launch_dgrad_dense_auto(p, c.stream);
         if (rc) return rc;
     }
-    return bn_finalize(c, bn, level, ic0);
+    return 0;
 }
 
 template <int NL>
@@ -1112,11 +1145,9 @@
         }
         return 0;
     }
-    BnFin4 pending{};
-    int pending_nl = 0;
     F34ReduceBatch red{};
     for (int j = kLayers - 1; j >= 0; --j) {
-        int rc = prep_dy(c, level, new0 + kGrowth * j, kGrowth, c.grads + k.cv[j].b, &pending, pending_nl, (fv && j == kLayers - 1) ? fv : nullptr);
+        int rc = prep_dy(c, level, new0 + kGrowth * j, kGrowth, c.grads + k.cv[j].b, (fv && j == kLayers - 1) ? fv : nullptr);
         if (rc) return rc;
         const bool defer = c.bwd->overlap == 2;
         if (!defer || j == 0) {
@@ -1135,15 +1166,12 @@
         }
         if (j > 0) {
             const int nl = kLayers - j;
-            BnFin4 a{};
-            DgradBlockParams p = newmap_params(c, k, j, &a);
+            DgradBlockParams p = newmap_params(c, k, j);
             if (fv) { p.vg = fv->vg; p.vw = fv->vw + ic0 + p.w_ci_off; }
             ProfScope prof(kProfDgradDense, c.stream, 2.0 * c.nt() * lv.plane * kGrowth * kGrowth * 9 * nl,
                            4.0 * c.nt() * lv.plane * (3.0 * kGrowth + kGrowth * nl));
             rc = nl == 1 ? launch_newmap<1>(bl.newmap[j], p, c.stream) : nl == 2 ? launch_newmap<2>(bl.newmap[j], p, c.stream) : launch_newmap<3>(bl.newmap[j], p, c.stream);
             if (rc) return rc;
-            pending = a;
-            pending_nl = nl;
         }
     }
     {
@@ -1165,25 +1193,13 @@
                 int used = 0;
                 rc = run_dgrad_wino3p_nl4(p, u, std::min(device_cu_count(), kFwPartBlocks), fwp, &used, c.stream);
                 if (rc == 0 && fwp) {
-                    final_w_reduce_kernel<<<c0, 64, 0, c.stream>>>(fwp, used, c0, fv->gw + ic0);
-                    ENDO_LAUNCH_CHECK();
+                    BiasReduceTable& tb = c.bias_parts->table;
+                    tb.fw_parts = fwp; tb.fw_blocks = used; tb.fw_count = c0; tb.fw_gw = fv->gw + ic0;
                 }
                 break;
             }
         }
         if (rc) return rc;
-    }
-    {
-        BnFin4 a;
-        for (int j = 0; j < kLayers; ++j) {
-            a.scratch[j] = c.scratch(k.bn[j]); a.saved[j] = c.saved(k.bn[j]); a.gamma[j] = c.params + k.bn[j].g;
-            a.ggamma[j] = c.grads + k.bn[j].g; a.gbeta[j] = c.grads + k.bn[j].b;
-        }
-        ProfScope prof(kProfSmall, c.stream, 0.0, 0.0);
-        bn_bwd_finalize4_kernel<<<dim3((c0 + 127) / 128, c.net->groups), 128, 0, c.stream>>>(a, kLayers, c.pq_p(level) + ic0, c.pq_q(level) + ic0, c0,
-                                                                         static_cast<double>(c.net->n) * lv.h * lv.w, c.training, c.net->gs,
-                                                                         c.net->slot_stride);
-        ENDO_LAUNCH_CHECK();
     }
     return 0;
 }
@@ -1216,7 +1232,7 @@
         }
         if (rc) return rc;
     }
-    return bn_finalize(c, b, level, 48);
+    return 0;
 }
 
 static int tu_bwd(const Ctx& c, int level, int src_level, int src_c0, const ConvP& cv) {
@@ -1244,9 +1260,7 @@
         fill_out(c, p, c.gbuf(src_level), src_level, src_c0, cv.cin);
         return launch_conv_dma_auto<3, 4, 3, IN_PLAIN, EPI_DGRAD_SUMPOOL, 4>(p, c.stream);
     }
-    float* wd = c.gradws + c.net->tuw_scratch_off;
-    tu_subpix_dgrad_weights_kernel<<<(16 * cv.cout * cv.cin + 255) / 256, 256, 0, c.stream>>>(c.params + cv.w, cv.cout, cv.cin, wd);
-    ENDO_LAUNCH_CHECK();
+    const float* wd = c.gradws + c.net->tuw_scratch_off + level * kTuSubpixFloats;
     ConvParams p{};
     fill_grid(c, p, src_level);
     fill_in(c, p, c.gbuf(level), level, 0, 4 * cv.cout);
@@ -1259,6 +1273,15 @@
 }
 
 static int64_t align_up(int64_t v, int64_t a) { return (v + a - 1) / a * a; }
+
+static void prep_zero_region(PassPrep& pp, char* base, int64_t bytes, const endo_net* net) {
+    pp.zero = reinterpret_cast<f32x4*>(base);
+    pp.zero_vecs = bytes / 16;
+    pp.zero_gs = net->gs / 4;
+    pp.groups = net->groups;
+    const int64_t blocks = (pp.zero_vecs * pp.groups + 4 * 256 - 1) / (4 * 256);
+    pp.zero_blocks = static_cast<int>(blocks < 1 ? 1 : (blocks > 1024 ? 1024 : blocks));
+}
 
 }
 
@@ -1272,7 +1295,7 @@
     net->n = n; net->h = h; net->w = w; net->groups = groups;
     net->wstream = nullptr; net->ev_fork = nullptr; net->ev_join = nullptr;
     default_options(net->opt);
-    int64_t off = 0, sums = 0, pq = 0;
+    int64_t off = 0, sums = 0;
     for (int l = 0; l <= kLevels; ++l) {
         auto& lv = net->lv[l];
         lv.h = h >> l; lv.w = w >> l; lv.t = level_channels(l);
@@ -1280,7 +1303,6 @@
         lv.act = off; lv.grad = off;
         off += align_up(static_cast<int64_t>(n) * lv.t * lv.plane, 64);
         lv.sums = sums; sums += 2 * lv.t;
-        lv.pq = pq; pq += lv.t;
     }
     const int64_t acts = off;
     net->pre_off = off; off += align_up(static_cast<int64_t>(n) * h * w, 64);
@@ -1299,15 +1321,15 @@
     byte_off += align_up(tb.wino_floats * 4, 256);
     net->wino4_off = byte_off / 4;
     byte_off += align_up(tb.wino4_floats * 4, 256);
+    net->tuw_off = byte_off / 4;
+    byte_off += align_up(static_cast<int64_t>(kLevels) * kTuPhaseFloats * 4, 256);
     net->tape_floats = byte_off / 4;
-    net->pq_off = acts;
-    net->pq_floats = 2 * pq;
-    net->scratch_off = align_up((acts + net->pq_floats) * 4, 256);
+    net->scratch_off = align_up(acts * 4, 256);
     net->slot_stride = align_up(tb.bn_width_total * 2, 32);
     net->scratch_bytes = net->slot_stride * 8 * kBnSlots;
     net->wg_scratch_off = (net->scratch_off + align_up(net->scratch_bytes, 256)) / 4;
     net->tuw_scratch_off = net->wg_scratch_off + std::max(std::max(kNsScratchFloats, kSpScratchFloats), 4 * kF34ScratchFloats);
-    net->wd_off = align_up(net->tuw_scratch_off + 4 * kNew * (4 * kNew + 16), 64);
+    net->wd_off = align_up(net->tuw_scratch_off + kLevels * kTuSubpixFloats, 64);
     net->gplane_off = align_up(net->wd_off + tb.wino_dgrad_floats, 64);
     net->bias_parts_off = net->gplane_off + align_up(static_cast<int64_t>(n) * h * w, 64);
     net->bias_parts_floats = static_cast<int64_t>(kBiasPartChannels) * n * groups * 32;
@@ -1323,6 +1345,7 @@
     net->fw_parts_off = net->bias_parts_off + align_up(net->bias_parts_floats, 64);
     net->gradws_floats = net->fw_parts_off + 2 * static_cast<int64_t>(kFwPartBlocks) * 192;
     net->gs = align_up(net->tape_floats > net->gradws_floats ? net->tape_floats : net->gradws_floats, 64);
+    if (int rc = build_consumer_ranges(net->ranges)) { delete net; return rc; }
     *out = net;
     return 0;
 }
@@ -1391,15 +1414,21 @@
     Ctx c{net, params, bn_running, tape, nullptr, nullptr, training, static_cast<hipStream_t>(stream_)};
     const FwdPlan plan = plan_fwd(c);
     c.fwd = &plan;
-    for (int g = 0; g < net->groups; ++g)
-        ENDO_CHECK(hipMemsetAsync(reinterpret_cast<char*>(tape + g * net->gs) + net->sums_off, 0, net->sums_bytes, c.stream));
-    if (!plan.bf16) {
+    {
         ProfScope prof(kProfSmall, c.stream, 0.0, 4.0 * (tb.wino_floats + tb.wino_floats * 9 / 16));
         WinoWeightTable wt = tb.wino;
         for (int l = 0; l < wt.layers; ++l) wt.mode[l] = plan.dense[l].chunk_weights ? 1 : 0;
-        wino_fwd_weights_kernel<<<(wt.start[wt.layers] + 255) / 256, 256, 0, c.stream>>>(wt, params, tape + net->wino_off);
-        ENDO_LAUNCH_CHECK();
-        if (plan.wino4_weights) wino4_fwd_weights_kernel<<<(tb.wino4.start[tb.wino4.layers] + 255) / 256, 256, 0, c.stream>>>(tb.wino4, params, tape + net->wino4_off);
+        PassPrep pp{};
+        if (!plan.bf16) pp.dense_blocks = (wt.start[wt.layers] + 255) / 256;
+        if (!plan.bf16 && plan.wino4_weights) pp.dense4_blocks = (tb.wino4.start[tb.wino4.layers] + 255) / 256;
+        for (int l = 0; l < kLevels; ++l) {
+            const ConvP& cv = tb.tu_conv[kLevels - 1 - l];
+            if (!plan.tu_subpix[l]) continue;
+            pp.tu[l] = {params + cv.w, tape + net->tuw_off + l * kTuPhaseFloats, cv.cout, cv.cin};
+            pp.tu_blocks[l] = (2 * cv.cin * 384 + 255) / 256;
+        }
+        prep_zero_region(pp, reinterpret_cast<char*>(tape) + net->sums_off, net->sums_bytes, net);
+        fwd_prepare_kernel<<<pp.total(), 256, 0, c.stream>>>(wt, tb.wino4, pp, params, tape + net->wino_off, tape + net->wino4_off);
         ENDO_LAUNCH_CHECK();
     }
     int rc;
@@ -1459,14 +1488,20 @@
         ENDO_CHECK(hipEventCreateWithFlags(&net->ev_fork, hipEventDisableTiming));
         ENDO_CHECK(hipEventCreateWithFlags(&net->ev_join, hipEventDisableTiming));
     }
-    for (int g = 0; g < net->groups; ++g)
-        ENDO_CHECK(hipMemsetAsync(gradws + g * net->gs + net->pq_off, 0,
-                                  static_cast<size_t>(net->scratch_off + net->scratch_bytes - net->pq_off * 4), c.stream));
-    if (plan.dgrad_weights) {
+    {
         ProfScope prof(kProfSmall, c.stream, 0.0, 4.0 * 2.0 * tb.wino_dgrad_floats);
         int layout1_blocks = 0;
         for (int b = 0; b < kBlocks; ++b) layout1_blocks |= plan.block[b].wino3_layout ? 1 << b : 0;
-        dgrad_wino_weights_kernel<<<(tb.wino_dgrad.start[tb.wino_dgrad.layers] + 255) / 256, 256, 0, c.stream>>>(tb.wino_dgrad, params, gradws + net->wd_off, layout1_blocks);
+        PassPrep pp{};
+        if (plan.dgrad_weights) pp.dense_blocks = (tb.wino_dgrad.start[tb.wino_dgrad.layers] + 255) / 256;
+        for (int l = 0; l < kLevels; ++l) {
+            const ConvP& cv = tb.tu_conv[kLevels - 1 - l];
+            if (plan.tu_dgrad[l] == TuDgrad::Plain) continue;
+            pp.tu[l] = {params + cv.w, gradws + net->tuw_scratch_off + l * kTuSubpixFloats, cv.cout, cv.cin};
+            pp.tu_blocks[l] = (16 * cv.cout * cv.cin + 255) / 256;
+        }
+        prep_zero_region(pp, reinterpret_cast<char*>(gradws) + net->scratch_off, net->scratch_bytes, net);
+        bwd_prepare_kernel<<<pp.total(), 256, 0, c.stream>>>(tb.wino_dgrad, layout1_blocks, pp, params, gradws + net->wd_off);
         ENDO_LAUNCH_CHECK();
     }
     int rc;
@@ -1516,10 +1551,12 @@
     {
         WgradParams p = first_wgrad_params(c);
         const auto& lv = net->lv[0];
+        BnConsumers cons;
         if (plan.first == FirstWgrad::F34Prep) {
             p.prep_x = c.act(0) + 48 * lv.plane;
-            p.prep_p = c.pq_p(0) + 48; p.prep_q = c.pq_q(0) + 48;
             p.prep_bias = grads + tb.first.b;
+            rc = bn_consumers(c, 0, 48, kFirst, cons);
+            if (rc) return rc;
         } else {
             rc = prep_dy(c, 0, 48, kFirst, grads + tb.first.b);
             if (rc) return rc;
@@ -1529,16 +1566,16 @@
         if (rc) return rc;
         ProfScope prof(kProfWgradOther, cw.stream, conv_flops(net, 0, 3, kFirst, 3), 4.0 * c.nt() * lv.plane * (3 + kFirst));
         switch (plan.first) {
-            case FirstWgrad::F34Prep: rc = launch_wgrad_f34<0, true, true>(p, gradws + net->wg_scratch_off, cw.stream); break;
+            case FirstWgrad::F34Prep: rc = launch_wgrad_f34<0, true, true>(p, gradws + net->wg_scratch_off, cw.stream, nullptr, &cons); break;
             case FirstWgrad::F34: rc = launch_wgrad_f34<0, true>(p, gradws + net->wg_scratch_off, cw.stream); break;
             case FirstWgrad::Taps: rc = launch_wgrad_taps<12, IN_PLAIN>(p, cw.stream); break;
             case FirstWgrad::Direct: rc = launch_wgrad<3, 3, IN_PLAIN, DY_PLAIN>(p, cw.stream); break;
         }
         if (rc) return rc;
     }
-    if (bias_parts.table.n > 0) {
+    if (bias_parts.table.n > 0 || bias_parts.table.fw_parts) {
         ProfScope prof(kProfSmall, c.stream, 0.0, 4.0 * bias_parts.used);
-        bias_reduce_kernel<<<dim3(bias_parts.table.n, 8), 256, 0, c.stream>>>(bias_parts.table);
+        bias_reduce_kernel<<<dim3(bias_parts.table.n + (bias_parts.table.fw_parts ? 1 : 0), 8), 256, 0, c.stream>>>(bias_parts.table);
         ENDO_LAUNCH_CHECK();
     }
     if (net->wstream) {
diff --git a/endoscopydepthestimation-pytorch_amd/csrc/wgrad_f34_kernels.h b/endoscopydepthestimation-pytorch_amd/csrc/wgrad_f34_kernels.h
--- a/endoscopydepthestimation-pytorch_amd/csrc/wgrad_f34_kernels.h
+++ b/endoscopydepthestimation-pytorch_amd/csrc/wgrad_f34_kernels.h
@@ -67,7 +67,7 @@
 }
 
 template <int EXP = 0, bool RAW = false, bool PREP = false>
-__global__ void __launch_bounds__(kConvThreads, 2) wgrad_f34_kernel(const WgradParams p, float* __restrict__ partial, const F34Plan plan) {
+__global__ void __launch_bounds__(kConvThreads, 2) wgrad_f34_kernel(const WgradParams p, float* __restrict__ partial, const F34Plan plan, const BnConsumers cons) {
     extern __shared__ __attribute__((aligned(16))) float smem[];
     const int tid = threadIdx.x;
     const int lane = tid & 63;
@@ -140,9 +140,34 @@
         const __amdgpu_buffer_rsrc_t xr = f34_rsrc(p.in + sm.in_off(p), p.cin * p.in_cs * 4);
         const __amdgpu_buffer_rsrc_t gr = f34_rsrc(p.dy + sm.dy_off(p) + (RAW ? static_cast<int64_t>(12 * group) * p.dy_cs : 0), 12 * p.dy_cs * 4);
         const __amdgpu_buffer_rsrc_t pr = f34_rsrc((PREP ? p.prep_x : p.dy) + sm.dy_off(p) + (RAW ? static_cast<int64_t>(12 * group) * p.dy_cs : 0), 12 * p.dy_cs * 4);
-        if (PREP && sm.grp != cst_grp) {
-            prep_pc = li < 12 ? p.prep_p[sm.grp * p.gs + 12 * group + li] : 0.f;
-            prep_qc = li < 12 ? p.prep_q[sm.grp * p.gs + 12 * group + li] : 0.f;
+        if constexpr (PREP) {
+            if (sm.grp != cst_grp) {
+                const int64_t go = sm.grp * p.gs;
+                const bool first_tile = u == sm.grp * p.group_n * YS * S;
+                double prun = 0.0, qrun = 0.0;
+                prep_pc = 0.f; prep_qc = 0.f;
+#pragma unroll 1
+                for (int e0 = 0; e0 < cons.n; e0 += 4) {
+                    const int e = e0 + lk;
+                    float pe = 0.f, qe = 0.f;
+                    if (e < cons.n && li < 12) {
+                        double s1, s2;
+                        bn_consumer_term(cons, e, 12 * group + li, go, s1, s2, pe, qe);
+                        if (first_tile) {
+                            atomicAdd(cons.e[e].ggamma + 12 * group + li, static_cast<float>(s2));
+                            atomicAdd(cons.e[e].gbeta + 12 * group + li, static_cast<float>(s1));
+                        }
+                    }
+#pragma unroll
+                    for (int j = 0; j < 4; ++j) {
+                        const float pj = __shfl(pe, li + 16 * j, 64), qj = __shfl(qe, li + 16 * j, 64);
+                        if (e0 + j < cons.n) {
+                            bn_consumer_fold_step(cons, e0 + j, pj, prep_pc, prun);
+                            bn_consumer_fold_step(cons, e0 + j, qj, prep_qc, qrun);
+                        }
+                    }
+                }
+            }
         }
         if (sm.grp != cst_grp) {
             sc = 0.f; sh = 0.f;
@@ -418,11 +443,12 @@
 }
 
 template <int EXP = 0, bool RAW = false, bool PREP = false>
-inline int launch_wgrad_f34(const WgradParams& p, float* scratch, hipStream_t stream, F34ReduceBatch* batch = nullptr) {
+inline int launch_wgrad_f34(const WgradParams& p, float* scratch, hipStream_t stream, F34ReduceBatch* batch = nullptr, const BnConsumers* cons = nullptr) {
     static_assert(!PREP || RAW, "the fused gradient preparation belongs to the first convolution's form");
     const F34Plan plan = wgrad_f34_plan(p, kF34Blocks / 2, RAW);
     constexpr int lds = 4 * 2 * kF34Xs * 4;
-    ENDO_CHECK(launch_dyn(wgrad_f34_kernel<EXP, RAW, PREP>, kF34Blocks, kConvThreads, lds, stream, p, scratch, plan));
+    if (PREP && !cons) return ENDO_E_BADARG;
+    ENDO_CHECK(launch_dyn(wgrad_f34_kernel<EXP, RAW, PREP>, kF34Blocks, kConvThreads, lds, stream, p, scratch, plan, cons ? *cons : BnConsumers{}));
     if (batch && !RAW && batch->count < 4) {
         const int k = batch->count++;
         batch->partial[k] = scratch; batch->dw[k] = p.dw; batch->plan[k] = plan; batch->cin[k] = p.cin;
diff --git a/endoscopydepthestimation-pytorch_amd/csrc/wgrad_kernels.h b/endoscopydepthestimation-pytorch_amd/csrc/wgrad_kernels.h
--- a/endoscopydepthestimation-pytorch_amd/csrc/wgrad_kernels.h
+++ b/endoscopydepthestimation-pytorch_amd/csrc/wgrad_kernels.h
@@ -30,8 +30,6 @@
     int group_n;
     int64_t gs, in_gs;
     const float* prep_x;
-    const float* prep_p;
-    const float* prep_q;
     float* prep_bias;
 };
 
diff --git a/endoscopydepthestimation-pytorch_amd/csrc/wino4_fwd_kernels.h b/endoscopydepthestimation-pytorch_amd/csrc/wino4_fwd_kernels.h
--- a/endoscopydepthestimation-pytorch_amd/csrc/wino4_fwd_kernels.h
+++ b/endoscopydepthestimation-pytorch_amd/csrc/wino4_fwd_kernels.h
@@ -16,9 +16,9 @@
 
 constexpr int kW4UStride = 576;
 
-__global__ void __launch_bounds__(256) wino4_fwd_weights_kernel(const WinoWeightTable t, const float* __restrict__ params, float* __restrict__ u) {
+__device__ __forceinline__ void wino4_fwd_weights_items(const WinoWeightTable& t, const float* __restrict__ params, float* __restrict__ u, int first, int step) {
     const int total = t.start[t.layers];
-    for (int item = blockIdx.x * blockDim.x + threadIdx.x; item < total; item += gridDim.x * blockDim.x) {
+    for (int item = first; item < total; item += step) {
         int l = 0;
         while (item >= t.start[l + 1]) ++l;
         const int e = item - t.start[l];
@@ -61,6 +61,9 @@
             for (int jj = 0; jj < 6; ++jj) dst[(i >> 1) * 192 + (i & 1) * 6 + jj] = o[jj];
         }
     }
+}
+__global__ void __launch_bounds__(256) wino4_fwd_weights_kernel(const WinoWeightTable t, const float* __restrict__ params, float* __restrict__ u) {
+    wino4_fwd_weights_items(t, params, u, blockIdx.x * blockDim.x + threadIdx.x, gridDim.x * blockDim.x);
 }
 
 struct Wino4Geom {
diff --git a/endoscopydepthestimation-pytorch_amd/csrc/wino_fwd_kernels.h b/endoscopydepthestimation-pytorch_amd/csrc/wino_fwd_kernels.h
--- a/endoscopydepthestimation-pytorch_amd/csrc/wino_fwd_kernels.h
+++ b/endoscopydepthestimation-pytorch_amd/csrc/wino_fwd_kernels.h
@@ -18,9 +18,9 @@
 };
 constexpr int kDenseChunkFloats = 9 * 16 * 16;
 
-__global__ void __launch_bounds__(256) wino_fwd_weights_kernel(const WinoWeightTable t, const float* __restrict__ params, float* __restrict__ u) {
+__device__ __forceinline__ void wino_fwd_weights_items(const WinoWeightTable& t, const float* __restrict__ params, float* __restrict__ u, int first, int step) {
     const int total = t.start[t.layers];
-    for (int item = blockIdx.x * blockDim.x + threadIdx.x; item < total; item += gridDim.x * blockDim.x) {
+    for (int item = first; item < total; item += step) {
         int l = 0;
         while (item >= t.start[l + 1]) ++l;
         const int e = item - t.start[l];
@@ -68,6 +68,9 @@
             for (int k = 0; k < 16; ++k) dst[256 + k] = 0.f;
         }
     }
+}
+__global__ void __launch_bounds__(256) wino_fwd_weights_kernel(const WinoWeightTable t, const float* __restrict__ params, float* __restrict__ u) {
+    wino_fwd_weights_items(t, params, u, blockIdx.x * blockDim.x + threadIdx.x, gridDim.x * blockDim.x);
 }
 
 constexpr int kWinoFwdStages = 2;
```

Result: no change. 516.5, median of 6 (+0.9%).
